# theislab/dca

Hardware: AMD Instinct MI355X
Metric: cells/sec training (ZINB AE, 68k x 20k) (higher is better)
Workload: dtype f32

## Files before the change

dca_amd/build.py:

```python
import os
import shutil
import subprocess
import sys

HERE = os.path.dirname(os.path.abspath(__file__))
ROOT = os.path.dirname(HERE)
CSRC = os.path.join(HERE, 'csrc')
LIB = os.path.join(CSRC, 'libdcahip.so')
SOURCES = ['dcahip_zinb.hip', 'dcahip_gemm.hip', 'dcahip_layers.hip', 'dcahip_heads.hip', 'dcahip_prep.hip', 'dcahip_opt.hip',
           'dcahip_dropout.hip', 'dcahip_sparse.hip', 'dcahip_peer.hip', 'dcahip_knn.hip', 'dcahip_kmeans.hip', 'dcahip_gram.hip',
           'dcahip_silhouette.hip', 'dcahip_ranksum.hip', 'dcahip_louvain.hip']
HEADERS = ['zinb_math.hpp', 'h2_math.hpp', 'philox.hpp', 'knn_dist.hpp']
ARCH = 'gfx950'
HOST_LIB = os.path.join(CSRC, 'libdcahost.so')
HOST_SOURCES = ['dcahost_tsv.cpp', 'dcahost_read.cpp']


def _hipcc():
    for c in (shutil.which('hipcc'), '/opt/rocm/bin/hipcc'):
        if c and os.path.exists(c):
            return c
    raise RuntimeError('hipcc not found: cannot build libdcahip.so')


def _deps():
    return [os.path.join(CSRC, s) for s in SOURCES + HEADERS] + [os.path.join(ROOT, 'include', 'dcahip.h')]


def source_fingerprint():
    import hashlib
    h = hashlib.sha256()
    for d in _deps():
        h.update(os.path.basename(d).encode())
        if os.path.exists(d):
            with open(d, 'rb') as f:
                h.update(f.read())
    return h.hexdigest()


def needs_build():
    if not os.path.exists(LIB):
        return True
    t = os.path.getmtime(LIB)
    if any(os.path.exists(d) and os.path.getmtime(d) > t for d in _deps()):
        return True
    try:
        with open(LIB + '.src') as f:
            return f.read().strip() != source_fingerprint()
    except OSError:
        return True


def _obj_path(src, tag):
    return os.path.join(CSRC, '_obj', os.path.basename(src) + ('.' + tag if tag else '') + '.o')


def _obj_fingerprint(src, hdrs, defines):
    import hashlib
    h = hashlib.sha256()
    for d in [src] + list(hdrs):
        h.update(os.path.basename(d).encode())
        with open(d, 'rb') as f:
            h.update(f.read())
    h.update('\0'.join(defines).encode())
    return h.hexdigest()


def _obj_is_fresh(obj, fp):
    try:
        with open(obj + '.src') as f:
            return os.path.exists(obj) and f.read().strip() == fp
    except OSError:
        return False


def build_hip(force=False, verbose=True, defines=(), out=None):
    out = out or LIB
    if not force and not defines and out == LIB and not needs_build():
        return LIB
    from concurrent.futures import ThreadPoolExecutor
    os.makedirs(os.path.join(CSRC, '_obj'), exist_ok=True)
    tag = '_'.join(d.replace('=', '-') for d in defines)
    hdrs = [os.path.join(CSRC, h) for h in HEADERS] + [os.path.join(ROOT, 'include', 'dcahip.h')]
    hdrs = [h for h in hdrs if os.path.exists(h)]
    srcs = [os.path.join(CSRC, s) for s in SOURCES if os.path.exists(os.path.join(CSRC, s))]
    jobs, stamps = [], []
    for src in srcs:
        obj = _obj_path(src, tag)
        fp = _obj_fingerprint(src, hdrs, defines)
        if force or not _obj_is_fresh(obj, fp):
            if os.path.exists(obj + '.src'):
                os.remove(obj + '.src')
            jobs.append([_hipcc(), '--offload-arch=' + ARCH, '-O3', '-std=c++17', '-fPIC', '-c',
                         '-I' + os.path.join(ROOT, 'include')] + ['-D' + d for d in defines] + ['-o', obj, src])
            stamps.append((obj, fp))
# ... 44 lines not shown
```

dca_amd/config.py:

```python
import os
from dataclasses import dataclass, fields


def _flag(name, default):
    v = os.environ.get(name)
    return default if v is None else v not in ('0', '', 'off', 'false', 'False')


@dataclass
class EngineConfig:
    stack: str = 'steps'
    bwd_chain: bool = True
    wide_planes: bool = True
    wide_h2: bool = True
    dp_sharded_opt: bool = False
    dp_graph: bool = True
    dp_peer_exchange: bool = False
    device_prep: bool = True
    fused_write: bool = True
    resident: str = 'auto'
    counts_compact: bool = False
    graph_steps: int = 8
    sparse_dw_min: int = 512
    lut_fwd_min: int = 1024
    enc0_nt_min: int = 256
    predict_chunk: int = 1024

    _ENV = {'stack': 'DCA_AMD_STACK', 'bwd_chain': 'DCA_AMD_BWD_CHAIN', 'wide_planes': 'DCA_AMD_WIDE_PLANES', 'wide_h2': 'DCA_AMD_WIDE_H2',
            'dp_sharded_opt': 'DCA_AMD_DP_SHARDED_OPT', 'dp_graph': 'DCA_AMD_DP_GRAPH', 'device_prep': 'DCA_AMD_DEVICE_PREP',
            'fused_write': 'DCA_AMD_FUSED_WRITE', 'dp_peer_exchange': 'DCA_AMD_DP_PEER', 'resident': 'DCA_AMD_RESIDENT',
            'counts_compact': 'DCA_AMD_COUNTS_COMPACT'}

    @classmethod
    def from_env(cls):
        c = cls()
        for f in fields(cls):
            env = cls._ENV.get(f.name)
            if env is None:
                continue
            if f.type is bool or isinstance(getattr(c, f.name), bool):
                setattr(c, f.name, _flag(env, getattr(c, f.name)))
            elif os.environ.get(env) is not None:
                setattr(c, f.name, type(getattr(c, f.name))(os.environ[env]))
        if c.stack not in ('steps', 'coop', 'off'):
            raise ValueError('DCA_AMD_STACK must be steps, coop or off (got %r)' % c.stack)
        if c.resident not in ('auto', 'counts', 'dense'):
            raise ValueError('DCA_AMD_RESIDENT must be auto, counts or dense (got %r)' % c.resident)
        return c


def current():
    return EngineConfig.from_env()
```

dca_amd/csrc/dcahip_heads.hip:

```cpp
#include <hip/hip_runtime.h>
#include <stdint.h>
#include <type_traits>
#include "dcahip.h"
#include "zinb_math.hpp"

namespace {

using f32x16 = __attribute__((ext_vector_type(16))) float;

constexpr int kTG = 32;
constexpr int kTR = 32;
constexpr int kLdS = 33;
constexpr int kWG = 2;
constexpr int kMaxGrid = 2048;
constexpr int kMaxSmallGrid = 8192;
constexpr int kCUs = 256;
constexpr int kZU = 4;
constexpr int kQCap = 320;

__device__ __forceinline__ int rowmap(int e, int hi) { return (e & 3) + 8 * (e >> 2) + 4 * hi; }

__device__ __forceinline__ void wave_sync() {
    __builtin_amdgcn_fence(__ATOMIC_RELEASE, "wavefront");
    __builtin_amdgcn_wave_barrier();
    __builtin_amdgcn_fence(__ATOMIC_ACQUIRE, "wavefront");
}

using f16x8 = __attribute__((ext_vector_type(8))) _Float16;
using f16x2v = __attribute__((ext_vector_type(2))) _Float16;
using f32x2v = __attribute__((ext_vector_type(2))) float;
using u32x4 = __attribute__((ext_vector_type(4))) unsigned;
using u32x2 = __attribute__((ext_vector_type(2))) unsigned;
using s16x4 = __attribute__((ext_vector_type(4))) short;

constexpr int kWR2 = 8;
constexpr int kWr8MinNT = 5;
constexpr int kHTile = 2 * 32 * 64;
constexpr int kTop = 13;
constexpr int kDExp0 = 8;
constexpr float kDLim = 30000.f;
constexpr int kDSlack = 2;
constexpr int kEHZero = 64;

#define MFMAH(a, b, c) __builtin_amdgcn_mfma_f32_32x32x16_f16(__builtin_bit_cast(f16x8, a), __builtin_bit_cast(f16x8, b), c, 0, 0, 0)

__device__ __forceinline__ unsigned pk_f16(float a, float b) {
    return __builtin_bit_cast(unsigned, __builtin_convertvector(f32x2v{a, b}, f16x2v));
}
__device__ __forceinline__ float resid_lo(unsigned p, float x) {
    float r;
    asm("v_fma_mix_f32 %0, %1, -1.0, %2 op_sel:[0,0,0] op_sel_hi:[1,0,0]" : "=v"(r) : "v"(p), "v"(x));
    return r;
}
__device__ __forceinline__ float resid_hi(unsigned p, float x) {
    float r;
    asm("v_fma_mix_f32 %0, %1, -1.0, %2 op_sel:[1,0,0] op_sel_hi:[1,0,0]" : "=v"(r) : "v"(p), "v"(x));
    return r;
}
__device__ __forceinline__ void split_pair(float x0, float x1, unsigned& p0, unsigned& p1) {
    p0 = pk_f16(x0, x1);
    p1 = pk_f16(resid_lo(p0, x0), resid_hi(p0, x1));
}
__device__ __forceinline__ void split8(const float (&x)[8], u32x4 (&f)[2]) {
#pragma unroll
    for (int j = 0; j < 4; ++j) {
        unsigned a, b;
        split_pair(x[2 * j], x[2 * j + 1], a, b);
        f[0][j] = a; f[1][j] = b;
    }
}
#ifdef DCA_EXP_H2_TWO
#define MFMA_H3(A, Bf, ACC) { ACC = MFMAH(A[0], Bf[1], ACC); ACC = MFMAH(A[0], Bf[0], ACC); }
#else
#define MFMA_H3(A, Bf, ACC) { ACC = MFMAH(A[1], Bf[0], ACC); ACC = MFMAH(A[0], Bf[1], ACC); ACC = MFMAH(A[0], Bf[0], ACC); }
#endif

__device__ __forceinline__ float pow2i(int e) { return __uint_as_float((unsigned)(127 + e) << 23); }
__device__ __forceinline__ int block_exp(float m) {
    if (!(m > 0.f) || !(m < INFINITY)) return 0;
    const int e = kTop + 1 - __builtin_amdgcn_frexp_expf(m);
    return e < -60 ? -60 : (e > 60 ? 60 : e);
}
__device__ __forceinline__ float wave_max(float v) {
    int l = (int)__builtin_amdgcn_mbcnt_hi(~0u, __builtin_amdgcn_mbcnt_lo(~0u, 0u));
    asm volatile("" : "+v"(l));
#pragma unroll
    for (int off = 32; off > 0; off >>= 1)
// ... 651 lines not shown

    __syncthreads();

    {
        float* red = lds;
#pragma unroll
        for (int step = 1; step < WR; step *= 2) {
            const int slot = r / (2 * step);
            float* rs = red + (long)slot * NRED * 64 + lane;
            if (r % (2 * step) == step) {
                int n = 0;
#pragma unroll
                for (int h = 0; h < NH; ++h)
#pragma unroll
                    for (int ib = 0; ib < 2; ++ib)
#pragma unroll
                        for (int e = 0; e < 16; ++e) rs[(n++) * 64] = dW[h][ib][e];
#pragma unroll
                for (int h = 0; h < NH; ++h) rs[(n++) * 64] = bsum[h];
                rs[(n++) * 64] = thsum;
            }
            __syncthreads();
            if (r % (2 * step) == 0 && r + step < WR) {
                int n = 0;
#pragma unroll
                for (int h = 0; h < NH; ++h)
#pragma unroll
                    for (int ib = 0; ib < 2; ++ib)
#pragma unroll
                        for (int e = 0; e < 16; ++e) dW[h][ib][e] += rs[(n++) * 64];
#pragma unroll
                for (int h = 0; h < NH; ++h) bsum[h] += rs[(n++) * 64];
                thsum += rs[(n++) * 64];
            }
            __syncthreads();
        }
    }
    if (r == 0 && tile_ok) {
        const bool direct = p.S == 1;
        float* out = direct ? p.gW : p.ws_dw + (long)s * p.dw_stride;
        const long ldo = direct ? p.ldg : p.ldws;
        const float fin = direct ? p.inv_n : 1.f;
        const bool cw = gene < p.plane;
#pragma unroll
        for (int h = 0; h < NH; ++h) {
#pragma unroll
            for (int ib = 0; ib < 2; ++ib)
#pragma unroll
                for (int e = 0; e < 16; ++e) {
                    const int i = ib * 32 + rowmap(e, hi);
                    if (cw && i < p.hL) out[(long)i * ldo + (long)h * p.plane + gene] = dW[h][ib][e] * fin;
                }
            const float bv = bsum[h] + __shfl_xor(bsum[h], 32, 64);
            if (cw && hi == 0) out[(long)p.hL * ldo + (long)h * p.plane + gene] = bv * fin;
        }
        if (CONST_DISP) {
            const float tv = thsum + __shfl_xor(thsum, 32, 64);
            if (direct) {
                if (gvalid && hi == 0) {
                    const float e = expf(p.theta_w[gene]);
                    p.g_theta[gene] = (e >= 1e-3f && e <= 1e4f) ? tv * p.inv_n * e : 0.f;
                }
            } else if (cw && hi == 0) {
                out[(long)(p.hL + 1) * ldo + gene] = tv;
            }
        }
    }
    __syncthreads();
    first_item = false;
    }

#pragma unroll
    for (int off = 32; off > 0; off >>= 1) dacc += __shfl_down(dacc, off, 64);
    if (lane == 0) lred[wave] = dacc;
    __syncthreads();
    if (tid == 0) {
        double v = 0.0;
        for (int w = 0; w < WR; ++w) v += lred[w];
        p.partials[blockIdx.x] = v;
    }
}


struct ReduceDwArgs {
    const float* ws; int S; long stride; int hL; long ldws, ncols; float* gW; long ldg;
    const float* theta_w; float* g_theta; int G;
    float scale;
    const float* ws2; int S2; const int* tail_tiles; int ntail; long plane;
    int tail_first;
};

__device__ __forceinline__ void reduce_dw_body(const ReduceDwArgs& q, int bid, int nblk) {
    const int hL = q.hL;
    const long ldws = q.ldws, ncols = q.ncols; float* gW = q.gW; const long ldg = q.ldg;
    const float* theta_w = q.theta_w; float* g_theta = q.g_theta; const int G = q.G;
    const float sc = q.scale;
    __shared__ unsigned tailbm[kMaxGrid / 32];
    if (q.ntail > 0) {
        for (int i = threadIdx.x; i < kMaxGrid / 32; i += 256) tailbm[i] = 0u;
        __syncthreads();
        for (int i = threadIdx.x; i < q.ntail; i += 256) {
            const int tl = q.tail_tiles ? q.tail_tiles[i] : q.tail_first + i;
            if (tl >= 0 && tl < kMaxGrid) atomicOr(&tailbm[tl >> 5], 1u << (tl & 31));
        }
        __syncthreads();
    }
    auto is_tail = [&](long col_in_plane) { const int tl = (int)(col_in_plane / kTG); return q.ntail > 0 && ((tailbm[tl >> 5] >> (tl & 31)) & 1u); };
    if ((ncols & 3) == 0 && (ldws & 3) == 0 && (ldg & 3) == 0 && (q.stride & 3) == 0 && (q.plane & 3) == 0 &&
        ((reinterpret_cast<uintptr_t>(q.ws) | reinterpret_cast<uintptr_t>(gW) | reinterpret_cast<uintptr_t>(q.ws2)) & 15) == 0) {
        const long nq = ncols >> 2, totalq = (long)(hL + 1) * nq;
        for (long idx = (long)bid * 256 + threadIdx.x; idx < totalq; idx += (long)nblk * 256) {
            const long i = idx / nq, c = (idx - i * nq) << 2;
            const bool tl = is_tail(c % q.plane);
            const float* ws = tl ? q.ws2 : q.ws; const int S = tl ? q.S2 : q.S; const long stride = q.stride;
            float4 v = *reinterpret_cast<const float4*>(ws + i * ldws + c);
            for (int s = 1; s < S; ++s) {
                const float4 x = *reinterpret_cast<const float4*>(ws + (long)s * stride + i * ldws + c);
                v.x += x.x; v.y += x.y; v.z += x.z; v.w += x.w;
            }
            v.x *= sc; v.y *= sc; v.z *= sc; v.w *= sc;
            *reinterpret_cast<float4*>(gW + i * ldg + c) = v;
        }
    } else {
        const long total = (long)(hL + 1) * ncols;
        for (long idx = (long)bid * 256 + threadIdx.x; idx < total; idx += (long)nblk * 256) {
            const long i = idx / ncols, c = idx - i * ncols;
            const bool tl = is_tail(c % q.plane);
            const float* ws = tl ? q.ws2 : q.ws; const int S = tl ? q.S2 : q.S;
            float v = 0.f;
            for (int s = 0; s < S; ++s) v += ws[(long)s * q.stride + i * ldws + c];
            gW[i * ldg + c] = v * sc;
        }
    }
    if (g_theta) {
        for (long c = (long)bid * 256 + threadIdx.x; c < G; c += (long)nblk * 256) {
            const bool tl = is_tail(c);
            const float* ws = tl ? q.ws2 : q.ws; const int S = tl ? q.S2 : q.S; const long stride = q.stride;
            float v = 0.f;
            for (int s = 0; s < S; ++s) v += ws[(long)s * stride + (long)(hL + 1) * ldws + c];
            const float e = expf(theta_w[c]);
            g_theta[c] = (e >= 1e-3f && e <= 1e4f) ? v * sc * e : 0.f;
        }
    }
}

__global__ __launch_bounds__(256) void heads_reduce_dw_kernel(ReduceDwArgs q) { reduce_dw_body(q, blockIdx.x, gridDim.x); }

struct ReduceDhArgs {
    const float* ws; int ntg, B, Bpad, KT, hL; float* dH; long lddh; float scale;
    const double* loss_partials; int n_partials; double loss_scale; float* loss_out;
    const float* ws2; int ntg2;
};

template <int GL>
__device__ __forceinline__ void reduce_dh_body(const ReduceDhArgs& q, int bid) {
    const float* ws = q.ws; const int ntg = q.ntg, B = q.B, KT = q.KT, hL = q.hL; float* dH = q.dH; const long lddh = q.lddh;
    const double* loss_partials = q.loss_partials; const int n_partials = q.n_partials; const double loss_scale = q.loss_scale;
    float* loss_out = q.loss_out;
    constexpr int OUT = 256 / GL;
    __shared__ float4 red[256];
    const int o = threadIdx.x % OUT, gl = threadIdx.x / OUT;
    const int q4 = KT / 4;
    const long nq = (long)B * q4;
    const long quad = (long)bid * OUT + o;
    float4 v = make_float4(0.f, 0.f, 0.f, 0.f);
    if (quad < nq) {
        const long tq = (long)kTR * q4;
        const long t = quad / tq, within = quad - t * tq;
        const float4* src = reinterpret_cast<const float4*>(ws) + t * ntg * tq + within;
        for (int gt0 = gl; gt0 < ntg; gt0 += 8 * GL) {
            float4 x[8];
#pragma unroll
            for (int u = 0; u < 8; ++u) {
                const int gt = gt0 + u * GL;
                x[u] = src[(long)(gt < ntg ? gt : gl) * tq];
            }
#pragma unroll
            for (int u = 0; u < 8; ++u)
                if (gt0 + u * GL < ntg) { v.x += x[u].x; v.y += x[u].y; v.z += x[u].z; v.w += x[u].w; }
        }
        if (q.ntg2 > 0) {
            const float4* src2 = reinterpret_cast<const float4*>(q.ws2) + t * q.ntg2 * tq + within;
            for (int gt = gl; gt < q.ntg2; gt += GL) { const float4 x = src2[(long)gt * tq]; v.x += x.x; v.y += x.y; v.z += x.z; v.w += x.w; }
        }
    }
    red[threadIdx.x] = v;
    __syncthreads();
    if (gl == 0 && quad < nq) {
#pragma unroll
        for (int k = 1; k < GL; ++k) {
            const float4 x = red[k * OUT + o];
            v.x += x.x; v.y += x.y; v.z += x.z; v.w += x.w;
        }
        const long row = quad / q4;
        const int i = (int)(quad - row * q4) * 4;
        float* d = dH + row * lddh + i;
        if (i + 0 < hL) d[0] = v.x * q.scale;
        if (i + 1 < hL) d[1] = v.y * q.scale;
        if (i + 2 < hL) d[2] = v.z * q.scale;
        if (i + 3 < hL) d[3] = v.w * q.scale;
    }
    if (loss_out && bid == 0) {
        __shared__ double lsum[256];
        double a = 0.0;
        for (int i = threadIdx.x; i < n_partials; i += 256) a += loss_partials[i];
        lsum[threadIdx.x] = a;
        __syncthreads();
        for (int st = 128; st > 0; st >>= 1) {
            if ((int)threadIdx.x < st) lsum[threadIdx.x] += lsum[threadIdx.x + st];
            __syncthreads();
        }
        if (threadIdx.x == 0) {
            float lf = (float)(lsum[0] * loss_scale);
            if (isnan(lf)) lf = INFINITY;
            *loss_out = lf;
        }
    }
}

template <int GL>
__global__ __launch_bounds__(256) void heads_reduce_dh_kernel(ReduceDhArgs q) { reduce_dh_body<GL>(q, blockIdx.x); }

template <int GL>
__global__ __launch_bounds__(256) void heads_reduce_both_kernel(ReduceDhArgs qh, ReduceDwArgs qw, int n_dh) {
    if ((int)blockIdx.x < n_dh) reduce_dh_body<GL>(qh, blockIdx.x);
    else reduce_dw_body(qw, blockIdx.x - n_dh, gridDim.x - n_dh);
}
// ... 463 lines not shown
        const long ldo = p.NT == 1 ? p.ldg : p.ldws;
        const float fin = p.NT == 1 ? p.inv_n : 1.f;
        const float wun = pow2i(-(eHt + kD0 - shift)) * 1.f;
#pragma unroll
        for (int ib = 0; ib < 2; ++ib)
#pragma unroll
            for (int e = 0; e < 16; ++e) {
                const int i = ib * 32 + rowmap(e, hi);
                const float v = dW[ib][e] * wun * fin;
                if (cw && i < p.hL) out[(long)i * ldo + (long)h * p.plane + gene] = v;
            }
        const float bv = (bsum + __shfl_xor(bsum, 32, 64)) * pow2i(-kD0) * fin;
        if (cw && hi == 0) out[(long)p.hL * ldo + (long)h * p.plane + gene] = bv;
    }

#pragma unroll
    for (int off = 32; off > 0; off >>= 1) dacc += __shfl_down(dacc, off, 64);
    if (lane == 0) lred[wave] = dacc;
    __syncthreads();
    if (tid == 0) p.partials[blockIdx.x] = ((lred[0] + lred[1]) + lred[2]) + lred[3];
}

__global__ __launch_bounds__(64) void x3_product_kernel(const float* A, const float* B, float* C, int K) {
    const int lane = threadIdx.x, l31 = lane & 31, hi = lane >> 5;
    float ma = 0.f, mb = 0.f;
    for (int k0 = 0; k0 < K; k0 += 16)
#pragma unroll
        for (int j = 0; j < 8; ++j) {
            ma = fmaxf(ma, fabsf(A[(long)l31 * K + k0 + 8 * hi + j]));
            mb = fmaxf(mb, fabsf(B[(long)(k0 + 8 * hi + j) * 32 + l31]));
        }
    const int ea = block_exp(wave_max(ma)), eb = block_exp(wave_max(mb));
    const float sa = pow2i(ea), sb = pow2i(eb);
    f32x16 acc;
#pragma unroll
    for (int e = 0; e < 16; ++e) acc[e] = 0.f;
    for (int k0 = 0; k0 < K; k0 += 16) {
        float av[8], bv[8];
#pragma unroll
        for (int j = 0; j < 8; ++j) {
            av[j] = A[(long)l31 * K + k0 + 8 * hi + j] * sa;
            bv[j] = B[(long)(k0 + 8 * hi + j) * 32 + l31] * sb;
        }
        u32x4 af[2], bf[2];
        split8(av, af);
        split8(bv, bf);
        MFMA_H3(af, bf, acc)
    }
    const float un = pow2i(-(ea + eb));
#pragma unroll
    for (int e = 0; e < 16; ++e) C[rowmap(e, hi) * 32 + l31] = acc[e] * un;
}

template <bool P, bool C, bool YC>
void launch_fused(const HeadsPlan& pl, const HeadsArgs2& a, hipStream_t s) {
    if (pl.small) hipLaunchKernelGGL((heads_fused_small_kernel<P, C, YC>), dim3(pl.grid), dim3(256), 0, s, a);
    else hipLaunchKernelGGL((heads_fused_h2_kernel<P, C, YC>), dim3(pl.grid), dim3(64 * kWR2), 0, s, a);
}

}

extern "C" long dcahip_heads_fused_workspace_bytes(int B, int hL, int G, long plane, int flags) {
    HeadsPlan p;
    if (!make_heads_plan(B, hL, G, plane, flags, &p)) return 0;
    long need = 0;
    for (int nt = 1; nt <= p.NT; ++nt) {
        const int b = nt * kTR < B ? nt * kTR : B;
        HeadsPlan q;
        if (!make_heads_plan(b, hL, G, plane, flags, &q)) continue;
        const long n = q.dw_bytes + q.dh_bytes + q.hs_bytes + q.dw2_bytes + q.dh2_bytes;
        if (n > need) need = n;
    }
    return need;
}

extern "C" int dcahip_x3_product_32x32(const float* A, const float* B, float* C, int K, void* stream) {
    if (!A || !B || !C || K <= 0 || (K & 15)) return DCAHIP_EINVAL;
    hipLaunchKernelGGL(x3_product_kernel, dim3(1), dim3(64), 0, static_cast<hipStream_t>(stream), A, B, C, K);
    return (int)hipGetLastError();
}

extern "C" int dcahip_heads_tile_order_len(int G) { return G > 0 ? (((G + kTG - 1) / kTG + kWG - 1) / kWG) * kWG : 0; }

extern "C" int dcahip_heads_fused(const float* H, long ldh, const float* Wh, long ldw,
                                  const float* bh, long plane, const float* theta_w,
                                  const float* y, long ldy,
                                  const unsigned char* yc, long ldc, const int* ovf_ptr, const int* ovf_col,
                                  const float* ovf_val, const float* sf, const int* perm,
                                  const long long* cursor, int B, int hL, int G, float ridge,
                                  float inv_n, int flags, float* gW, long ldg, float* g_theta,
                                  float* dH, long lddh, double* loss_partials, int* n_partials_out,
                                  void* workspace, long workspace_bytes, const int* tile_order,
                                  float* loss_out, int d_exp, void* stream) {
    const bool has_pi = flags & DCAHIP_NLL_HAS_PI, cdisp = flags & DCAHIP_NLL_CONST_DISP;
    HeadsPlan pl;
    if (!make_heads_plan(B, hL, G, plane, flags, &pl)) return DCAHIP_EINVAL;
    if (!H || !Wh || !bh || (!y && !yc) || !sf || !gW || !dH || !loss_partials || !workspace) return DCAHIP_EINVAL;
    if (cdisp && (!theta_w || !g_theta)) return DCAHIP_EINVAL;
    if (workspace_bytes < pl.dw_bytes + pl.dh_bytes + pl.hs_bytes + pl.dw2_bytes + pl.dh2_bytes) return DCAHIP_EINVAL;
    if (!al16(H) || !al16(Wh) || !al16(workspace) || (ldh & 3) || (ldw & 3) || ldh < ((hL + 3) & ~3))
        return DCAHIP_EINVAL;
    if (d_exp > 0 || d_exp < -24 || !(ridge >= 0.f) || ridge > 1e3f) return DCAHIP_EINVAL;
    const int NH = 1 + (cdisp ? 0 : 1) + (has_pi ? 1 : 0);
    if (ldw < (long)NH * plane || ldg < (long)NH * plane) return DCAHIP_EINVAL;
    if (yc ? (ldc < G || ldc > 0xffffffffL) : (ldy < G || ldy > 0xffffffffL)) return DCAHIP_EINVAL;
    float* ws_dh = static_cast<float*>(workspace);
    float* ws_dw = ws_dh + pl.dh_bytes / sizeof(float);
    float* ws_dh2 = ws_dw + pl.dw_bytes / sizeof(float);
    float* ws_dw2 = ws_dh2 + pl.dh2_bytes / sizeof(float);
    hipStream_t s = static_cast<hipStream_t>(stream);
    bool direct_dw = false;
    {
        unsigned short* HA = reinterpret_cast<unsigned short*>(reinterpret_cast<char*>(workspace) + pl.dh_bytes + pl.dw_bytes +
                                                               pl.dh2_bytes + pl.dw2_bytes);
        unsigned short* HT = HA + (long)pl.NT * kHTile;
        int* eH = reinterpret_cast<int*>(HT + (long)pl.NT * kHTile);
        if (!pl.small) {
            hipLaunchKernelGGL(heads_split_h_kernel, dim3(pl.NT), dim3(256), 0, s, H, ldh, B, hL, HA, HT, eH);
            int rc0 = (int)hipGetLastError();
            if (rc0 != 0) return rc0;
        }
        direct_dw = pl.S == 1;
        HeadsArgs2 a{HA, HT, eH, H, ldh, gW, ldg, g_theta, Wh, ldw, bh, theta_w, y, ldy, yc, ldc, ovf_ptr, ovf_col, ovf_val,
                     sf, perm, cursor, ws_dw, pl.dw_stride, ws_dh,
                     pl.npart, pl.nitems, tile_order, loss_partials, plane, pl.ldws, B, hL, G, pl.S, pl.NT, ridge, inv_n, d_exp, 0};
        auto launch = [&](const HeadsPlan& q, const HeadsArgs2& b) {
            if (yc) {
                if (has_pi && cdisp) launch_fused<true, true, true>(q, b, s);
                else if (has_pi) launch_fused<true, false, true>(q, b, s);
                else if (cdisp) launch_fused<false, true, true>(q, b, s);
                else launch_fused<false, false, true>(q, b, s);
            } else {
                if (has_pi && cdisp) launch_fused<true, true, false>(q, b, s);
                else if (has_pi) launch_fused<true, false, false>(q, b, s);
                else if (cdisp) launch_fused<false, true, false>(q, b, s);
                else launch_fused<false, false, false>(q, b, s);
            }
        };
        launch(pl, a);
        if (pl.ntail > 0) {
            HeadsPlan q2 = pl;
            q2.grid = pl.grid2; q2.S = pl.S2;
            HeadsArgs2 b = a;
            b.ws_dw = ws_dw2; b.ws_dh = ws_dh2; b.npart = pl.npart2; b.nitems = pl.nitems2; b.S = pl.S2;
            b.partials = loss_partials + pl.grid; b.tile_base = pl.nmain;
            launch(q2, b);
        }
    }
    int rc = (int)hipGetLastError();
    if (rc != 0) return rc;
    const int n_part = pl.grid + pl.grid2;
    if (n_partials_out) *n_partials_out = n_part;
    {
        const int KT = pl.HLB * 32;
        const long nq = (long)B * (KT / 4);
        const ReduceDhArgs qh{ws_dh, pl.npart, B, pl.NT * kTR, KT, hL, dH, lddh, inv_n, loss_partials, n_part, (double)inv_n, loss_out,
                              ws_dh2, pl.npart2};
        const long total = (long)(hL + 1) * pl.ldws;
        long gr = (total / 4 + 255) / 256;
        if (gr > 2048) gr = 2048;
        if (gr < 1) gr = 1;
        const ReduceDwArgs qw{ws_dw, pl.S, pl.dw_stride, hL, pl.ldws, pl.ldws, gW, ldg, cdisp ? theta_w : nullptr,
                              cdisp ? g_theta : nullptr, G, inv_n,
                              ws_dw2, pl.S2, (pl.ntail > 0 && tile_order) ? tile_order + pl.nmain : nullptr, pl.ntail, plane, pl.nmain};
        const int gl = (nq <= 1024 && pl.npart >= 256) ? 64 : (nq >= 64L * 512 ? 4 : 16);
        const int n_dh = (int)((nq + 256 / gl - 1) / (256 / gl));
        if (!direct_dw) {
            const dim3 grid(n_dh + (int)gr);
            if (gl == 64) hipLaunchKernelGGL(heads_reduce_both_kernel<64>, grid, dim3(256), 0, s, qh, qw, n_dh);
            else if (gl == 4) hipLaunchKernelGGL(heads_reduce_both_kernel<4>, grid, dim3(256), 0, s, qh, qw, n_dh);
            else hipLaunchKernelGGL(heads_reduce_both_kernel<16>, grid, dim3(256), 0, s, qh, qw, n_dh);
        } else {
            if (gl == 64) hipLaunchKernelGGL(heads_reduce_dh_kernel<64>, dim3(n_dh), dim3(256), 0, s, qh);
            else if (gl == 4) hipLaunchKernelGGL(heads_reduce_dh_kernel<4>, dim3(n_dh), dim3(256), 0, s, qh);
            else hipLaunchKernelGGL(heads_reduce_dh_kernel<16>, dim3(n_dh), dim3(256), 0, s, qh);
        }
        rc = (int)hipGetLastError();
    }
    return rc;
}
```

dca_amd/csrc/dcahip_layers.hip:

```cpp
#include <hip/hip_runtime.h>
#include <stdint.h>
#include "dcahip.h"

namespace {

constexpr int kMaxChunks = 256;
constexpr int kApplyRows = 16;

constexpr float kSeluScale = 1.0507009873554805f, kSeluAlpha = 1.6732632423543772f;
constexpr int kActPre = 12;

__device__ __attribute__((noinline)) float act_fwd_other(int a, float x) {
    switch (a) {
        case 2: return tanhf(x);
        case 3: { const float e = expf(-fabsf(x)); const float s = 1.f / (1.f + e); return x >= 0.f ? s : e * s; }
        case 4: return x > 0.f ? x : expm1f(x);
        case 5: return kSeluScale * (x > 0.f ? x : kSeluAlpha * expm1f(x));
        case 6: return fmaxf(x, 0.f) + log1pf(expf(-fabsf(x)));
        case 7: return x / (1.f + fabsf(x));
        case 10: return fminf(fmaxf(0.2f * x + 0.5f, 0.f), 1.f);
        case 11: return expf(x);
        case 12: { const float e = expf(-fabsf(x)); const float s = 1.f / (1.f + e); return x * (x >= 0.f ? s : e * s); }
        case 13: return 0.5f * x * (1.f + erff(x * 0.70710678118654752f));
        default: return x > 0.f ? x : 0.3f * x;
    }
}
__device__ __forceinline__ float act_fwd(int a, float x) {
    if (a == 1) return fmaxf(x, 0.f);
    if (a == 0) return x;
    return act_fwd_other(a, x);
}

__device__ __attribute__((noinline)) float act_grad_other(int a, float v) {
    switch (a) {
        case 2: return 1.f - v * v;
        case 3: return v * (1.f - v);
        case 4: return v > 0.f ? 1.f : v + 1.f;
        case 5: return v > 0.f ? kSeluScale : v + kSeluScale * kSeluAlpha;
        case 6: return -expm1f(-v);
        case 7: { const float t = 1.f - fabsf(v); return t * t; }
        case 10: return v > 0.f && v < 1.f ? 0.2f : 0.f;
        case 11: return v;
        case 12: {
            const float e = expf(-fabsf(v)); const float s0 = 1.f / (1.f + e); const float s = v >= 0.f ? s0 : e * s0;
            return s * (1.f + v * (1.f - s));
        }
        case 13:
            return 0.5f * (1.f + erff(v * 0.70710678118654752f)) + v * 0.39894228040143268f * expf(-0.5f * v * v);
        default: return v > 0.f ? 1.f : 0.3f;
    }
}
__device__ __forceinline__ float act_grad(int a, float h) {
    if (a == 1) return h > 0.f ? 1.f : 0.f;
    if (a == 0) return 1.f;
    return act_grad_other(a, h);
}
__device__ __forceinline__ float act_slope(int a, float h, float xh, float bc) {
    if (a == 1) return h > 0.f ? 1.f : 0.f;
    if (a == 0) return 1.f;
    return act_grad_other(a, a >= kActPre ? xh + bc : h);
}
__device__ __forceinline__ float pre_beta(int a, const float* beta, int c) {
    return a >= kActPre ? beta[c] : 0.f;
}

__host__ __device__ inline int n_chunks(int B) {
    int r = (B + 63) / 64;
    return r < 1 ? 1 : (r > kMaxChunks ? kMaxChunks : r);
}
__host__ __device__ inline int chunk_rows(int B, int R) { return (B + R - 1) / R; }
inline int strip_blocks(int H, int row_blocks) {
    const int strips = (H + 63) / 64;
    int y = row_blocks > 0 ? 512 / row_blocks : strips;
    if (y < 1) y = 1;
    return y < strips ? y : strips;
}

__device__ __forceinline__ float wg_rowlane_sum(float v, float* sm ) {
    const int tx = threadIdx.x & 63, ty = threadIdx.x >> 6;
    __syncthreads();
    sm[ty * 64 + tx] = v;
    __syncthreads();
    return (sm[tx] + sm[64 + tx]) + (sm[128 + tx] + sm[192 + tx]);
}

// ... 737 lines not shown
            for (int r = 0; r < a.B; ++r) {
                const float d = dZs[r][c];
                cs += d;
#pragma unroll
                for (int j = 0; j < NK; ++j) {
                    const int k = wg + kBwdWGs * (ty + 4 * j);
                    acc[j] = fmaf(k < a.K ? Hs[r][k] : 0.f, d, acc[j]);
                }
            }
#pragma unroll
            for (int j = 0; j < NK; ++j) {
                const int k = wg + kBwdWGs * (ty + 4 * j);
                if (k < a.K) a.gW[(long)k * a.ldg + c] = acc[j];
            }
            if (wg == 0 && ty == 0) a.gW[(long)a.K * a.ldg + c] = cs;
        }
    }
    if (a.dHp) {
        const int k = tx;
        if (k < a.K) {
            constexpr int NR = RPT / kBwdWGs;
            float acc[NR];
#pragma unroll
            for (int j = 0; j < NR; ++j) acc[j] = 0.f;
            for (int c = 0; c < a.H; ++c) {
                const float w = Ws[k][c];
#pragma unroll
                for (int j = 0; j < NR; ++j) {
                    const int r = wg + kBwdWGs * (ty + 4 * j);
                    acc[j] = fmaf(r < a.B ? dZs[r][c] : 0.f, w, acc[j]);
                }
            }
#pragma unroll
            for (int j = 0; j < NR; ++j) {
                const int r = wg + kBwdWGs * (ty + 4 * j);
                if (r < a.B) a.dHp[(long)r * a.lddp + k] = acc[j];
            }
        }
    }
}

__global__ __launch_bounds__(256) void relu_bwd_kernel(const float* dH, long ldd, const float* Hact,
                                                       long ldh, int B, int H, float* dZ, long ldz, int act) {
    const long total = (long)B * H;
    for (long i = (long)blockIdx.x * 256 + threadIdx.x; i < total; i += (long)gridDim.x * 256) {
        const int r = (int)(i / H), c = (int)(i - (long)r * H);
        dZ[(long)r * ldz + c] = dH[(long)r * ldd + c] * act_grad(act, Hact[(long)r * ldh + c]);
    }
}

__global__ __launch_bounds__(256) void relu_fwd_kernel(const float* Z, long ldz, int B, int H,
                                                       float* Hout, long ldh, int act) {
    const long total = (long)B * H;
    for (long i = (long)blockIdx.x * 256 + threadIdx.x; i < total; i += (long)gridDim.x * 256) {
        const int r = (int)(i / H), c = (int)(i - (long)r * H);
        Hout[(long)r * ldh + c] = act_fwd(act, Z[(long)r * ldz + c]);
    }
}

__global__ __launch_bounds__(256) void colsum_chain_kernel(const float* x, long ldx, int B, int N,
                                                           const float* theta_w, float* out) {
    __shared__ float sm[256];
    const int tx = threadIdx.x & 63, ty = threadIdx.x >> 6;
    const int c = blockIdx.x * 64 + tx;
    float s = 0.f;
    if (c < N) for (int i = ty; i < B; i += 4) s += x[(long)i * ldx + c];
    const float tot = wg_rowlane_sum(s, sm);
    if (c < N && ty == 0) {
        float chain = 1.f;
        if (theta_w) {
            const float e = expf(theta_w[c]);
            chain = (e >= 1e-3f && e <= 1e4f) ? e : 0.f;
        }
        out[c] = tot * chain;
    }
}

struct StepEnd {
    const float* loss; double weight; float* hist; int rows_per_slot; double* acc; long long* cursor; int advance; int on;
};

__global__ __launch_bounds__(256) void rmsprop_clip_kernel(float* w, const float* g, float* ms,
                                                           long n, const float* lrp, float rho,
                                                           float eps, float clip, StepEnd se) {
    if (se.on && blockIdx.x == 0 && threadIdx.x == 0) {
        const long long c = se.cursor ? *se.cursor : 0;
        if (se.loss) {
            const float l = *se.loss;
            if (se.hist) se.hist[se.rows_per_slot > 0 ? c / se.rows_per_slot : 0] = l;
            if (se.acc) *se.acc += (double)l * se.weight;
        }
        if (se.cursor) *se.cursor = c + se.advance;
    }
    const float lr = *lrp;
    const long nv = n >> 2;
    const long stride = (long)gridDim.x * 256;
    for (long i = (long)blockIdx.x * 256 + threadIdx.x; i < nv; i += stride) {
        float4 gv = reinterpret_cast<const float4*>(g)[i];
        float4 mv = reinterpret_cast<const float4*>(ms)[i];
        float4 wv = reinterpret_cast<const float4*>(w)[i];
        float* gp = &gv.x; float* mp = &mv.x; float* wp = &wv.x;
#pragma unroll
        for (int j = 0; j < 4; ++j) {
            float gj = gp[j];
            if (clip > 0.f) gj = fminf(fmaxf(gj, -clip), clip);
            mp[j] = rho * mp[j] + (1.f - rho) * gj * gj;
            wp[j] = wp[j] - lr * gj / (sqrtf(mp[j]) + eps);
        }
        reinterpret_cast<float4*>(ms)[i] = mv;
        reinterpret_cast<float4*>(w)[i] = wv;
    }
    for (long i = (nv << 2) + (long)blockIdx.x * 256 + threadIdx.x; i < n; i += stride) {
        float gj = g[i];
        if (clip > 0.f) gj = fminf(fmaxf(gj, -clip), clip);
        const float m = rho * ms[i] + (1.f - rho) * gj * gj;
        ms[i] = m;
        w[i] = w[i] - lr * gj / (sqrtf(m) + eps);
    }
}

__global__ __launch_bounds__(256) void transpose_kernel(const float* __restrict__ src, long lds_, int R, int C,
                                                        float* __restrict__ dst, long ldd,
                                                        const int* __restrict__ perm, const long long* __restrict__ cursor) {
    __shared__ float tile[32][33];
    const int tx = threadIdx.x & 31, ty = threadIdx.x >> 5;
    const int r0 = blockIdx.y * 32, c0 = blockIdx.x * 32;
    const long long cur = (perm && cursor) ? *cursor : 0;
#pragma unroll
    for (int k = 0; k < 4; ++k) {
        const int r = r0 + ty + 8 * k, c = c0 + tx;
        float v = 0.f;
        if (r < R && c < C) {
            const long sr = perm ? (long)perm[cur + r] : (long)r;
            v = src[sr * lds_ + c];
        }
        tile[ty + 8 * k][tx] = v;
    }
    __syncthreads();
#pragma unroll
    for (int k = 0; k < 4; ++k) {
        const int c = c0 + ty + 8 * k, r = r0 + tx;
        if (c < C && r < R) dst[(long)c * ldd + r] = tile[tx][ty + 8 * k];
    }
}

__global__ __launch_bounds__(256) void transpose64_kernel(const float* __restrict__ src, long lds_, int R, int C,
                                                          float* __restrict__ dst, long ldd,
                                                          const int* __restrict__ perm, const long long* __restrict__ cursor) {
    __shared__ float tile[64][65];
    const int tq = threadIdx.x & 15, tr = threadIdx.x >> 4;
    const int r0 = blockIdx.y * 64, c0 = blockIdx.x * 64;
    const long long cur = (perm && cursor) ? *cursor : 0;
    float4 v[4];
#pragma unroll
    for (int k = 0; k < 4; ++k) {
        const int r = r0 + tr + 16 * k, c = c0 + 4 * tq;
        const int rc = r < R ? r : R - 1;
        const long sr = perm ? (long)perm[cur + rc] : (long)rc;
        v[k] = *reinterpret_cast<const float4*>(src + sr * lds_ + (c < C ? c : 0));
    }
#pragma unroll
    for (int k = 0; k < 4; ++k) {
        const int r = tr + 16 * k, c = 4 * tq;
        tile[r][c] = v[k].x; tile[r][c + 1] = v[k].y; tile[r][c + 2] = v[k].z; tile[r][c + 3] = v[k].w;
    }
    __syncthreads();
#pragma unroll
    for (int k = 0; k < 4; ++k) {
        const int c = tr + 16 * k, r = 4 * tq;
        if (c0 + c < C) {
            const float4 o = make_float4(tile[r][c], tile[r + 1][c], tile[r + 2][c], tile[r + 3][c]);
            float* d = dst + (long)(c0 + c) * ldd + r0 + r;
            if (r0 + r + 4 <= R) *reinterpret_cast<float4*>(d) = o;
            else {
                if (r0 + r < R) d[0] = o.x;
                if (r0 + r + 1 < R) d[1] = o.y;
                if (r0 + r + 2 < R) d[2] = o.z;
            }
        }
    }
}

constexpr int kStackMaxLayers = 8;
constexpr int kStackRows = 64;
constexpr int kStackMaxWG = 256;
constexpr int kStackLd = 68;

struct StackBwdLayer {
    const float* W; long ldw; int K, H;
    const float* Hact; long ldh; const float* xhat; long ldx; const float* inv_std;
    const float* Hprev; long ldp;
    float* gW; long ldg; float* dbeta;
    float* dHin; long lddh;
    const float* beta;
};

struct StackFwdArgs {
    SmallLayer l[kStackMaxLayers];
    int n, B, act, nwg, first, last;
    float momentum, eps;
// ... 331 lines not shown
            }
        }
        __syncthreads();
        prep(i - 1, false, true);
        fresh = true;
    }
    if (a.last > a.n) {
        if (fresh) grid_barrier(a.sync, (unsigned)nwg * (++nbar));
        for (int i = 1; i < a.n; ++i) {
            const StackBwdLayer& L = a.l[i];
            const int total = (L.K + 1) * L.H;
            const float* gw = a.gwp + (long)i * nwg * 65 * 64;
            const int el = tid & 31, sl = tid >> 5;
            const int per = (nwg + 7) / 8;
            for (int e0 = wg * 32; e0 < total; e0 += nwg * 32) {
                const int e = e0 + el;
                const int ec = e < total ? e : total - 1;
                const int k = ec / L.H, cc = ec - k * L.H;
                const float* src = gw + (long)k * 64 + cc;
                float v = 0.f;
                for (int b0 = sl * per; b0 < min(nwg, (sl + 1) * per); b0 += 16) {
                    float pv[16];
#pragma unroll
                    for (int u = 0; u < 16; ++u) pv[u] = src[(long)min(b0 + u, nwg - 1) * 65 * 64];
#pragma unroll
                    for (int u = 0; u < 16; ++u) if (b0 + u < min(nwg, (sl + 1) * per)) v += pv[u];
                }
                __syncthreads();
                smf[tid] = v;
                __syncthreads();
                if (tid < 32 && e < total) {
                    float t = 0.f;
#pragma unroll
                    for (int q8 = 0; q8 < 8; ++q8) t += smf[q8 * 32 + tid];
                    L.gW[(long)k * L.ldg + cc] = t;
                }
            }
        }
    }
    if (nbar) grid_exit(a.sync, (unsigned)nwg);
}

__device__ __forceinline__ bool w_tile_vec(const float* W, long ldw, int H) {
    return (H & 3) == 0 && (ldw & 3) == 0 && (reinterpret_cast<uintptr_t>(W) & 15) == 0;
}
template <int VEC = 0>
__device__ __forceinline__ void w_tile_request(const float* W, long ldw, int K, int H, int tid, float4 (&wv)[4]) {
    if (VEC == 0 && (!W || K <= 0)) {
#pragma unroll
        for (int q = 0; q < 4; ++q) wv[q] = make_float4(0.f, 0.f, 0.f, 0.f);
        return;
    }
    const bool vec = VEC == 1 || (VEC == 0 && w_tile_vec(W, ldw, H));
    if (vec) {
#pragma unroll
        for (int q = 0; q < 4; ++q) {
            const int idx = tid + 256 * q, k = min(idx >> 4, K - 1), c4 = min((idx & 15) * 4, H - 4);
            wv[q] = *reinterpret_cast<const float4*>(W + (long)k * ldw + c4);
        }
    } else {
#pragma unroll
        for (int q = 0; q < 4; ++q) {
            const int idx = tid + 256 * q, k = min(idx >> 4, K - 1), c4 = (idx & 15) * 4;
            const float* src = W + (long)k * ldw;
            wv[q].x = src[min(c4 + 0, H - 1)]; wv[q].y = src[min(c4 + 1, H - 1)];
            wv[q].z = src[min(c4 + 2, H - 1)]; wv[q].w = src[min(c4 + 3, H - 1)];
        }
    }
}
__device__ __forceinline__ void w_tile_store(float* wl, int K, int H, int tid, const float4 (&wv)[4]) {
#pragma unroll
    for (int q = 0; q < 4; ++q) {
        const int idx = tid + 256 * q, k = idx >> 4, c4 = (idx & 15) * 4;
        float4 v = wv[q];
        if (k >= K || c4 + 0 >= H) v.x = 0.f;
        if (k >= K || c4 + 1 >= H) v.y = 0.f;
        if (k >= K || c4 + 2 >= H) v.z = 0.f;
        if (k >= K || c4 + 3 >= H) v.w = 0.f;
        *reinterpret_cast<float4*>(wl + k * kStackLd + c4) = v;
    }
}

constexpr int kStepRows = 32;

struct StepFwdArgs {
    SmallLayer cur, nxt;
    int B, act, nwg, stats_only;
    float momentum, eps;
    const float* part_in;
    float* part_out;
    const float* ext_in; const float* ext_counts; int ext_E;
};

__global__ __launch_bounds__(256) void stack_fwd_step_kernel(StepFwdArgs a) {
    __shared__ __attribute__((aligned(16))) float ht[kStepRows * kStackLd];
    __shared__ __attribute__((aligned(16))) float wl[64 * kStackLd];
    __shared__ float smf[256];
    __shared__ double smd[1024];
    const int tid = threadIdx.x, tx = tid & 63, ty = tid >> 6;
    const int wg = blockIdx.x, E = a.nwg;
    const int cr = chunk_rows(a.B, E);
    const int r0 = wg * cr;
    const int nrows = max(0, min(a.B, r0 + cr) - r0);
    const int c = tx;
    const SmallLayer& L = a.cur;
    const int H = L.H, cc = c < H ? c : H - 1;
    float z[kStepRows / 4];
#pragma unroll
    for (int j = 0; j < kStepRows / 4; ++j) {
        const int r = ty + 4 * j;
        z[j] = L.Z[(long)(r0 + (r < nrows ? r : (nrows > 0 ? nrows - 1 : 0))) * L.ldz + cc];
    }
    float out_z[kStepRows / 4];
    int Hs = H;
    if (!a.stats_only) {
        const bool ext = a.ext_in && !(a.ext_E == 1 && a.ext_counts[0] == (float)a.B);
        const float* const ein = ext ? a.ext_in : a.part_in;
        const float* const cnt = ext ? a.ext_counts : nullptr;
        const int Em = ext ? a.ext_E : E;
        float pm[32], pq[32];
#pragma unroll
        for (int u = 0; u < 32; ++u) {
            const long eo = (long)(ty + 4 * u < Em ? ty + 4 * u : Em - 1) * 2;
            pm[u] = ein[(eo + 0) * H + cc]; pq[u] = ein[(eo + 1) * H + cc];
        }
        const SmallLayer& N = a.nxt;
        const int K = H, HN = N.W ? N.H : 0;
        float4 wv[4];
        w_tile_request(N.W, N.ldw, N.W ? K : 0, HN, tid, wv);
        const float beta = L.beta ? L.beta[cc] : 0.f;
        const float nbias = (N.W && N.bias && c < HN) ? N.bias[c] : 0.f;
        double n = 0.0, sw = 0.0, sq = 0.0;
#pragma unroll
        for (int u = 0; u < 32; ++u) {
            const int e = ty + 4 * u;
            const double ne = (e < Em && c < H) ? entry_count(cnt, e, Em, a.B) : 0.0;
            n += ne; sw += ne * (double)pm[u]; sq += ne > 0.0 ? (double)pq[u] + ne * (double)pm[u] * (double)pm[u] : 0.0;
        }
        for (int e0 = ty + 128; e0 < Em; e0 += 128) {
#pragma unroll 4
            for (int u = 0; u < 32; ++u) {
                const int e = e0 + 4 * u;
                if (e < Em && c < H) {
                    const double ne = entry_count(cnt, e, Em, a.B);
                    const double me = (double)ein[((long)e * 2 + 0) * H + cc], qe = (double)ein[((long)e * 2 + 1) * H + cc];
                    n += ne; sw += ne * me; sq += ne > 0.0 ? qe + ne * me * me : 0.0;
                }
            }
        }
        smd[ty * 64 + tx] = n; smd[256 + ty * 64 + tx] = sw; smd[512 + ty * 64 + tx] = sq;
        __syncthreads();
        n = (smd[tx] + smd[64 + tx]) + (smd[128 + tx] + smd[192 + tx]);
        sw = (smd[256 + tx] + smd[320 + tx]) + (smd[384 + tx] + smd[448 + tx]);
        sq = (smd[512 + tx] + smd[576 + tx]) + (smd[640 + tx] + smd[704 + tx]);
        const double meand = n > 0.0 ? sw / n : 0.0;
        const float mean = (float)meand;
        double m2 = sq - n * meand * meand;
        if (m2 < 0.0) m2 = 0.0;
        const float var = n > 0.0 ? bn_var(m2, n) : 0.f;
        const float inv = bn_inv_std(var, a.eps);
        if (wg == 0 && ty == 0 && c < H) {
            L.mm[c] = bn_moving(L.mm[c], mean, a.momentum);
            L.mv[c] = bn_moving(L.mv[c], var, a.momentum);
            if (L.inv_std) L.inv_std[c] = inv;
        }
#pragma unroll
        for (int j = 0; j < kStepRows / 4; ++j) {
            const int r = ty + 4 * j;
            float h = 0.f;
            if (r < nrows && c < H) {
                const float xh = bn_xhat(z[j], mean, inv);
                h = act_fwd(a.act, xh + beta);
                if (L.xhat) L.xhat[(long)(r0 + r) * L.ldx + c] = xh;
                L.Hout[(long)(r0 + r) * L.ldh + c] = h;
            }
            ht[r * kStackLd + c] = h;
        }
        if (!N.W) return;
        w_tile_store(wl, K, HN, tid, wv);
        __syncthreads();
        float acc[kStepRows / 4];
#pragma unroll
        for (int j = 0; j < kStepRows / 4; ++j) acc[j] = 0.f;
        tile_fwd<kStepRows / 4, kStackLd, kStackLd, 0>(acc, wl, ht, (K + 3) & ~3, tx, ty);
        Hs = HN;
#pragma unroll
        for (int j = 0; j < kStepRows / 4; ++j) {
            const int r = ty + 4 * j;
            out_z[j] = acc[j] + nbias;
            if (r < nrows && c < HN && N.Z) N.Z[(long)(r0 + r) * N.ldz + c] = out_z[j];
        }
    } else {
#pragma unroll
        for (int j = 0; j < kStepRows / 4; ++j) out_z[j] = z[j];
    }
    float sv = 0.f;
#pragma unroll
    for (int j = 0; j < kStepRows / 4; ++j) if (ty + 4 * j < nrows && c < Hs) sv += out_z[j];
    const float tot = wg_rowlane_sum(sv, smf);
    const float bmean = nrows > 0 ? tot / (float)nrows : 0.f;
    float q = 0.f;
#pragma unroll
    for (int j = 0; j < kStepRows / 4; ++j) if (ty + 4 * j < nrows && c < Hs) { const float d = out_z[j] - bmean; q += d * d; }
    const float bm2 = wg_rowlane_sum(q, smf);
    if (c < Hs && ty == 0) {
        a.part_out[((long)wg * 2 + 0) * Hs + c] = bmean;
        a.part_out[((long)wg * 2 + 1) * Hs + c] = bm2;
    }
}

struct StepBwdArgs {
    StackBwdLayer cur, low;
    int B, act, nwg, sums_only;
    float n_total;
    float* dZ0; long ldz0;
    const float* part_in;
    float* part_out;
    float* gwp;
    const float* ext_in;
};

__global__ __launch_bounds__(256) void stack_bwd_step_kernel(StepBwdArgs a) {
    __shared__ __attribute__((aligned(16))) float dyt[kStepRows * kStackLd];
    __shared__ __attribute__((aligned(16))) float ht[kStepRows * kStackLd];
    __shared__ __attribute__((aligned(16))) float wl[64 * kStackLd];
    __shared__ float smf[256];
    const int tid = threadIdx.x, tx = tid & 63, ty = tid >> 6;
    const int wg = blockIdx.x, E = a.nwg;
    const int cr = chunk_rows(a.B, E);
    const int r0 = wg * cr;
    const int nrows = max(0, min(a.B, r0 + cr) - r0);
    const int c = tx;
    const StackBwdLayer& L = a.cur;
    const int H = L.H, cc = c < H ? c : H - 1;
    float dh[kStepRows / 4], hv[kStepRows / 4], xv[kStepRows / 4];
#pragma unroll
    for (int j = 0; j < kStepRows / 4; ++j) {
        const int r = ty + 4 * j;
        const long row = r0 + (r < nrows ? r : (nrows > 0 ? nrows - 1 : 0));
        dh[j] = L.dHin[row * L.lddh + cc]; hv[j] = L.Hact[row * L.ldh + cc]; xv[j] = L.xhat[row * L.ldx + cc];
    }
    float dy[kStepRows / 4];
    const float bc = pre_beta(a.act, L.beta, cc);
    if (a.sums_only) {
        float s1 = 0.f, s2 = 0.f;
        tile_dy_sums(dy, xv, c < H, nrows, ty, [&](int j) { return dh[j] * act_slope(a.act, hv[j], xv[j], bc); }, s1, s2);
        const float t1 = wg_rowlane_sum(s1, smf), t2 = wg_rowlane_sum(s2, smf);
        if (c < H && ty == 0) { a.part_out[((long)wg * 2 + 0) * H + c] = t1; a.part_out[((long)wg * 2 + 1) * H + c] = t2; }
        return;
    }
    const float* const ein = a.ext_in ? a.ext_in : a.part_in;
    const int Em = a.ext_in ? 1 : E;
    float p1[16], p2[16];
#pragma unroll
    for (int u = 0; u < 16; ++u) {
        const long eo = (long)(ty + 4 * u < Em ? ty + 4 * u : Em - 1) * 2;
        p1[u] = ein[(eo + 0) * H + cc]; p2[u] = ein[(eo + 1) * H + cc];
    }
    const bool has_low = a.low.Hact != nullptr;
    const int K = has_low ? L.K : 0;
    float4 wv[4];
    float hp[kStepRows / 4];
    w_tile_request(has_low ? L.W : nullptr, L.ldw, K, H, tid, wv);
#pragma unroll
    for (int j = 0; j < kStepRows / 4; ++j) {
        const int r = ty + 4 * j;
        const long row = r0 + (r < nrows ? r : (nrows > 0 ? nrows - 1 : 0));
        const int kc = tx < K ? tx : (K > 0 ? K - 1 : 0);
        hp[j] = has_low ? L.Hprev[row * L.ldp + kc] : 0.f;
    }
    const float inv = L.inv_std[cc];
    float v1 = 0.f, v2 = 0.f;
#pragma unroll
    for (int u = 0; u < 16; ++u) if (ty + 4 * u < Em && c < H) { v1 += p1[u]; v2 += p2[u]; }
#pragma unroll 1
    for (int e0 = ty + 64; e0 < Em; e0 += 64) {
        float q1[16], q2[16];
#pragma unroll
        for (int u = 0; u < 16; ++u) {
            const long eo = (long)(e0 + 4 * u < Em ? e0 + 4 * u : Em - 1) * 2;
            q1[u] = ein[(eo + 0) * H + cc]; q2[u] = ein[(eo + 1) * H + cc];
        }
#pragma unroll
        for (int u = 0; u < 16; ++u) if (e0 + 4 * u < Em && c < H) { v1 += q1[u]; v2 += q2[u]; }
    }
    v1 = wg_rowlane_sum(v1, smf);
    v2 = wg_rowlane_sum(v2, smf);
    if (wg == 0 && ty == 0 && c < H && L.dbeta && !a.ext_in) L.dbeta[c] = v1;
    const float m1 = v1 / a.n_total, m2 = v2 / a.n_total;
#pragma unroll
    for (int j = 0; j < kStepRows / 4; ++j) {
        const int r = ty + 4 * j;
        float dz = 0.f;
        if (r < nrows && c < H) {
            dz = bn_dz(inv, dh[j] * act_slope(a.act, hv[j], xv[j], bc), xv[j], m1, m2);
            if (!has_low) a.dZ0[(long)(r0 + r) * a.ldz0 + c] = dz;
        }
        dyt[r * kStackLd + c] = dz;
        ht[r * kStackLd + tx] = (r < nrows && tx < K) ? hp[j] : 0.f;
    }
    if (!has_low) return;
    w_tile_store(wl, K, H, tid, wv);
    __syncthreads();
    float lh[kStepRows / 4], lx[kStepRows / 4];
#pragma unroll
// ... 437 lines not shown
    double sk = 0.0, sc = 0.0;
    for (int r = blockIdx.y; r < B; r += gridDim.y) {
        const float dp = d_pi[(long)r * ldd + g];
        sk += (double)(dp * m[(long)r * lda + g]);
        sc += (double)dp;
        d_mean[(long)r * ldd + g] = -(d_mean[(long)r * ldd + g] + kg * dp);
    }
    partial[((long)blockIdx.y * 2 + 0) * G + g] = sk;
    partial[((long)blockIdx.y * 2 + 1) * G + g] = sc;
}

__global__ __launch_bounds__(256) void elempi_finish_kernel(const double* __restrict__ partial, int R, int G,
                                                            float* __restrict__ gk, float* __restrict__ gc) {
    const int g = blockIdx.x * 256 + threadIdx.x;
    if (g >= G) return;
    double sk = 0.0, sc = 0.0;
    for (int y = 0; y < R; ++y) {
        sk += partial[((long)y * 2 + 0) * G + g];
        sc += partial[((long)y * 2 + 1) * G + g];
    }
    gk[g] = (float)sk;
    gc[g] = (float)sc;
}

constexpr int kElemPiSlices = 32;

extern "C" int dcahip_elempi_workspace_doubles(int G) { return G > 0 ? kElemPiSlices * 2 * G : 0; }

extern "C" int dcahip_elempi_fwd(float* a_mean, long lda, const float* k, const float* c, int B, int G,
                                 float* a_pi, long ldp, void* stream) {
    if (!a_mean || !k || !c || !a_pi || B <= 0 || G <= 0 || lda < G || ldp < G) return DCAHIP_EINVAL;
    const int gy = B < 64 ? B : 64;
    hipLaunchKernelGGL(elempi_fwd_kernel, dim3((G + 255) / 256, gy), dim3(256), 0, static_cast<hipStream_t>(stream),
                       a_mean, lda, k, c, B, G, a_pi, ldp);
    return (int)hipGetLastError();
}

extern "C" int dcahip_elempi_bwd(const float* m, long lda, float* d_mean, const float* d_pi, long ldd, const float* k,
                                 int B, int G, float* gk, float* gc, double* workspace, void* stream) {
    if (!m || !d_mean || !d_pi || !k || !gk || !gc || !workspace || B <= 0 || G <= 0 || lda < G || ldd < G)
        return DCAHIP_EINVAL;
    const int R = B < kElemPiSlices ? B : kElemPiSlices;
    hipStream_t s = static_cast<hipStream_t>(stream);
    hipLaunchKernelGGL(elempi_bwd_kernel, dim3((G + 255) / 256, R), dim3(256), 0, s, m, lda, d_mean, d_pi, ldd, k, B, G,
                       workspace);
    hipLaunchKernelGGL(elempi_finish_kernel, dim3((G + 255) / 256), dim3(256), 0, s, workspace, R, G, gk, gc);
    return (int)hipGetLastError();
}

extern "C" int dcahip_bcast_cols(const float* s, long lds, int B, int G, float* out, long ldo, void* stream) {
    if (!s || !out || B <= 0 || G <= 0 || ldo < G || lds < 1) return DCAHIP_EINVAL;
    int gx = (G + 255) / 256;
    if (gx > 64) gx = 64;
    hipLaunchKernelGGL(bcast_cols_kernel, dim3(gx, B), dim3(256), 0, static_cast<hipStream_t>(stream), s, lds, B, G, out, ldo);
    return (int)hipGetLastError();
}

extern "C" int dcahip_row_sums_strided(const float* x, long ldx, int B, int G, float* out, long ldo, void* stream) {
    if (!x || !out || B <= 0 || G <= 0 || ldx < G || ldo < 1) return DCAHIP_EINVAL;
    hipLaunchKernelGGL(row_sums_strided_kernel, dim3((B + 3) / 4), dim3(256), 0, static_cast<hipStream_t>(stream),
                       x, ldx, B, G, out, ldo);
    return (int)hipGetLastError();
}

extern "C" int dcahip_colsum_chain(const float* x, long ldx, int B, int N, const float* theta_w,
                                   float* out, void* stream) {
    if (!x || !out || B <= 0 || N <= 0) return DCAHIP_EINVAL;
    hipLaunchKernelGGL(colsum_chain_kernel, dim3((N + 63) / 64), dim3(256), 0,
                       static_cast<hipStream_t>(stream), x, ldx, B, N, theta_w, out);
    return (int)hipGetLastError();
}

extern "C" int dcahip_rmsprop_clip(float* w, const float* g, float* ms, long n, const float* lr,
                                   float rho, float eps, float clip, const float* loss, double weight,
                                   float* hist, int rows_per_slot, double* acc, long long* cursor, int advance,
                                   void* stream) {
    if (!w || !g || !ms || !lr || n <= 0) return DCAHIP_EINVAL;
    if (!al16(w) || !al16(g) || !al16(ms)) return DCAHIP_EINVAL;
    long grid = ((n >> 2) + 255) / 256;
    if (grid > 2048) grid = 2048;
    if (grid < 1) grid = 1;
    hipLaunchKernelGGL(rmsprop_clip_kernel, dim3((int)grid), dim3(256), 0,
                       static_cast<hipStream_t>(stream), w, g, ms, n, lr, rho, eps, clip,
                       StepEnd{loss, weight, hist, rows_per_slot, acc, cursor, advance, (loss || hist || acc || cursor) ? 1 : 0});
    return (int)hipGetLastError();
}

extern "C" int dcahip_hidden_stack_max_rows(void) { return kStackMaxWG * kStackRows; }

extern "C" long dcahip_hidden_stack_workspace_bytes(int n_layers, int B) {
    if (n_layers < 1 || n_layers > kStackMaxLayers || B <= 0 || B > kStackMaxWG * kStackRows) return 0;
    const long nwg = stack_workgroups(B, 16);
    return 256 + ((long)n_layers * nwg * 2 * 64 + (long)n_layers * nwg * 65 * 64) * (long)sizeof(float);
}

static int stack_plan(int n, int B, int rows_per_wg, int first, int last, int nsteps, int* nwg_out) {
    if (rows_per_wg < 16 || rows_per_wg > kStackRows || first < 0 || last < first || last >= nsteps) return DCAHIP_EINVAL;
    const int nwg = stack_workgroups(B, rows_per_wg);
    if (nwg > kStackMaxPhaseWG) return DCAHIP_EINVAL;
    if (last > first && nwg > kStackMaxWG) return DCAHIP_EINVAL;
    *nwg_out = nwg;
    return 0;
}

static bool stack_shape_ok(const void* layers, int n, int B) {
    return layers && n >= 1 && n <= kStackMaxLayers && B > 0 && B <= kStackMaxWG * kStackRows;
}

static bool stack_workspace_ok(const void* workspace, long workspace_bytes, int n, int B) {
    return workspace && workspace_bytes >= dcahip_hidden_stack_workspace_bytes(n, B) && al16(workspace);
}

static bool stack_fwd_layers(const dcahip_small_layer* layers, int n, bool need_z, SmallLayer* l) {
    for (int i = 0; i < n; ++i) {
        const dcahip_small_layer& q = layers[i];
        if (q.H <= 0 || q.H > 64 || !q.Hout || !q.moving_mean || !q.moving_var) return false;
        if (i == 0 ? !q.Z : (!q.W || q.K != layers[i - 1].H || (need_z && !q.Z))) return false;
        l[i] = small_layer(q);
    }
    return true;
}

static bool stack_bwd_layers(const dcahip_stack_bwd_layer* layers, int n, int act, bool need_dh, StackBwdLayer* l) {
    for (int i = 0; i < n; ++i) {
        const dcahip_stack_bwd_layer& q = layers[i];
        if (q.H <= 0 || q.H > 64 || !q.Hact || !q.xhat || !q.inv_std || (act >= kActPre && !q.beta)) return false;
        if (i > 0 && (!q.W || !q.Hprev || !q.gW || q.K != layers[i - 1].H || q.K > 64)) return false;
        if (!q.dH && (i == n - 1 || need_dh)) return false;
        l[i] = StackBwdLayer{q.W, q.ldw, q.K, q.H, q.Hact, q.ldh, q.xhat, q.ldx, q.inv_std, q.Hprev, q.ldp, q.gW, q.ldg,
                             q.dbeta, q.dH, q.lddh, q.beta};
    }
    return true;
}

static StepFwdArgs stack_fwd_step(const SmallLayer* l, int n, int B, float momentum, float eps, int act, int step, int nwg,
                                  float* part) {
    StepFwdArgs q{};
    const int i = step == 0 ? 0 : step - 1;
    q.cur = l[i];
    if (step > 0 && i + 1 < n) q.nxt = l[i + 1];
    q.B = B; q.act = act; q.nwg = nwg; q.stats_only = step == 0; q.momentum = momentum; q.eps = eps;
    q.part_in = part + (long)i * nwg * 2 * 64;
    q.part_out = part + (long)step * nwg * 2 * 64;
    return q;
}

static int stack_bwd_made(int n, int step) { return step == 0 ? n - 1 : n - step - 1; }

static StepBwdArgs stack_bwd_step(const StackBwdLayer* l, int n, int B, float n_total, int act, float* dZ0, long ldz0, int step,
                                  int nwg, float* part) {
    StepBwdArgs q{};
    const int i = step == 0 ? n - 1 : n - step;
    const int made = stack_bwd_made(n, step);
    q.cur = l[i];
    if (step > 0 && i > 0) q.low = l[i - 1];
    q.B = B; q.act = act; q.nwg = nwg; q.sums_only = step == 0; q.n_total = n_total;
    q.dZ0 = dZ0; q.ldz0 = ldz0;
    q.part_in = part + (long)i * nwg * 2 * 64;
    q.part_out = part + (long)(made >= 0 ? made : 0) * nwg * 2 * 64;
    q.gwp = part + (long)n * nwg * 2 * 64 + (long)i * nwg * 65 * 64;
    return q;
}

extern "C" int dcahip_hidden_stack_fwd(const dcahip_small_layer* layers, int n, int B, float momentum, float eps, int act,
                                       int rows_per_wg, int first_step, int last_step,
                                       void* workspace, long workspace_bytes, void* stream) {
    if (!stack_shape_ok(layers, n, B) || !stack_workspace_ok(workspace, workspace_bytes, n, B)) return DCAHIP_EINVAL;
    StackFwdArgs a{};
    if (stack_plan(n, B, rows_per_wg, first_step, last_step, n + 1, &a.nwg)) return DCAHIP_EINVAL;
    if (!stack_fwd_layers(layers, n, !(first_step == 0 && last_step == n), a.l)) return DCAHIP_EINVAL;
    a.n = n; a.B = B; a.act = act; a.first = first_step; a.last = last_step; a.momentum = momentum; a.eps = eps;
    a.sync = static_cast<unsigned*>(workspace);
    a.part = reinterpret_cast<float*>(static_cast<char*>(workspace) + 256);
    if (first_step == last_step && rows_per_wg == kStepRows) {
        const StepFwdArgs q = stack_fwd_step(a.l, n, B, momentum, eps, act, first_step, a.nwg, a.part);
        hipLaunchKernelGGL(stack_fwd_step_kernel, dim3(a.nwg), dim3(256), 0, static_cast<hipStream_t>(stream), q);
        return (int)hipGetLastError();
    }
    hipLaunchKernelGGL(hidden_stack_fwd_kernel, dim3(a.nwg), dim3(256), 0, static_cast<hipStream_t>(stream), a);
    return (int)hipGetLastError();
}

extern "C" int dcahip_hidden_stack_step_blocks(int B) { return B > 0 ? stack_workgroups(B, kStepRows) : 0; }

extern "C" int dcahip_hidden_stack_fwd_sync(const dcahip_small_layer* layers, int n, int B, float momentum, float eps, int act,
                                            int step, const float* ext_entries, const float* ext_counts, int ext_E,
                                            float* stat_out, void* workspace, long workspace_bytes, void* stream) {
    if (!stack_shape_ok(layers, n, B) || !stack_workspace_ok(workspace, workspace_bytes, n, B)) return DCAHIP_EINVAL;
    if (step < 0 || step > n || (step > 0 && (!ext_entries || !ext_counts || ext_E <= 0))) return DCAHIP_EINVAL;
    const int nwg = stack_workgroups(B, kStepRows);
    if (nwg > kStackMaxPhaseWG) return DCAHIP_EINVAL;
    SmallLayer l[kStackMaxLayers];
    if (!stack_fwd_layers(layers, n, true, l)) return DCAHIP_EINVAL;
    float* part = reinterpret_cast<float*>(static_cast<char*>(workspace) + 256);
    StepFwdArgs q = stack_fwd_step(l, n, B, momentum, eps, act, step, nwg, part);
    if (step > 0) { q.ext_in = ext_entries; q.ext_counts = ext_counts; q.ext_E = ext_E; }
    hipStream_t st = static_cast<hipStream_t>(stream);
    hipLaunchKernelGGL(stack_fwd_step_kernel, dim3(nwg), dim3(256), 0, st, q);
    if (step < n && stat_out) {
        const int Hm = l[step].H;
        hipLaunchKernelGGL(moments_combine_kernel, dim3((Hm + 63) / 64), dim3(256), 0, st,
                           (const float*)q.part_out, (const float*)nullptr, nwg, Hm, stat_out, B);
    }
    return (int)hipGetLastError();
}

extern "C" int dcahip_hidden_stack_bwd_sync(const dcahip_stack_bwd_layer* layers, int n, int B, float n_total, int act,
                                            float* dZ0, long ldz0, int step, const float* ext_sums, float* sums_out,
                                            void* workspace, long workspace_bytes, void* stream) {
    if (!stack_shape_ok(layers, n, B) || !dZ0 || !stack_workspace_ok(workspace, workspace_bytes, n, B)) return DCAHIP_EINVAL;
    if (step < 0 || step > n || (step > 0 && !ext_sums)) return DCAHIP_EINVAL;
    const int nwg = stack_workgroups(B, kStepRows);
    if (nwg > kStackMaxPhaseWG) return DCAHIP_EINVAL;
    StackBwdLayer l[kStackMaxLayers];
    if (!stack_bwd_layers(layers, n, act, true, l)) return DCAHIP_EINVAL;
    float* part = reinterpret_cast<float*>(static_cast<char*>(workspace) + 256);
    StepBwdArgs q = stack_bwd_step(l, n, B, n_total, act, dZ0, ldz0, step, nwg, part);
    if (step > 0) q.ext_in = ext_sums;
    hipStream_t st = static_cast<hipStream_t>(stream);
    hipLaunchKernelGGL(stack_bwd_step_kernel, dim3(nwg), dim3(256), 0, st, q);
    const int made = stack_bwd_made(n, step);
    if (made >= 0 && sums_out)
        hipLaunchKernelGGL(stack_sums_combine_kernel, dim3(1), dim3(64), 0, st, (const float*)q.part_out, nwg, l[made].H, sums_out,
                           l[made].dbeta);
    return (int)hipGetLastError();
}

extern "C" int dcahip_hidden_stack_bwd(const dcahip_stack_bwd_layer* layers, int n, int B, float n_total, int act,
                                       float* dZ0, long ldz0, int rows_per_wg, int first_step, int last_step,
                                       void* workspace, long workspace_bytes, void* stream) {
    if (!stack_shape_ok(layers, n, B) || !dZ0) return DCAHIP_EINVAL;
    const bool one_launch = first_step == 0 && last_step == n + 1;
    const bool chain = one_launch && B <= kStackRows && n <= 4;
    if (!chain && !stack_workspace_ok(workspace, workspace_bytes, n, B)) return DCAHIP_EINVAL;
    StackBwdArgs a{};
    if (stack_plan(n, B, rows_per_wg, first_step, last_step, n + 2, &a.nwg)) return DCAHIP_EINVAL;
    if (!stack_bwd_layers(layers, n, act, !one_launch, a.l)) return DCAHIP_EINVAL;
    a.n = n; a.B = B; a.act = act; a.first = first_step; a.last = last_step; a.n_total = n_total;
    a.dZ0 = dZ0; a.ldz0 = ldz0;
    if (chain) {
        ChainBwdArgs q{};
        for (int i = 0; i < n; ++i) q.l[i] = a.l[i];
        q.B = B; q.act = act; q.n_total = n_total; q.dZ0 = dZ0; q.ldz0 = ldz0;
        bool vec = true;
        for (int i = 1; i < n; ++i) vec = vec && (q.l[i].H & 3) == 0 && (q.l[i].ldw & 3) == 0 && al16(q.l[i].W);
        hipStream_t st = static_cast<hipStream_t>(stream);
        if (B <= 32) { if (vec) launch_bwd_chain<8, true>(n, q, st); else launch_bwd_chain<8, false>(n, q, st); }
        else { if (vec) launch_bwd_chain<16, true>(n, q, st); else launch_bwd_chain<16, false>(n, q, st); }
        return (int)hipGetLastError();
    }
    a.sync = static_cast<unsigned*>(workspace);
    a.part = reinterpret_cast<float*>(static_cast<char*>(workspace) + 256);
    a.gwp = a.part + (long)n * a.nwg * 2 * 64;
    if (first_step == last_step && first_step <= n && rows_per_wg == kStepRows) {
        const StepBwdArgs q = stack_bwd_step(a.l, n, B, n_total, act, dZ0, ldz0, first_step, a.nwg, a.part);
        hipLaunchKernelGGL(stack_bwd_step_kernel, dim3(a.nwg), dim3(256), 0, static_cast<hipStream_t>(stream), q);
        return (int)hipGetLastError();
    }
    hipLaunchKernelGGL(hidden_stack_bwd_kernel, dim3(a.nwg), dim3(256), 0, static_cast<hipStream_t>(stream), a);
    return (int)hipGetLastError();
}
```

dca_amd/engine.py:

```python
import math

import numpy as np
import torch

from . import prep as _prep

BN_MOMENTUM = 0.99
BN_EPS = 1e-3
RMS_RHO = 0.9
RMS_EPS = 1e-7

AE_HEADS = {
    'zinb-conddisp': (('mean', 'disp', 'pi'), False),
    'zinb': (('mean', 'pi'), True),
    'nb-conddisp': (('mean', 'disp'), False),
    'nb': (('mean',), True),
    'poisson': (('mean',), False),
    'normal': (('mean',), False),
    'nb-shared': (('mean', 'disp'), False, ('disp',)),
    'zinb-shared': (('mean', 'disp', 'pi'), False, ('disp', 'pi')),
    'nb-fork': (('mean', 'disp'), False, ()),
    'zinb-fork': (('mean', 'disp', 'pi'), False, ()),
}
AE_FORK = ('nb-fork', 'zinb-fork')
AE_HEADS['zinb-elempi'] = (('mean', 'disp', 'pi'), False, ())
AE_ELEMPI = ('zinb-elempi',)
ACT_CODES = {'linear': 0, 'relu': 1, 'tanh': 2, 'sigmoid': 3, 'elu': 4, 'selu': 5, 'softplus': 6,
             'softsign': 7, 'LeakyReLU': 8, 'PReLU': 9,
             'hard_sigmoid': 10, 'exponential': 11, 'swish': 12, 'gelu': 13}
ACT_PRE = 12


def unsupported_activation(activation):
    if activation == 'softmax':
        return NotImplementedError("activation 'softmax' is not available on the MI355X path: it normalises over a layer's "
                                   "units (a row reduction), not element by element like the other Activation names")
    return NotImplementedError('activation %r is not available on the MI355X path (supported: %s)'
                               % (activation, ', '.join(ACT_CODES)))
INPUT_DROPOUT_LAYER = 255
AE_LOSS_FLAG = {'poisson': 4, 'normal': 8}


def _r4(x):
    return (x + 3) // 4 * 4


def _r16(x):
    return (x + 15) // 16 * 16


def _d_exp_of_histogram(cnt, numel):
    tail = torch.flip(torch.cumsum(torch.flip(cnt, [0]), 0), [0]).to(torch.float64) / float(numel)
    over = torch.nonzero(tail > 5e-5)
    c = float(over.max().item()) if over.numel() else 0.0
    need = 2.0 * c / 117.0
    return 0 if need <= 1.0 else -min(24, int(np.ceil(np.log2(need))))


class _NullSection:
    def __enter__(self):
        return self

    def __exit__(self, *a):
        return False


_NULL = _NullSection()


class EventProfiler:

    class _Sec:
        def __init__(self, prof, name):
            self.prof, self.name = prof, name

        def __enter__(self):
            self.s = torch.cuda.Event(enable_timing=True)
            self.e = torch.cuda.Event(enable_timing=True)
            self.s.record()
            return self

        def __exit__(self, *a):
            self.e.record()
            self.prof.ev.setdefault(self.name, []).append((self.s, self.e))
            return False

    def __init__(self):
# ... 139 lines not shown
        return flat[off:off + int(np.prod(shape))].view(*shape)

    def head_cols(self, head):
        if head in self.shared:
            c = len(self.planes) * self.Gp + self.shared.index(head)
            return c, c + 1
        k = self.planes.index(head)
        return k * self.Gp, k * self.Gp + self.G_out

    def plane_offset(self, head):
        if head in self.shared:
            return self.NH + self.shared.index(head) * self.Gp
        if head not in self.planes:
            return self.NH
        return self.planes.index(head) * self.Gp


class Engine:
    def __init__(self, ae_type, input_size, output_size=None, hidden_size=(64, 32, 64),
                 batchnorm=True, ridge=0.0, ops=None, comm=None, device=None, activation='relu',
                 hidden_dropout=0., input_dropout=0., dropout_seed=0, sharedpi=False, config=None):
        if ae_type not in AE_HEADS:
            raise NotImplementedError('ae_type %r is not available on the MI355X path yet '
                                      '(supported: %s)' % (ae_type, ', '.join(AE_HEADS)))
        if ops is None:
            from .ops import HipOps
            ops = HipOps()
        self.ops = ops
        self.comm = comm or SingleProcess()
        from . import config as _config
        self.cfg = config if config is not None else _config.current()
        self.dev = torch.device(device) if device is not None else (
            torch.device('cuda', torch.cuda.current_device()) if ops.device_type == 'cuda'
            else torch.device('cpu'))
        output_size = input_size if output_size is None else output_size
        self.lay = ParamLayout(ae_type, input_size, output_size, hidden_size, batchnorm, prelu=(activation == 'PReLU'))
        self.ridge = float(ridge)
        if activation not in ACT_CODES:
            raise unsupported_activation(activation)
        self.act = ACT_CODES[activation]
        self.act_pre = self.act >= ACT_PRE
        self.prelu = activation == 'PReLU'
        if self.prelu:
            self.act = 0
        lay = self.lay
        self.has_pi = 'pi' in lay.heads
        self.flags = (1 if self.has_pi else 0) | (2 if lay.const_disp else 0) | AE_LOSS_FLAG.get(ae_type, 0)
        self.center = lay.center
        f32 = dict(dtype=torch.float32, device=self.dev)
        pad = 4 * self.comm.world
        self.flat_len = (lay.total + pad - 1) // pad * pad
        self.w = torch.zeros(self.flat_len, **f32)
        self.g = torch.zeros(self.flat_len, **f32)
        self.ms = torch.zeros(self.flat_len, **f32)
        self.sharded_opt = self.comm.dp and self.cfg.dp_sharded_opt
        if self.comm.dp and self.cfg.dp_peer_exchange and batchnorm and hasattr(self.comm, 'enable_peer_exchange') \
                and self.dev.type == 'cuda' and self.lay.hidden:
            self.comm.enable_peer_exchange(2 * max(self.lay.hidden))
        self.mm = [torch.zeros(h, **f32) for h in lay.hidden] if batchnorm else []
        self.mv = [torch.ones(h, **f32) for h in lay.hidden] if batchnorm else []
        self.lr = torch.full((1,), 1e-3, **f32)
        self.cursor = torch.zeros(1, dtype=torch.int64, device=self.dev)
        self.acc = torch.zeros(2, dtype=torch.float64, device=self.dev)
        self.partials = torch.zeros(ops.max_partials, dtype=torch.float64, device=self.dev)
        self.val_loss_tmp = torch.zeros(1, **f32)
        self.clip = 5.0
        self.ldD = lay.ldA + (lay.Gp if lay.const_disp else 0)
        self.Bmax = 0
        self._hl = None
        self.X = self.Y = self.sf = self.perm = None
        self.has_targets = False
        self.csr = None
        self.out_cols = self.col_out = None
        self.perm_id = self.cursor0 = None
        self.tile_order = None
        self.hist = None
        self.prof = None
        self.use_fused = not (lay.shared or lay.fork or lay.elempi)
        self.sharedpi = bool(sharedpi) and lay.elempi
        self.ws_elempi = torch.zeros(ops.elempi_workspace_doubles(lay.G_out), dtype=torch.float64, device=self.dev) \
            if lay.elempi else None
        self.ws_heads = None
        self._pending = None
        self.W0T = None
        self.WhT = self.HT = self.XT = self.dZT = None
        self.pl = None
        self.opt_kind = 'rmsprop'
        self.slot2 = None
        self.m_sched = None
        self.opt_iter = torch.zeros(1, dtype=torch.int64, device=self.dev)
        self.reg = None
        self.reg_ws = None
        self._counts_world_key = None
        self._counts_local, self._counts_world = {}, {}
        n_conf = len(tuple(hidden_size))
        hd = list(hidden_dropout) if isinstance(hidden_dropout, (list, tuple)) else [hidden_dropout] * n_conf
        assert len(hd) == n_conf
        if lay.fork:
            hd = hd[:lay.center + 1] + [hd[-1]]
        self.drop = [float(r) for r in hd]
        self.in_drop = float(input_dropout)
        assert all(0.0 <= r < 1.0 for r in self.drop + [self.in_drop]), 'dropout rates must be in [0, 1)'
        self.has_dropout = any(r > 0.0 for r in self.drop) or self.in_drop > 0.0
        self.drop_seed = int(dropout_seed) & (2 ** 64 - 1)
        self.drop_iter = torch.zeros(1, dtype=torch.int64, device=self.dev)
        self.row0 = 0
        self.Xb = None
        self.cc = self.cc_in = None
        self.cc_csr = None
        self._tile_lut = False
        self.ws_enc0 = self.ws_enc0l = None
        self.ws_stack = None
        self.stack_mode = self.cfg.stack
        self.sparse_dw_min = self.cfg.sparse_dw_min

    def _t(self, name):
        return self.prof.section(name) if self.prof is not None else _NULL

    @property
    def _kperm(self):
        return self.perm_id if self.csr is not None else self.perm

    @property
    def _kcur(self):
        return self.cursor0 if self.csr is not None else self.cursor

    @property
    def _dhl(self):
        return self.dH[-1] if self.lay.hidden else self.dHin0

    def init_params(self, seed=0, init='glorot_uniform'):
        rng = np.random.RandomState(seed)
        lay = self.lay
        p = {}
        fan_in = lay.G_in
        for i, h in enumerate(lay.hidden):
            if lay.fork and i == len(lay.hidden) - 1:
                p['W%d' % i] = np.concatenate([keras_initializer(init, rng, fan_in, lay.hfork)
                                               for _ in range(lay.fork)], axis=1)
            else:
                p['W%d' % i] = keras_initializer(init, rng, fan_in, h)
            fan_in = h
        for hd in lay.dense_heads:
            p['W_' + hd] = keras_initializer(init, rng, lay.hL, 1 if hd in lay.shared else lay.G_out)
        if lay.elempi:
            units = 1 if self.sharedpi else lay.G_out
            k = keras_initializer(init, rng, units, units, shape=(units,))
            p['pi_k'] = np.full(lay.G_out, k[0], np.float32) if self.sharedpi else k
        self.set_params(p)

    def set_params(self, p):
        lay = self.lay
        w = self.w.cpu()
        for name, (off, shape) in lay.seg.items():
            if name in ('Wh', 'bh', 'theta_w', 'pi_k', 'pi_c'):
                continue
            if name in p:
                w[off:off + int(np.prod(shape))] = torch.as_tensor(
                    np.asarray(p[name], dtype=np.float32).reshape(-1))
        Wh = lay.view(w, 'Wh'); bh = lay.view(w, 'bh')
        for hd in lay.dense_heads:
            c0, c1 = lay.head_cols(hd)
            if 'W_' + hd in p:
                Wh[:, c0:c1] = torch.as_tensor(np.asarray(p['W_' + hd], dtype=np.float32))
            if 'b_' + hd in p:
                bh[c0:c1] = torch.as_tensor(np.asarray(p['b_' + hd], dtype=np.float32))
# ... 827 lines not shown
        if not lay.fork:
            return [(0, lay.NH, 0)]
        return [(j * lay.Gp, lay.Gp, j * lay.hfork) for j in range(lay.fork)]

    def _plane(self, buf, head):
        lay = self.lay
        if head not in lay.heads:
            return None
        return buf[:, lay.plane_offset(head):]

    def _nll(self, B, perm, cursor, Y, sf, inv_n, grad):
        lay, ops = self.lay, self.ops
        A, D = self.A, self.D
        tw = lay.view(self.w, 'theta_w') if lay.const_disp else None
        if grad and self._h2(B):
            return ops.zinb_nll_planes_h2(self._plane(A, 'mean'), self._plane(A, 'disp'), self._plane(A, 'pi'), lay.ldA, tw,
                                          Y, self.ldy, sf, perm, cursor, B, lay.G_out, self.ridge, inv_n, self.flags, self.d_exp,
                                          self.pl['D'], lay.plane_offset('mean'),
                                          0 if lay.const_disp else lay.plane_offset('disp'),
                                          lay.plane_offset('pi') if 'pi' in lay.heads else 0,
                                          self.Dth, self.ldD, self.partials)
        if grad and self._planes_nll(B):
            return ops.zinb_nll_planes(self._plane(A, 'mean'), self._plane(A, 'disp'), self._plane(A, 'pi'), lay.ldA, tw,
                                       Y, self.ldy, sf, perm, cursor, B, lay.G_out, self.ridge, inv_n, self.flags,
                                       self.pl['D'], lay.plane_offset('mean'),
                                       0 if lay.const_disp else lay.plane_offset('disp'),
                                       lay.plane_offset('pi') if 'pi' in lay.heads else 0,
                                       self.Dth, self.ldD, self.partials)
        d_disp = (self.Dth if lay.const_disp else self._plane(D, 'disp')) if grad else None
        n = ops.zinb_nll(self._plane(A, 'mean'), self._plane(A, 'disp'), self._plane(A, 'pi'),
                         lay.ldA, tw, Y, self.ldy, sf, perm, cursor, B, lay.G_out, self.ridge,
                         inv_n, self.flags, self._plane(D, 'mean') if grad else None, d_disp,
                         self._plane(D, 'pi') if grad else None, self.ldD if grad else 0,
                         self.partials)
        if grad and lay.elempi:
            gk, gc = lay.view(self.g, 'pi_k'), lay.view(self.g, 'pi_c')
            ops.elempi_bwd(self._plane(A, 'mean'), lay.ldA, self._plane(D, 'mean'), self._plane(D, 'pi'), self.ldD,
                           lay.view(self.w, 'pi_k'), B, lay.G_out, gk, gc, self.ws_elempi)
            if self.sharedpi:
                gk[:lay.G_out] = gk[:lay.G_out].sum()
                gc[:lay.G_out] = gc[:lay.G_out].sum()
        if grad:
            for hd in lay.shared:
                c0, _ = lay.head_cols(hd)
                ops.row_sums_strided(self._plane(D, hd), self.ldD, B, lay.G_out, D[:, c0:], self.ldD)
        return n

    def _not_capturing(self, what):
        if self.dev.type == 'cuda' and torch.cuda.is_current_stream_capturing():
            raise RuntimeError('host -> device copy inside a graph capture (%s): run one eager step of this shape first' % what)

    def set_world_counts(self, world_counts):
        key = tuple(world_counts)
        if self._counts_world_key != key:
            cw = self._counts_world.get(key)
            if cw is None:
                self._not_capturing('per-rank row counts not seen before')
                cw = torch.as_tensor(world_counts, dtype=torch.float32).to(self.dev)
                self._counts_world[key] = cw
            self.counts_world = cw
            self._counts_world_key = key
        self.row0 = int(sum(world_counts[:self.comm.rank]))

    def assert_finite(self, where=''):
        lay = self.lay
        bad = []
        if not bool(torch.isfinite(self.g[lay.P]).item()):
            bad.append('loss')
        if not bool(torch.isfinite(self.g[:lay.P]).all().item()) or not bool(torch.isfinite(self.w[:lay.P]).all().item()):
            for name in lay.seg:
                for flat, kind in ((self.g, 'gradient of '), (self.w, '')):
                    if not bool(torch.isfinite(lay.view(flat, name)).all().item()):
                        bad.append(kind + name)
        if bad:
            raise FloatingPointError('dca: %s has inf/nans%s' % (', '.join(bad), (' (' + where + ')') if where else ''))

    def train_step(self, B, B_global=None, world_counts=None, rows_per_slot=None):
        lay, ops, comm = self.lay, self.ops, self.comm
        Bg = B if B_global is None else B_global
        inv_n = 1.0 / (float(Bg) * lay.G_out)
        w, g = self.w, self.g
        if comm.dp:
            self.set_world_counts(world_counts)
        if B > 0:
            if self.csr is not None:
                with self._t('csr_gather'):
                    self._gather_step(B)
            self._forward_backward(B, Bg, inv_n)
        else:
            self._empty_step()
        if comm.dp and self._use_sharded_opt():
            sh = self.flat_len // comm.world
            lo = comm.rank * sh
            comm.all_reduce_sum(g[lay.P:lay.P + 1])
            gs = comm.reduce_scatter_sum(g, self._g_shard(sh))
            n_upd = max(0, min(sh, lay.P - lo))
            if n_upd > 0:
                with self._t('rmsprop_clip'):
                    ops.rmsprop_clip(w[lo:lo + sh], gs, self.ms[lo:lo + sh], n_upd, self.lr, RMS_RHO, RMS_EPS, self.clip)
            comm.all_gather_into(w, w[lo:lo + sh])
            if self.has_dropout:
                ops.counter_add(self.drop_iter, 1)
            ops.step_end(g[lay.P:], float(Bg), self.hist, rows_per_slot or max(self.Bmax, 1), self.acc, self.cursor, B)
            return
        if comm.dp:
            comm.all_reduce_sum(g[:lay.seg['Wh'][0]])
            if self._pending is not None:
                comm.wait(self._pending)
                self._pending = None
        if self.reg is not None:
            ops.l1l2_apply(self.reg, w, g, g[lay.P:], self.reg_ws)
        fused_end = self.opt_kind == 'rmsprop' and not self.has_dropout and hasattr(ops, 'rmsprop_clip_end')
        if fused_end:
            with self._t('rmsprop_clip'):
                ops.rmsprop_clip_end(w, g, self.ms, lay.P, self.lr, RMS_RHO, RMS_EPS, self.clip, g[lay.P:], float(Bg),
                                     self.hist, rows_per_slot or max(self.Bmax, 1), self.acc, self.cursor, B)
            return
        if self.opt_kind == 'rmsprop':
            with self._t('rmsprop_clip'):
                ops.rmsprop_clip(w, g, self.ms, lay.P, self.lr, RMS_RHO, RMS_EPS, self.clip)
        elif self.opt_kind == 'nadam':
            ops.nadam_step(w, g, self.ms, self.slot2, lay.P, self.lr, self.opt_iter, self.m_sched, self.clip)
            ops.counter_add(self.opt_iter, 1)
        else:
            ops.optimizer_step(self.opt_kind, w, g, None if self.opt_kind == 'sgd' else self.ms,
                               self.slot2, lay.P, self.lr, self.opt_iter, self.clip)
            ops.counter_add(self.opt_iter, 1)
        if self.has_dropout:
            ops.counter_add(self.drop_iter, 1)
        ops.step_end(g[lay.P:], float(Bg), self.hist, rows_per_slot or max(self.Bmax, 1), self.acc,
                     self.cursor, B)

    def _heads_compact(self):
        kw = {'compact': self.cc} if self.cc is not None else {}
        if getattr(self, 'heads_d_exp', 0):
            kw['d_exp'] = self.heads_d_exp
        return kw

    def _use_sharded_opt(self):
        return self.sharded_opt and self.opt_kind == 'rmsprop' and self.reg is None

    def _g_shard(self, sh):
        if getattr(self, '_gshard', None) is None or self._gshard.numel() != sh:
            self._gshard = torch.zeros(sh, dtype=torch.float32, device=self.dev)
        return self._gshard

    def _launch_heads_bucket(self):
        if self.comm.dp and not self._use_sharded_opt():
            lay = self.lay
            self._pending = self.comm.all_reduce_sum_async(self.g[lay.seg['Wh'][0]:lay.P + 1])

    def _empty_step(self):
        lay = self.lay
        self.g.zero_()
        for i, h in enumerate(lay.hidden):
            if lay.batchnorm:
                entries, cnts, E = self._batch_moments(i, 0, h, self.counts_world)
                self.ops.bn_relu_apply(self.Z[i], self.ldh[i], 0, h, entries, cnts, E,
                                       lay.view(self.w, 'beta%d' % i), self.mm[i], self.mv[i],
                                       BN_MOMENTUM, BN_EPS, self.act, self.H[i], self.ldh[i], None, 0, None)
        self._launch_heads_bucket()
        for i in reversed(range(len(lay.hidden))):
            if lay.batchnorm:
                s = torch.zeros(2 * lay.hidden[i], dtype=torch.float32, device=self.dev)
                self.comm.all_reduce_sum(s)

    def heads_fused_launch(self, B, KL, inv_n):
        lay, w, g = self.lay, self.w, self.g
        self.ops.heads_fused(self._hl[0], self._hl[1], lay.view(w, 'Wh'), lay.NH,
                             lay.view(w, 'bh'), lay.Gp,
                             lay.view(w, 'theta_w') if lay.const_disp else None, self.Y,
                             self.ldy, self.sf, self._kperm, self._kcur, B, KL, lay.G_out,
                             self.ridge, inv_n, self.flags, lay.view(g, 'Wh'), lay.NH,
                             lay.view(g, 'theta_w') if lay.const_disp else None,
                             self._dhl, self._hl[1], self.partials, self.ws_heads,
                             tile_order=self.tile_order, loss_out=g[lay.P:], **self._heads_compact())

    def _forward_backward(self, B, Bg, inv_n):
        lay, ops, comm = self.lay, self.ops, self.comm
        w, g = self.w, self.g
        KL = self._hidden_forward(B, ('perm',), True, self.counts_world)
        self._last_heads_args = (B, KL, inv_n)
        if self.ws_heads is not None:
            with self._t('heads_fused'):
                self.heads_fused_launch(B, KL, inv_n)
        else:
            self._heads_backward_unfused(B, KL, inv_n)
        self._launch_heads_bucket()
        L = len(lay.hidden)
        chain = self._stack_chain(B)
        sync = self._stack_sync(B)
        coop = chain or sync or self._stack_coop(B)
        if coop:
            layers = []
            for i, h in enumerate(lay.hidden):
                d = dict(H=h, Hact=self.H[i], ldh=self.ldh[i], xhat=self.XH[i], ldx=self.ldh[i], inv_std=self.inv_std[i],
                         dbeta=lay.view(g, 'beta%d' % i), dH=self.dH[i], lddh=self.ldh[i], **self._pre_kw(i))
                if i > 0:
                    d.update(W=lay.view(w, 'W%d' % i), ldw=h, K=lay.hidden[i - 1], Hprev=self.H[i - 1], ldp=self.ldh[i - 1],
                             gW=lay.view(g, 'W%d' % i), ldg=h)
                layers.append(d)
            if sync:
                ops.hidden_stack_bwd_sync(layers, B, float(Bg), self.act, self.dZ[0], self.ldh[0], 0, None, self.bsum[L - 1],
                                          self.ws_stack)
                comm.all_reduce_sum(self.bsum[L - 1])
                for st in range(1, L + 1):
                    i = L - st
                    ops.hidden_stack_bwd_sync(layers, B, float(Bg), self.act, self.dZ[0], self.ldh[0], st, self.bsum[i],
                                              self.bsum[i - 1] if i > 0 else None, self.ws_stack)
                    if i > 0:
                        comm.all_reduce_sum(self.bsum[i - 1])
                ops.hidden_stack_bwd(layers, B, float(Bg), self.act, self.dZ[0], self.ldh[0], self.ws_stack,
                                     rows_per_wg=32, steps=(L + 1, L + 1))
            elif chain:
                ops.hidden_stack_bwd(layers, B, float(Bg), self.act, self.dZ[0], self.ldh[0], None, rows_per_wg=64)
            elif self.stack_mode == 'coop' and B <= 256 * 64:
                ops.hidden_stack_bwd(layers, B, float(Bg), self.act, self.dZ[0], self.ldh[0], self.ws_stack, rows_per_wg=64)
            else:
                for st in range(L + 2):
                    ops.hidden_stack_bwd(layers, B, float(Bg), self.act, self.dZ[0], self.ldh[0], self.ws_stack,
                                         rows_per_wg=self._stack_rows(B), steps=(st, st))
        for i in reversed(range(L)):
            if coop and i > 0:
                continue
            h = lay.hidden[i]
            if not coop:
                if self.drop[i] > 0.0:
                    ops.dropout_apply(self.dH[i], self.ldh[i], None, None, B, h, self.drop[i], self.drop_seed,
                                      self.drop_iter, i, self.row0, self.dH[i], self.ldh[i])
                if self.prelu:
                    ops.prelu_bwd(self.dH[i], self.ldh[i], self.H[i], self.ldh[i], lay.view(w, 'alpha%d' % i), B, h,
                                  lay.view(g, 'alpha%d' % i), self.ws_prelu)
                if self._layer_small(B, i):
                    Kp = lay.hidden[i - 1]
                    ops.dense_bn_bwd_small(self.dH[i], self.ldh[i], self._slope_in(i), self.ldh[i],
                                           self.XH[i] if lay.batchnorm else None, self.ldh[i], self.inv_std[i],
                                           self.Hcur[i - 1], self.ldh[i - 1], lay.view(w, 'W%d' % i), h, B, Kp, h,
                                           lay.batchnorm, float(Bg), self.act, lay.view(g, 'W%d' % i), h,
                                           lay.view(g, 'beta%d' % i) if lay.batchnorm else None,
                                           self.dH[i - 1], self.ldh[i - 1], **self._pre_kw(i))
                    continue
                if lay.batchnorm and self._bn_small(B):
                    ops.bn_bwd_small(self.dH[i], self.ldh[i], self.H[i], self.ldh[i], self.XH[i], self.ldh[i],
                                     self.inv_std[i], float(Bg), B, h, self.dZ[i], self.ldh[i],
                                     lay.view(g, 'beta%d' % i), self.act, **self._pre_kw(i))
                elif lay.batchnorm:
                    ops.bn_bwd_sums(self.dH[i], self.ldh[i], self.H[i], self.ldh[i], self.XH[i],
                                    self.ldh[i], B, h, self.bpart[i], self.act, **self._pre_kw(i))
                    E = ops.col_moments_chunks(B)
                    sums, dbeta = self.bpart[i], lay.view(g, 'beta%d' % i)
                    if comm.dp:
                        sums, E = self._reduce_bwd_sums(i, E, h, dbeta), 1
                        dbeta = None
                    ops.bn_bwd_apply(self.dH[i], self.ldh[i], self.H[i], self.ldh[i], self.XH[i],
                                     self.ldh[i], self.inv_std[i], sums, E, float(Bg), B, h,
                                     self.dZ[i], self.ldh[i], dbeta, self.act, **self._pre_kw(i))
                else:
                    ops.relu_bwd(self.dH[i], self.ldh[i], self._slope_in(i), self.ldh[i], B, h, self.dZ[i],
                                 self.ldh[i], self.act)
            Kp = lay.G_in if i == 0 else lay.hidden[i - 1]
            gW = lay.view(g, 'W%d' % i)
            if i == 0:
                with self._t('gemm_enc0_dW'):
                    if self._sparse_dw(B):
                        if self.cc_in.lutp is None:
                            self._not_capturing('first use of the byte-store weight gradient')
                            self.cc_in.ensure_lut(ops)
                        ops.enc0_dw_sparse(self.cc_in, self._kperm, self._kcur, 0, B, Kp, h, self.dZ[0], self.ldh[0], gW, h,
                                           self.ws_enc0)
                    elif self._h2_enc0(B, True):
                        ops.absmax_exp(self.dZ[0], self.ldh[0], B, h, self.pl_exp['dZ0'])
                        ops.split_planes_h2(self.dZ[0], self.ldh[0], B, h, self.pl['dZ0'], self.pl_exp['dZ0'])
                        ops.gemm_h2(1, 0, Kp, h, B, self.pl['X'], self.pl['dZ0'], gW, h, exp_a=self.x_exp,
                                    exp_b=self.pl_exp['dZ0'], colsum_row=True, ws=self.ws)
                    elif self._planes_enc0(B, True):
                        ops.split_planes(self.dZ[0], self.ldh[0], B, h, self.pl['dZ0'])
                        ops.gemm_p3(1, 0, Kp, h, B, self.pl['X'], self.pl['dZ0'], gW, h, colsum_row=True, ws=self.ws)
                    elif self.in_drop > 0.0:
                        ops.sgemm(1, 0, Kp, h, B, self.Xb, self.ldx, self.dZ[0], self.ldh[0], gW, h,
                                  colsum_row=True, ws=self.ws)
                    elif self.XT is not None and B >= 256:
                        ops.transpose(self.X, self.ldx, B, Kp, self.XT, self.ldb_t, perm=self._kperm, cursor=self._kcur)
                        ops.transpose(self.dZ[0], self.ldh[0], B, h, self.dZT, self.ldb_t)
                        ops.sgemm(0, 1, Kp, h, B, self.XT, self.ldb_t, self.dZT, self.ldb_t, gW, h, ws=self.ws)
                        ops.row_sums_strided(self.dZT, self.ldb_t, h, B, lay.view(g, 'b0'), 1)
                    else:
                        ops.sgemm(1, 0, Kp, h, B, self.X, self.ldx, self.dZ[0], self.ldh[0], gW, h,
                                  perm=self._kperm, cursor=self._kcur, colsum_row=True, ws=self.ws)
            else:
                ops.sgemm(1, 0, Kp, h, B, self.Hcur[i - 1], self.ldh[i - 1], self.dZ[i], self.ldh[i], gW,
                          h, colsum_row=True, ws=self.ws)
                ops.sgemm(0, 1, B, Kp, h, self.dZ[i], self.ldh[i], lay.view(w, 'W%d' % i), h,
                          self.dH[i - 1], self.ldh[i - 1], ws=self.ws)

    def _heads_backward_unfused(self, B, KL, inv_n):
        lay, ops = self.lay, self.ops
        w, g = self.w, self.g
        self._heads_forward(B, KL)
        with self._t('zinb_nll'):
            n = self._nll(B, self._kperm, self._kcur, self.Y, self.sf, inv_n, True)
        ops.loss_finalize(self.partials, n, inv_n, g[lay.P:])
        gWh, Wh = lay.view(g, 'Wh'), lay.view(w, 'Wh')
# ... 422 lines not shown
```

dca_amd/hip.py:

```python
import ctypes
import os
import re

import torch

from . import build as _build

_c = ctypes

NLL_HAS_PI = 1
NLL_CONST_DISP = 2
NLL_POISSON = 4
NLL_MSE = 8

REG_MAX_SEGS = 16


class SmallLayer(_c.Structure):
    _fields_ = [('W', _c.c_void_p), ('ldw', _c.c_long), ('bias', _c.c_void_p), ('K', _c.c_int), ('H', _c.c_int),
                ('beta', _c.c_void_p), ('moving_mean', _c.c_void_p), ('moving_var', _c.c_void_p),
                ('Z', _c.c_void_p), ('ldz', _c.c_long), ('xhat', _c.c_void_p), ('ldx', _c.c_long),
                ('Hout', _c.c_void_p), ('ldh', _c.c_long), ('inv_std', _c.c_void_p)]


class StackBwdLayer(_c.Structure):
    _fields_ = [('W', _c.c_void_p), ('ldw', _c.c_long), ('K', _c.c_int), ('H', _c.c_int),
                ('Hact', _c.c_void_p), ('ldh', _c.c_long), ('xhat', _c.c_void_p), ('ldx', _c.c_long),
                ('inv_std', _c.c_void_p), ('Hprev', _c.c_void_p), ('ldp', _c.c_long),
                ('gW', _c.c_void_p), ('ldg', _c.c_long), ('dbeta', _c.c_void_p), ('dH', _c.c_void_p), ('lddh', _c.c_long),
                ('beta', _c.c_void_p)]


class RegDesc(_c.Structure):
    _fields_ = [('nseg', _c.c_int), ('start', _c.c_long * REG_MAX_SEGS), ('end', _c.c_long * REG_MAX_SEGS),
                ('l1', _c.c_float * REG_MAX_SEGS), ('l2', _c.c_float * REG_MAX_SEGS)]


ACT_CODES = {'linear': 0, 'relu': 1, 'tanh': 2, 'sigmoid': 3, 'elu': 4, 'selu': 5, 'softplus': 6,
             'softsign': 7, 'LeakyReLU': 8, 'hard_sigmoid': 10, 'exponential': 11, 'swish': 12, 'gelu': 13}
ACT_PRE = 12

OPT_KINDS = {'sgd': 0, 'rmsprop': 1, 'adagrad': 2, 'adadelta': 3, 'adam': 4, 'adamax': 5}

_SCALARS = {'int': _c.c_int, 'long': _c.c_long, 'long long': _c.c_long, 'unsigned long long': _c.c_ulonglong,
            'float': _c.c_float, 'double': _c.c_double}
_STRUCTS = {'dcahip_small_layer': SmallLayer, 'dcahip_stack_bwd_layer': StackBwdLayer, 'dcahip_reg_desc': RegDesc}
_POINTEES = set(_SCALARS) | {'void', 'unsigned', 'unsigned char'}


def _ctype(param):
    param = re.sub(r'^(.*\S)\s+(\w+)\s*\[\s*\d*\s*\]$', r'\1* \2', param)
    words = param.replace('*', ' * ').split()
    if '*' in words:
        base = ' '.join(w for w in words[:words.index('*')] if w != 'const')
        if base in _STRUCTS:
            return _c.POINTER(_STRUCTS[base])
        if base in _POINTEES:
            return _c.c_void_p
    elif ' '.join(words[:-1]) in _SCALARS:
        return _SCALARS[' '.join(words[:-1])]
    raise ValueError('dca_amd.hip: include/dcahip.h: cannot bind the parameter %r' % param)


def _parse_header(text):
    text = re.sub(r'/\*.*?\*/', ' ', text, flags=re.S)
    sigs = {}
    for res, name, params in re.findall(r'\b(int|long)\s+(dcahip_\w+)\s*\(([^()]*)\)\s*;', text):
        params = [q.strip() for q in params.split(',')]
        sigs[name] = (_SCALARS[res], [] if params in ([''], ['void']) else [_ctype(q) for q in params])
    missed = set(re.findall(r'\b(dcahip_\w+)\s*\(', text)) - set(sigs)
    if missed:
        raise ValueError('dca_amd.hip: include/dcahip.h: cannot split the declaration of %s' % ', '.join(sorted(missed)))
    return sigs


with open(os.path.join(_build.ROOT, 'include', 'dcahip.h')) as _f:
    _SIGNATURES = _parse_header(_f.read())

_lib = None


class HipExtensionMissing(RuntimeError):
    pass


def lib():
    global _lib
    if _lib is not None:
        return _lib
    path = _build.LIB
    if _build.needs_build():
        try:
            _build.build_hip(verbose=False)
        except Exception as e:
            if not os.path.exists(path):
                raise HipExtensionMissing(
                    'dca_amd: libdcahip.so is missing and could not be built (%s). The HIP '
                    'extension is mandatory; there is no CPU fallback.' % e) from e
    try:
        L = ctypes.CDLL(path)
    except OSError as e:
        raise HipExtensionMissing('dca_amd: cannot load %s: %s' % (path, e)) from e
    for name, (res, args) in _SIGNATURES.items():
        fn = getattr(L, name)
        fn.restype, fn.argtypes = res, args
    assert L.dcahip_version() == 2
    _lib = L
    return L


def exported_symbols():
    return sorted(_SIGNATURES)


def require_gpu():
    if not torch.cuda.is_available():
        raise RuntimeError('dca_amd: no AMD GPU visible (torch.cuda.is_available() is False); the '
                           'training path runs on MI355X only -- there is no CPU fallback.')


def ptr(t):
    if t is None:
        return None
    if not t.is_cuda:
        raise RuntimeError('dca_amd.hip: host tensor passed to a HIP kernel')
    return t.data_ptr()


_raw_stream = getattr(torch._C, '_cuda_getCurrentRawStream', None)
# ... 12 lines not shown
```

dca_amd/ops.py:

```python
import ctypes

import torch

from . import hip


class HipOps:
    name = 'hip'
    device_type = 'cuda'

    def __init__(self):
        hip.require_gpu()
        self.L = hip.lib()
        self.max_partials = self.L.dcahip_zinb_max_partials()

    def zinb_nll(self, a_mean, a_disp, a_pi, lda, theta_w, Y, ldy, sf, perm, cursor, B, G, ridge,
                 inv_n, flags, d_mean, d_disp, d_pi, ldd, partials):
        n = ctypes.c_int(0)
        p = hip.ptr
        hip.check(self.L.dcahip_zinb_nll(p(a_mean), p(a_disp), p(a_pi), lda, p(theta_w), p(Y), ldy,
                                         p(sf), p(perm), p(cursor), B, G, ridge, inv_n, flags,
                                         p(d_mean), p(d_disp), p(d_pi), ldd, p(partials),
                                         ctypes.byref(n), hip.stream()), 'zinb_nll')
        return n.value
# ... 37 lines not shown
        p = hip.ptr
        hip.check(self.L.dcahip_group_moments(p(a_mean), lda, p(sf), p(codes), B, G, K, flags, p(sum_acc), p(sumsq_acc),
                                              ldg, p(ws), hip.stream()), 'group_moments')

    def gram_workspace_doubles(self, B, G):
        n = int(self.L.dcahip_gram_workspace_doubles(B, G))
        hip.check(min(n, 0), 'gram_workspace_doubles')
        return n

    def gram(self, x, ldx, cols, keep, shift, B, G, cross, ldc, dsum, ws):
        p = hip.ptr
        hip.check(self.L.dcahip_gram(p(x), ldx, p(cols), p(keep), p(shift), B, G, p(cross), ldc, p(dsum), p(ws),
                                     hip.stream()), 'gram')

    def ranksum_workspace_bytes(self, g, n):
        from .groups import check_ranksum_args
        check_ranksum_args(int(g), int(n))
        nbytes = int(self.L.dcahip_ranksum_workspace_bytes(g, n))
        hip.check(min(nbytes, 0), 'ranksum_workspace_bytes')
        return nbytes

    def ranksum(self, x, ldx, g, n, order, m, gstart, K, ref, rank2, tie, ldr, ws):
        from .groups import check_ranksum_args
        g, n, m, K, ref = int(g), int(n), int(m), int(K), int(ref)
        check_ranksum_args(g, n, m, K, ref)
        if ldx < n or ldr < g:
            raise ValueError('dca_amd: ranksum: ldx = %d for %d cells, ldr = %d for %d genes' % (ldx, n, ldr, g))
        if x.dtype != torch.float32 or rank2.dtype != torch.int64 or tie.dtype != torch.int64:
            raise ValueError('dca_amd: ranksum: x is float32, rank2 and tie are int64')
        if gstart.dtype != torch.int32 or gstart.numel() < K + 1 or (m and (order.dtype != torch.int32 or order.numel() < m)):
            raise ValueError('dca_amd: ranksum: order is int32 [%d], gstart int32 [%d]' % (m, K + 1))
        need = self.ranksum_workspace_bytes(g, n)
        if ws.numel() * ws.element_size() < need:
            raise ValueError('dca_amd: ranksum: the workspace holds %d bytes, %d are needed'
                             % (ws.numel() * ws.element_size(), need))
        p = hip.ptr
        hip.check(self.L.dcahip_ranksum(p(x), ldx, g, n, p(order) if m else None, m, p(gstart), K, ref, p(rank2), p(tie), ldr,
                                        p(ws), hip.stream()), 'ranksum')

    def loss_finalize(self, partials, n, scale, loss_out):
        hip.check(self.L.dcahip_loss_finalize(hip.ptr(partials), n, scale, hip.ptr(loss_out),
                                              hip.stream()), 'loss_finalize')

    def step_end(self, loss, weight, hist, rows_per_slot, acc, cursor, advance):
        p = hip.ptr
        hip.check(self.L.dcahip_step_end(p(loss), weight, p(hist), rows_per_slot, p(acc), p(cursor),
                                         advance, hip.stream()), 'step_end')

    def heads_infer(self, a_mean, a_disp, a_pi, lda, sf, B, G, mean_sf, theta, pi, ldo, flags=0):
        p = hip.ptr
        hip.check(self.L.dcahip_zinb_heads_infer(p(a_mean), p(a_disp), p(a_pi), lda, p(sf), B, G,
                                                 p(mean_sf), p(theta), p(pi), ldo, flags, hip.stream()),
                  'heads_infer')

    def heads_fused_workspace_bytes(self, B, hL, G, plane, flags):
        return self.L.dcahip_heads_fused_workspace_bytes(B, hL, G, plane, flags)

    def x3_product_32x32(self, A, B, C, K):
        hip.check(self.L.dcahip_x3_product_32x32(hip.ptr(A), hip.ptr(B), hip.ptr(C), K, hip.stream()), "x3_product_32x32")

    def has(self, entry):
        return hasattr(self.L, entry)

    def heads_tile_order_len(self, G):
        return int(self.L.dcahip_heads_tile_order_len(G))

    def heads_fused(self, H, ldh, Wh, ldw, bh, plane, theta_w, Y, ldy, sf, perm, cursor, B, hL, G,
                    ridge, inv_n, flags, gW, ldg, g_theta, dH, lddh, partials, ws, tile_order=None, loss_out=None,
                    compact=None, d_exp=0):
        n = ctypes.c_int(0)
        p = hip.ptr
        c = compact
        hip.check(self.L.dcahip_heads_fused(p(H), ldh, p(Wh), ldw, p(bh), plane, p(theta_w), p(Y), ldy,
                                            p(c.Yc) if c is not None else None, c.ldc if c is not None else 0,
                                            p(c.ovf_ptr) if c is not None else None,
                                            p(c.ovf_col) if c is not None else None,
                                            p(c.ovf_val) if c is not None else None,
                                            p(sf), p(perm), p(cursor), B, hL, G, ridge, inv_n, flags,
                                            p(gW), ldg, p(g_theta), p(dH), lddh, p(partials),
                                            ctypes.byref(n), p(ws), ws.numel() * ws.element_size(),
                                            p(tile_order), p(loss_out), int(d_exp), hip.stream()), 'heads_fused')
        return n.value

    def counts_compact_ld(self, G):
        return int(self.L.dcahip_counts_compact_ld(G))

    def counts_compact(self, Y, ldy, n, G, Yc, ldc, status):
        hip.check(self.L.dcahip_counts_compact(hip.ptr(Y), ldy, n, G, hip.ptr(Yc), ldc, hip.ptr(status), hip.stream()),
                  'counts_compact')

    def enc0_lut_entries(self):
        return int(self.L.dcahip_enc0_lut_entries())

    def enc0_lut(self, fac, do_log, n, lutp):
        hip.check(self.L.dcahip_enc0_lut(hip.ptr(fac), int(do_log), n, hip.ptr(lutp), hip.stream()), 'enc0_lut')

    def enc0_sparse_supported(self, H1):
        return bool(self.L.dcahip_enc0_sparse_supported(int(H1)))

    def enc0_dw_sparse_workspace_bytes(self, B, G, H1):
        return int(self.L.dcahip_enc0_dw_sparse_workspace_bytes(B, G, H1))

    def enc0_dw_sparse(self, c, perm, cursor, row_base, B, G, H1, dZ, ldz, gW, ldg, ws, form=0):
        p = hip.ptr
        c.ensure_lut(self)
        hip.check(self.L.dcahip_enc0_dw_sparse(p(c.Yc), c.ldc, p(c.ovf_ptr), p(c.ovf_col), p(c.ovf_val), p(c.fac),
                                               int(c.do_log), p(c.lutp), p(c.mean), p(c.std), p(perm), p(cursor), int(row_base),
                                               B, G, H1, p(dZ), ldz, p(gW), ldg, p(ws), ws.numel() * ws.element_size(),
                                               int(form), hip.stream()), 'enc0_dw_sparse')

    def enc0_fwd_lut_workspace_bytes(self, B, G, H1):
        return int(self.L.dcahip_enc0_fwd_lut_workspace_bytes(B, G, H1))

    def enc0_fwd_lut(self, c, perm, cursor, row_base, B, G, H1, W, ldw, bias, Z, ldz, ws):
        p = hip.ptr
        c.ensure_lut(self)
        hip.check(self.L.dcahip_enc0_fwd_lut(p(c.Yc), c.ldc, p(c.ovf_ptr), p(c.ovf_col), p(c.ovf_val), p(c.fac),
                                             int(c.do_log), p(c.lutp), p(c.mean), p(c.std), p(perm), p(cursor), int(row_base),
                                             B, G, H1, p(W), ldw, p(bias), p(Z), ldz, p(ws),
                                             ws.numel() * ws.element_size(), hip.stream()), 'enc0_fwd_lut')

    def sgemm_workspace_bytes(self, ta, tb, M, N, K, colsum_row=False, split_k=0):
        return self.L.dcahip_sgemm_workspace_bytes(int(ta), int(tb), M, N, K, int(colsum_row), split_k)

    def sgemm(self, ta, tb, M, N, K, A, lda, B, ldb, C, ldc, bias=None, perm=None, cursor=None,
              colsum_row=False, split_k=0, ws=None):
        p = hip.ptr
        wsb = ws.numel() * ws.element_size() if ws is not None else 0
        hip.check(self.L.dcahip_sgemm(int(ta), int(tb), M, N, K, p(A), lda, p(B), ldb, p(C), ldc,
                                      p(bias), p(perm), p(cursor), int(colsum_row), split_k, p(ws),
                                      wsb, hip.stream()), 'sgemm')

    def sgemm_plan(self, ta, tb, M, N, K, A, lda, B, ldb, colsum_row=False, split_k=0):
        out = (ctypes.c_int * 8)()
        hip.check(self.L.dcahip_sgemm_plan(int(ta), int(tb), M, N, K, int(colsum_row), split_k, hip.ptr(A), lda,
                                           hip.ptr(B), ldb, ctypes.addressof(out)), 'sgemm_plan')
        return tuple(out)

    @staticmethod
    def sgemm_reduce_lanes(split, outputs):
        if split <= 1:
            return 0
        return 16 if split >= 16 and outputs <= 65536 else 1

    def planes_alloc(self, rows, cols, device):
        return torch.zeros(3, rows, (cols + 7) // 8 * 8, dtype=torch.bfloat16, device=device)

    def split_planes(self, src, ld, R, C, planes, perm=None, cursor=None):
        hip.check(self.L.dcahip_split_planes(hip.ptr(src), ld, hip.ptr(perm), hip.ptr(cursor), R, C, hip.ptr(planes),
                                             planes.shape[2], planes.stride(0), hip.stream()), 'split_planes')

    def gemm_p3_workspace_bytes(self, M, N, K, colsum_row=False, split_k=0):
        return self.L.dcahip_gemm_p3_workspace_bytes(M, N, K, int(colsum_row), split_k)

    def gemm_p3(self, ta, tb, M, N, K, A, B, C, ldc, bias=None, perm=None, cursor=None, colsum_row=False, split_k=0,
                ws=None):
        p = hip.ptr
        wsb = ws.numel() * ws.element_size() if ws is not None else 0
        hip.check(self.L.dcahip_gemm_p3(int(ta), int(tb), M, N, K, p(A), A.stride(1), A.stride(0), p(B), B.stride(1),
                                        B.stride(0), p(C), ldc, p(bias), p(perm), p(cursor), int(colsum_row), split_k,
                                        p(ws), wsb, hip.stream()), 'gemm_p3')

    def absmax_exp(self, src, ld, R, C, exp):
        hip.check(self.L.dcahip_absmax_exp(hip.ptr(src), ld, R, C, hip.ptr(exp), hip.ptr(exp[1:]), hip.stream()), 'absmax_exp')

    def split_planes_h2(self, src, ld, R, C, planes, exp=None, perm=None, cursor=None):
# ... 19 lines not shown
                                               hip.ptr(dst), ld_dst, hip.stream()), 'transpose')

    def col_moments_chunks(self, B):
        return self.L.dcahip_col_moments_chunks(B)

    def col_moments(self, Z, ldz, B, H, part):
        hip.check(self.L.dcahip_col_moments(hip.ptr(Z), ldz, B, H, hip.ptr(part), hip.stream()),
                  'col_moments')

    def moments_combine(self, entries, counts, E, H, out):
        hip.check(self.L.dcahip_moments_combine(hip.ptr(entries), hip.ptr(counts), E, H, hip.ptr(out),
                                                hip.stream()), 'moments_combine')

    def bn_relu_apply(self, Z, ldz, B, H, entries, counts, E, beta, mm, mv, momentum, eps, relu,
                      Hout, ldh, xhat, ldx, inv_std):
        p = hip.ptr
        hip.check(self.L.dcahip_bn_relu_apply(p(Z), ldz, B, H, p(entries), p(counts), E, p(beta),
                                              p(mm), p(mv), momentum, eps, int(relu), p(Hout), ldh,
                                              p(xhat), ldx, p(inv_std), hip.stream()), 'bn_relu_apply')

    def bn_bwd_sums(self, dH, ldd, Hact, ldh, xhat, ldx, B, H, part, act=1, beta=None):
        p = hip.ptr
        hip.check(self.L.dcahip_bn_bwd_sums(p(dH), ldd, p(Hact), ldh, p(xhat), ldx, B, H, p(part),
                                            act, p(beta), hip.stream()), 'bn_bwd_sums')

    def bn_bwd_apply(self, dH, ldd, Hact, ldh, xhat, ldx, inv_std, sums, E, n_total, B, H, dZ, ldz,
                     dbeta, act=1, beta=None):
        p = hip.ptr
        hip.check(self.L.dcahip_bn_bwd_apply(p(dH), ldd, p(Hact), ldh, p(xhat), ldx, p(inv_std),
                                             p(sums), E, float(n_total), B, H, p(dZ), ldz, p(dbeta),
                                             act, p(beta), hip.stream()), 'bn_bwd_apply')

    @property
    def bn_fused_max_rows(self):
        return int(self.L.dcahip_bn_fused_max_rows())

    def bn_relu_train_small(self, Z, ldz, B, H, beta, mm, mv, momentum, eps, act, Hout, ldh, xhat, ldx, inv_std):
        p = hip.ptr
        hip.check(self.L.dcahip_bn_relu_train_small(p(Z), ldz, B, H, p(beta), p(mm), p(mv), momentum, eps, int(act),
                                                    p(Hout), ldh, p(xhat), ldx, p(inv_std), hip.stream()),
                  'bn_relu_train_small')

    def bn_bwd_small(self, dH, ldd, Hact, ldh, xhat, ldx, inv_std, n_total, B, H, dZ, ldz, dbeta, act=1, beta=None):
        p = hip.ptr
        hip.check(self.L.dcahip_bn_bwd_small(p(dH), ldd, p(Hact), ldh, p(xhat), ldx, p(inv_std), float(n_total), B, H,
                                             p(dZ), ldz, p(dbeta), act, p(beta), hip.stream()), 'bn_bwd_small')

    @property
    def dense_small_max_k(self):
        return int(self.L.dcahip_dense_small_max_k())

    def dense_bn_small(self, Hp, ldp, W, ldw, bias, B, K, H, batchnorm, beta, mm, mv, momentum, eps, act, Z, ldz,
                       xhat, ldx, Hout, ldh, inv_std):
        p = hip.ptr
        hip.check(self.L.dcahip_dense_bn_small(p(Hp), ldp, p(W), ldw, p(bias), B, K, H, int(batchnorm), p(beta), p(mm), p(mv),
                                               momentum, eps, int(act), p(Z), ldz, p(xhat), ldx, p(Hout), ldh, p(inv_std),
                                               hip.stream()), 'dense_bn_small')

    def hidden_small_chain(self, layers, Hin, ldin, B, batchnorm, momentum, eps, act):
        arr = self._small_layers(layers)
        hip.check(self.L.dcahip_hidden_small_chain(arr, len(layers), hip.ptr(Hin), ldin, B, int(batchnorm), momentum, eps,
                                                   int(act), hip.stream()), 'hidden_small_chain')

    @property
    def hidden_stack_max_rows(self):
        return int(self.L.dcahip_hidden_stack_max_rows())

    def hidden_stack_workspace_bytes(self, n_layers, B):
        return int(self.L.dcahip_hidden_stack_workspace_bytes(n_layers, B))

    def hidden_stack_fwd(self, layers, B, momentum, eps, act, ws, rows_per_wg=64, steps=None):
        arr = self._small_layers(layers)
        first, last = steps if steps is not None else (0, len(layers))
        hip.check(self.L.dcahip_hidden_stack_fwd(arr, len(layers), B, momentum, eps, int(act), int(rows_per_wg), first, last,
                                                 hip.ptr(ws), ws.numel() * ws.element_size(), hip.stream()), 'hidden_stack_fwd')

    def hidden_stack_bwd(self, layers, B, n_total, act, dZ0, ldz0, ws, rows_per_wg=64, steps=None):
        arr = self._bwd_layers(layers)
        first, last = steps if steps is not None else (0, len(layers) + 1)
        hip.check(self.L.dcahip_hidden_stack_bwd(arr, len(layers), B, float(n_total), int(act), hip.ptr(dZ0), ldz0,
                                                 int(rows_per_wg), first, last, hip.ptr(ws),
                                                 0 if ws is None else ws.numel() * ws.element_size(),
                                                 hip.stream()), 'hidden_stack_bwd')

    def _small_layers(self, layers):
        arr = (hip.SmallLayer * len(layers))()
        for q, d in zip(arr, layers):
            for k in ('W', 'bias', 'beta', 'moving_mean', 'moving_var', 'Z', 'xhat', 'Hout', 'inv_std'):
                setattr(q, k, hip.ptr(d.get(k)))
            for k in ('ldw', 'K', 'H', 'ldz', 'ldx', 'ldh'):
                setattr(q, k, int(d.get(k, 0)))
        return arr

    def _bwd_layers(self, layers):
        arr = (hip.StackBwdLayer * len(layers))()
        for q, d in zip(arr, layers):
            for k in ('W', 'Hact', 'xhat', 'inv_std', 'Hprev', 'gW', 'dbeta', 'dH', 'beta'):
                setattr(q, k, hip.ptr(d.get(k)))
            for k in ('ldw', 'K', 'H', 'ldh', 'ldx', 'ldp', 'ldg', 'lddh'):
                setattr(q, k, int(d.get(k, 0)))
        return arr

    def hidden_stack_fwd_sync(self, layers, B, momentum, eps, act, step, ext_entries, ext_counts, ext_E, stat_out, ws):
        arr = self._small_layers(layers)
        hip.check(self.L.dcahip_hidden_stack_fwd_sync(arr, len(layers), B, momentum, eps, int(act), int(step),
                                                      hip.ptr(ext_entries), hip.ptr(ext_counts), int(ext_E), hip.ptr(stat_out),
                                                      hip.ptr(ws), ws.numel() * ws.element_size(), hip.stream()),
                  'hidden_stack_fwd_sync')

    def hidden_stack_bwd_sync(self, layers, B, n_total, act, dZ0, ldz0, step, ext_sums, sums_out, ws):
        arr = self._bwd_layers(layers)
        hip.check(self.L.dcahip_hidden_stack_bwd_sync(arr, len(layers), B, float(n_total), int(act), hip.ptr(dZ0), ldz0,
                                                      int(step), hip.ptr(ext_sums), hip.ptr(sums_out), hip.ptr(ws),
                                                      ws.numel() * ws.element_size(), hip.stream()), 'hidden_stack_bwd_sync')

    def dense_bn_bwd_small(self, dH, ldd, Hact, ldh, xhat, ldx, inv_std, Hp, ldp, W, ldw, B, K, H, batchnorm, n_total, act,
                           gW, ldg, dbeta, dHp, lddp, beta=None):
        p = hip.ptr
        hip.check(self.L.dcahip_dense_bn_bwd_small(p(dH), ldd, p(Hact), ldh, p(xhat), ldx, p(inv_std), p(Hp), ldp, p(W), ldw,
                                                   B, K, H, int(batchnorm), float(n_total), int(act), p(gW), ldg, p(dbeta),
                                                   p(dHp), lddp, p(beta), hip.stream()), 'dense_bn_bwd_small')

    def relu_bwd(self, dH, ldd, Hact, ldh, B, H, dZ, ldz, act=1):
        p = hip.ptr
        hip.check(self.L.dcahip_relu_bwd(p(dH), ldd, p(Hact), ldh, B, H, p(dZ), ldz, act, hip.stream()),
                  'relu_bwd')

    def relu_fwd(self, Z, ldz, B, H, Hout, ldh, act=1):
        hip.check(self.L.dcahip_relu_fwd(hip.ptr(Z), ldz, B, H, hip.ptr(Hout), ldh, act, hip.stream()),
                  'relu_fwd')

    def colsum_chain(self, x, ldx, B, N, theta_w, out):
        p = hip.ptr
        hip.check(self.L.dcahip_colsum_chain(p(x), ldx, B, N, p(theta_w), p(out), hip.stream()),
                  'colsum_chain')

    def optimizer_step(self, kind, w, g, slot1, slot2, n, lr, it, clip):
        p = hip.ptr
        hip.check(self.L.dcahip_optimizer_step(hip.OPT_KINDS[kind], p(w), p(g), p(slot1), p(slot2), n, p(lr),
                                               p(it), clip, hip.stream()), 'optimizer_step')

    def prelu_workspace_doubles(self, h):
        return int(self.L.dcahip_prelu_workspace_doubles(h))

    def prelu_fwd(self, x, ldx, alpha, B, h, out, ldo):
        p = hip.ptr
        hip.check(self.L.dcahip_prelu_fwd(p(x), ldx, p(alpha), B, h, p(out), ldo, hip.stream()), 'prelu_fwd')

    def prelu_bwd(self, d, ldd, x, ldx, alpha, B, h, galpha, ws):
        p = hip.ptr
        hip.check(self.L.dcahip_prelu_bwd(p(d), ldd, p(x), ldx, p(alpha), B, h, p(galpha), p(ws), hip.stream()),
                  'prelu_bwd')

    def elempi_workspace_doubles(self, G):
        return int(self.L.dcahip_elempi_workspace_doubles(G))

    def elempi_fwd(self, a_mean, lda, k, c, B, G, a_pi, ldp):
        p = hip.ptr
        hip.check(self.L.dcahip_elempi_fwd(p(a_mean), lda, p(k), p(c), B, G, p(a_pi), ldp, hip.stream()), 'elempi_fwd')

    def elempi_bwd(self, m, lda, d_mean, d_pi, ldd, k, B, G, gk, gc, ws):
        p = hip.ptr
        hip.check(self.L.dcahip_elempi_bwd(p(m), lda, p(d_mean), p(d_pi), ldd, p(k), B, G, p(gk), p(gc), p(ws),
                                           hip.stream()), 'elempi_bwd')

    def bcast_cols(self, s, lds, B, G, out, ldo):
# ... 272 lines not shown
                 cluster_mean=torch.full((k,), nan, dtype=torch.float64, device=dev),
                 mean=torch.full((1,), nan, dtype=torch.float64, device=dev))
        status = torch.zeros(1, dtype=torch.int32, device=dev)
        hip.check(self.L.dcahip_silhouette(p(X) if n else None, ldx, n, d, p(labels) if n else None, k, splits, p(r['s']), p(r['a']),
                                           p(r['b']), p(r['nearest']), p(r['counts']), p(r['cluster_mean']), p(r['mean']),
                                           p(ws), p(status), hip.stream()), 'silhouette')
        self.silhouette_raise(status, r['counts'])
        return r

    def graph_symmetrize_workspace_bytes(self, n, k):
        from .community import check_graph_args
        check_graph_args(int(n), int(k))
        nbytes = int(self.L.dcahip_graph_symmetrize_workspace_bytes(n, k))
        hip.check(min(nbytes, 0), 'graph_symmetrize_workspace_bytes')
        return nbytes

    def graph_symmetrize(self, idx):
        from .community import check_graph_args
        p = hip.ptr
        if idx.dtype != torch.int32 or idx.dim() != 2 or (idx.shape[1] > 1 and idx.stride(1) != 1):
            raise ValueError('dca_amd: louvain: the neighbour indices are a 2-d int32 tensor with unit column stride')
        n, k = idx.shape
        check_graph_args(n, k)
        dev = idx.device
        rowptr = torch.zeros(n + 1, dtype=torch.int64, device=dev)
        deg = torch.zeros(n, dtype=torch.int32, device=dev)
        cap = 2 * n * k
        col = torch.empty(max(cap, 1), dtype=torch.int32, device=dev)
        if n == 0:
            return rowptr, col[:0], deg
        ws = torch.empty(max(self.graph_symmetrize_workspace_bytes(n, k), 16), dtype=torch.uint8, device=dev)
        status = torch.zeros(1, dtype=torch.int32, device=dev)
        hip.check(self.L.dcahip_graph_symmetrize(p(idx), idx.stride(0) if n > 1 else k, n, k, p(rowptr), p(col), cap, p(deg),
                                                 p(ws), p(status), hip.stream()), 'graph_symmetrize')
        bad = int(status.item())
        if bad:
            raise ValueError('dca_amd: louvain: %d neighbour indices lie outside 0 .. %d (and are not the padding -1)' % (bad, n - 1))
        return rowptr, col[:int(rowptr[n].item())], deg

    def louvain_level(self, rowptr, col, wt, twom, g, max_sweeps, labels=None, best_q=None):
        return LouvainLevel(self, rowptr, col, wt, twom, g, max_sweeps, labels, best_q)

    def csr_gather(self, csr, perm, cursor, row0, B, sf, fac, do_log, mean, std, Y, ldy, X, ldx, sf_out, status):
        p = hip.ptr
        hip.check(self.L.dcahip_csr_gather(p(csr.indptr), p(csr.indices), p(csr.values), csr.nnz, csr.n, csr.G, p(perm),
                                           p(cursor), int(row0), B, p(sf), p(fac), int(bool(do_log)), p(mean), p(std),
                                           p(Y), ldy, p(X), ldx if X is not None else 0, p(sf_out), p(status),
                                           hip.stream()), 'csr_gather')

    def csr_gather_cols(self, csr, col_out, G_out, perm, cursor, row0, B, sf, fac, do_log, mean, std, Y, ldy, X, ldx, sf_out,
                        status):
        p = hip.ptr
        assert col_out.dtype == torch.int32 and col_out.numel() >= csr.G
        hip.check(self.L.dcahip_csr_gather_cols(p(csr.indptr), p(csr.indices), p(csr.values), csr.nnz, csr.n, csr.G, p(perm),
                                                p(cursor), int(row0), B, p(sf), p(fac), int(bool(do_log)), p(mean), p(std),
                                                p(Y), ldy, p(X), ldx if X is not None else 0, p(sf_out), p(status),
                                                p(col_out), int(G_out), hip.stream()), 'csr_gather_cols')

    def csr_gather_compact(self, csr, perm, cursor, row0, B, sf, fac, do_log, mean, std, Yc, ldc, ovf_ptr, ovf_col, ovf_val,
                           X, ldx, sf_out, fac_out, status):
        p = hip.ptr
        cap = int(ovf_col.numel()) if ovf_col is not None else 0
        hip.check(self.L.dcahip_csr_gather_compact(p(csr.indptr), p(csr.indices), p(csr.values), csr.nnz, csr.n, csr.G,
                                                   p(perm), p(cursor), int(row0), B, p(sf), p(fac), int(bool(do_log)), p(mean),
                                                   p(std), p(Yc), ldc, p(ovf_ptr), p(ovf_col), p(ovf_val), cap, p(X),
                                                   ldx if X is not None else 0, p(sf_out), p(fac_out), p(status),
                                                   hip.stream()), 'csr_gather_compact')

    def csr_col_pass(self, csr, fac, do_log, col_part, status):
        p = hip.ptr
        hip.check(self.L.dcahip_csr_col_pass(p(csr.indptr), p(csr.indices), p(csr.values), csr.nnz, csr.n, csr.G, p(fac),
                                             int(bool(do_log)), p(col_part), p(status), hip.stream()), 'csr_col_pass')

    def csr_row_sums(self, csr, out, status):
        p = hip.ptr
        hip.check(self.L.dcahip_csr_row_sums(p(csr.indptr), p(csr.indices), p(csr.values), csr.nnz, csr.n, csr.G, p(out),
                                             p(status), hip.stream()), 'csr_row_sums')

    def rmsprop_clip_end(self, w, g, ms, n, lr, rho, eps, clip, loss, weight, hist, rows_per_slot, acc, cursor, advance):
        p = hip.ptr
        hip.check(self.L.dcahip_rmsprop_clip(p(w), p(g), p(ms), n, p(lr), rho, eps, clip, p(loss), weight, p(hist),
                                             rows_per_slot, p(acc), p(cursor), advance, hip.stream()), 'rmsprop_clip')

    def rmsprop_clip(self, w, g, ms, n, lr, rho, eps, clip):
        self.rmsprop_clip_end(w, g, ms, n, lr, rho, eps, clip, None, 0.0, None, 0, None, None, 0)


class LouvainLevel:

    def __init__(self, ops, rowptr, col, wt, twom, g, max_sweeps, labels=None, best_q=None):
        from .community import check_level_args
        n = rowptr.numel() - 1
        nnz = col.numel()
        twom, g, max_sweeps = int(twom), int(g), int(max_sweeps)
        check_level_args(n, nnz, twom, g, max_sweeps)
        if rowptr.dtype != torch.int64 or col.dtype != torch.int32 or not rowptr.is_contiguous() or not col.is_contiguous() or \
                (wt is not None and (wt.dtype != torch.int32 or wt.numel() != nnz or not wt.is_contiguous())):
            raise ValueError('dca_amd: louvain: the graph is rowptr int64 [n + 1], col int32 [nnz], wt int32 [nnz] or None')
        dev = rowptr.device
        p = hip.ptr
        self.n, self.g, self.twom = n, g, twom
        self.ki = torch.zeros(n, dtype=torch.int32, device=dev)
        self.labels = torch.zeros(n, dtype=torch.int32, device=dev)
        self.tot = torch.zeros(n, dtype=torch.int32, device=dev)
        self.labels_new = torch.zeros(n, dtype=torch.int32, device=dev)
        self.tot_new = torch.zeros(n, dtype=torch.int32, device=dev)
        self.state = torch.zeros(24, dtype=torch.int64, device=dev)
        self._keep = (rowptr, col, wt)
        graph = (n, nnz, p(rowptr), p(col) if nnz else None, p(wt) if wt is not None and nnz else None)
        L = ops.L
        hip.check(L.dcahip_louvain_begin(*graph, p(self.ki) if n else None, p(self.labels) if n else None,
                                         p(self.tot) if n else None, twom, g, p(self.state), hip.stream()), 'louvain_begin')
        if labels is not None:
            if labels.dtype != torch.int32 or tuple(labels.shape) != (n,):
                raise ValueError('dca_amd: louvain: labels is an int32 tensor of shape (%d,)' % n)
            if n and (int(labels.min()) < 0 or int(labels.max()) >= n):
                raise ValueError('dca_amd: louvain: labels lie in 0 .. %d' % (n - 1))
            self.labels.copy_(labels)
            self.tot.zero_().index_add_(0, labels.long(), self.ki)
            q = int(best_q)
            if not -(1 << 127) <= q < 1 << 127:
                raise ValueError('dca_amd: louvain: best_q is a 128-bit integer')
            self.state[2] = self.state[10] = (q & ((1 << 64) - 1)) - ((1 << 64) if q & (1 << 63) else 0)
            self.state[3] = self.state[11] = q >> 64
        tail = (p(self.ki), p(self.labels), p(self.tot), p(self.labels_new), p(self.tot_new)) if n else (None,) * 5
        fn, st = L.dcahip_louvain_sweep, p(self.state)

        def sweep(s):
            hip.check(fn(*graph, *tail, twom, g, int(s), max_sweeps, st, hip.stream()), 'louvain_sweep')
        self.sweep = sweep

    def read(self, s):
        w = [int(v) for v in self.state.cpu().tolist()]
        st = w[8 * ((s + 1) & 1):][:8]
        sm = w[16 + 4 * (s & 1):][:4]
        u = lambda v: v & ((1 << 64) - 1)
        return dict(done=st[0], sweeps=st[1], q=(st[3] << 64) | u(st[2]), idle=st[4], kept=bool(st[5]), moved=u(sm[0]),
                    inside=u(sm[1]), tot2=u(sm[2]))
```

include/dcahip.h:

```cpp
#ifndef DCAHIP_H
#define DCAHIP_H

#ifdef __cplusplus
extern "C" {
#endif

#define DCAHIP_VERSION 2
#define DCAHIP_EINVAL (-22)

#define DCAHIP_NLL_HAS_PI      1
#define DCAHIP_NLL_CONST_DISP  2
#define DCAHIP_NLL_POISSON     4
#define DCAHIP_NLL_MSE         8

int dcahip_version(void);

int dcahip_zinb_max_partials(void);

int dcahip_zinb_nll(const float* a_mean, const float* a_disp, const float* a_pi, long lda,
                    const float* theta_w,
                    const float* y, long ldy, const float* sf,
                    const int* perm, const long long* cursor,
                    int B, int G, float ridge, float inv_n, int flags,
                    float* d_mean, float* d_disp, float* d_pi, long ldd,
                    double* loss_partials, int* n_partials_out, void* stream);

int dcahip_zinb_nll_planes(const float* a_mean, const float* a_disp, const float* a_pi, long lda,
                           const float* theta_w, const float* y, long ldy, const float* sf,
                           const int* perm, const long long* cursor, int B, int G, float ridge,
                           float inv_n, int flags, void* d_planes, long ldp, long plane_stride,
                           long col_mean, long col_disp, long col_pi, float* d_theta, long ldd_theta,
                           double* loss_partials, int* n_partials_out, void* stream);

int dcahip_zinb_nll_planes_h2(const float* a_mean, const float* a_disp, const float* a_pi, long lda,
                              const float* theta_w, const float* y, long ldy, const float* sf,
                              const int* perm, const long long* cursor, int B, int G, float ridge,
                              float inv_n, int flags, int d_exp, void* d_planes, long ldp, long plane_stride,
                              long col_mean, long col_disp, long col_pi, float* d_theta, long ldd_theta,
                              double* loss_partials, int* n_partials_out, void* stream);

int dcahip_nll_marginals_workspace_doubles(int B, int G);
int dcahip_nll_marginals(const float* a_mean, const float* a_disp, const float* a_pi, long lda,
                         const float* theta_w, const float* y, long ldy, const float* sf,
                         int B, int G, float ridge, int flags,
                         double* cell_out, double* gene_acc, double* workspace, void* stream);

#define DCAHIP_GROUP_NO_SF   16
#define DCAHIP_GROUP_LOG1P   32
int dcahip_group_moments_workspace_doubles(int B, int G, int K);
int dcahip_group_moments(const float* a_mean, long lda, const float* sf, const int* codes,
                         int B, int G, int K, int flags,
                         double* sum_acc, double* sumsq_acc, long ldg,
                         double* workspace, void* stream);

long dcahip_ranksum_workspace_bytes(int g, int n);
int dcahip_ranksum(const float* x, long ldx, int g, int n,
                   const int* order, int m, const int* gstart, int K, int ref,
                   long long* rank2, long long* tie, long ldr,
                   void* workspace, void* stream);

long dcahip_gram_workspace_doubles(int B, int G);
int dcahip_gram(const float* x, long ldx, const int* cols, const int* keep, const double* shift,
                int B, int G, double* cross, long ldc, double* dsum, double* ws, void* stream);

int dcahip_loss_finalize(const double* partials, int n_partials, double scale,
                         float* loss_out, void* stream);

int dcahip_step_end(const float* loss, double weight, float* hist, int rows_per_slot,
                    double* acc, long long* cursor, int advance, void* stream);

int dcahip_zinb_heads_infer(const float* a_mean, const float* a_disp, const float* a_pi,
                            long lda, const float* sf, int B, int G,
                            float* mean_sf, float* theta, float* pi, long ldo, int flags,
                            void* stream);

long dcahip_heads_fused_workspace_bytes(int B, int hL, int G, long plane, int flags);
int dcahip_heads_tile_order_len(int G);
int dcahip_heads_fused(const float* H, long ldh, const float* Wh, long ldw, const float* bh,
                       long plane, const float* theta_w,
                       const float* y, long ldy,
                       const unsigned char* yc, long ldc, const int* ovf_ptr, const int* ovf_col,
                       const float* ovf_val, const float* sf,
                       const int* perm, const long long* cursor,
                       int B, int hL, int G, float ridge, float inv_n, int flags,
                       float* gW, long ldg, float* g_theta, float* dH, long lddh,
                       double* loss_partials, int* n_partials_out,
                       void* workspace, long workspace_bytes, const int* tile_order,
                       float* loss_out, int d_exp, void* stream);
int dcahip_x3_product_32x32(const float* A, const float* B, float* C, int K, void* stream);

int dcahip_sgemm(int ta, int tb, int M, int N, int K,
                 const float* A, long lda, const float* B, long ldb, float* C, long ldc,
                 const float* bias, const int* perm, const long long* cursor,
                 int colsum_row, int split_k, void* workspace, long workspace_bytes,
                 void* stream);
long dcahip_sgemm_workspace_bytes(int ta, int tb, int M, int N, int K, int colsum_row, int split_k);
int dcahip_sgemm_plan(int ta, int tb, int M, int N, int K, int colsum_row, int split_k,
                      const float* A, long lda, const float* B, long ldb, int out[8]);
int dcahip_split_planes(const float* src, long ld, const int* perm, const long long* cursor, long R, int C,
                        void* planes, long ldp, long plane_stride, void* stream);
int dcahip_gemm_p3(int ta, int tb, int M, int N, int K, const void* A, long lda, long plane_a,
                   const void* B, long ldb, long plane_b, float* C, long ldc, const float* bias,
                   const int* perm, const long long* cursor, int colsum_row, int split_k,
                   void* workspace, long workspace_bytes, void* stream);
long dcahip_gemm_p3_workspace_bytes(int M, int N, int K, int colsum_row, int split_k);
int dcahip_absmax_exp(const float* src, long ld, long R, int C, int* exp_out, void* scratch_word, void* stream);
int dcahip_split_planes_h2(const float* src, long ld, const int* perm, const long long* cursor, long R, int C,
                           void* planes, long ldp, long plane_stride, const int* exp, void* stream);
int dcahip_gemm_h2_supported(int M, int N, int K);
long dcahip_gemm_h2_workspace_bytes(int M, int N, int K, int colsum_row, int split_k);
int dcahip_gemm_h2(int ta, int tb, int M, int N, int K, const void* A, long lda, long plane_a, const int* exp_a, int exp_a_add,
                   const void* B, long ldb, long plane_b, const int* exp_b, int exp_b_add, float alpha,
                   float* C, long ldc, const float* bias, int colsum_row, int split_k,
                   void* workspace, long workspace_bytes, void* stream);
int dcahip_transpose(const float* src, long ld_src, int R, int C, float* dst, long ld_dst, void* stream);
int dcahip_transpose_rows(const float* src, long ld_src, const int* perm, const long long* cursor, int R, int C,
                          float* dst, long ld_dst, void* stream);

int dcahip_col_moments_chunks(int B);
int dcahip_col_moments(const float* Z, long ldz, int B, int H, float* part, void* stream);
int dcahip_moments_combine(const float* entries, const float* counts, int E, int H,
                           float* out , void* stream);
int dcahip_bn_relu_apply(const float* Z, long ldz, int B, int H,
                         const float* entries, const float* counts, int E,
                         const float* beta, float* moving_mean, float* moving_var,
                         float momentum, float eps, int relu,
                         float* Hout, long ldh, float* xhat, long ldx, float* inv_std,
                         void* stream);

int dcahip_bn_fused_max_rows(void);
int dcahip_dense_small_max_k(void);
int dcahip_dense_bn_small(const float* Hp, long ldp, const float* W, long ldw, const float* bias,
                          int B, int K, int H, int batchnorm, const float* beta,
                          float* moving_mean, float* moving_var, float momentum, float eps, int act,
                          float* Z, long ldz, float* xhat, long ldx, float* Hout, long ldh,
                          float* inv_std, void* stream);
int dcahip_dense_bn_bwd_small(const float* dH, long ldd, const float* Hact, long ldh,
                              const float* xhat, long ldx, const float* inv_std,
                              const float* Hp, long ldp, const float* W, long ldw,
                              int B, int K, int H, int batchnorm, float n_total, int act,
                              float* gW, long ldg, float* dbeta, float* dHp, long lddp, const float* beta,
                              void* stream);
typedef struct dcahip_small_layer {
    const float* W; long ldw;
    const float* bias;
    int K, H;
    const float* beta; float* moving_mean; float* moving_var;
    float* Z; long ldz;
    float* xhat; long ldx; float* Hout; long ldh; float* inv_std;
} dcahip_small_layer;
int dcahip_hidden_small_chain(const dcahip_small_layer* layers, int n, const float* Hin, long ldin, int B,
                              int batchnorm, float momentum, float eps, int act, void* stream);
typedef struct dcahip_stack_bwd_layer {
    const float* W; long ldw; int K, H;
    const float* Hact; long ldh;
    const float* xhat; long ldx; const float* inv_std;
    const float* Hprev; long ldp;
    float* gW; long ldg; float* dbeta;
    float* dH; long lddh;
    const float* beta;
} dcahip_stack_bwd_layer;
int dcahip_hidden_stack_max_rows(void);
long dcahip_hidden_stack_workspace_bytes(int n_layers, int B);
int dcahip_hidden_stack_fwd(const dcahip_small_layer* layers, int n, int B, float momentum, float eps, int act,
                            int rows_per_wg, int first_step, int last_step,
                            void* workspace, long workspace_bytes, void* stream);
int dcahip_hidden_stack_bwd(const dcahip_stack_bwd_layer* layers, int n, int B, float n_total, int act,
                            float* dZ0, long ldz0, int rows_per_wg, int first_step, int last_step,
                            void* workspace, long workspace_bytes, void* stream);

int dcahip_hidden_stack_step_blocks(int B);
int dcahip_hidden_stack_fwd_sync(const dcahip_small_layer* layers, int n, int B, float momentum, float eps, int act,
                                 int step, const float* ext_entries, const float* ext_counts, int ext_E,
                                 float* stat_out, void* workspace, long workspace_bytes, void* stream);
int dcahip_hidden_stack_bwd_sync(const dcahip_stack_bwd_layer* layers, int n, int B, float n_total, int act,
                                 float* dZ0, long ldz0, int step, const float* ext_sums, float* sums_out,
                                 void* workspace, long workspace_bytes, void* stream);
int dcahip_bn_relu_train_small(const float* Z, long ldz, int B, int H, const float* beta,
                               float* moving_mean, float* moving_var, float momentum, float eps,
                               int act, float* Hout, long ldh, float* xhat, long ldx,
                               float* inv_std, void* stream);
int dcahip_bn_bwd_small(const float* dH, long ldd, const float* Hact, long ldh,
                        const float* xhat, long ldx, const float* inv_std, float n_total,
                        int B, int H, float* dZ, long ldz, float* dbeta, int act, const float* beta, void* stream);

int dcahip_bn_bwd_sums(const float* dH, long ldd, const float* Hact, long ldh,
                       const float* xhat, long ldx, int B, int H, float* part, int act, const float* beta,
                       void* stream);
int dcahip_bn_bwd_apply(const float* dH, long ldd, const float* Hact, long ldh,
                        const float* xhat, long ldx, const float* inv_std,
                        const float* sums, int E, float n_total, int B, int H,
                        float* dZ, long ldz, float* dbeta, int act, const float* beta, void* stream);
int dcahip_relu_bwd(const float* dH, long ldd, const float* Hact, long ldh, int B, int H,
                    float* dZ, long ldz, int act, void* stream);
int dcahip_relu_fwd(const float* Z, long ldz, int B, int H, float* Hout, long ldh, int act, void* stream);
int dcahip_prelu_workspace_doubles(int h);
int dcahip_prelu_fwd(const float* x, long ldx, const float* alpha, int B, int h, float* out, long ldo, void* stream);
int dcahip_prelu_bwd(float* d, long ldd, const float* x, long ldx, const float* alpha, int B, int h,
                     float* galpha, double* workspace, void* stream);
int dcahip_elempi_workspace_doubles(int G);
int dcahip_elempi_fwd(float* a_mean, long lda, const float* k, const float* c, int B, int G,
                      float* a_pi, long ldp, void* stream);
int dcahip_elempi_bwd(const float* m, long lda, float* d_mean, const float* d_pi, long ldd, const float* k,
                      int B, int G, float* gk, float* gc, double* workspace, void* stream);
int dcahip_bcast_cols(const float* s, long lds, int B, int G, float* out, long ldo, void* stream);
int dcahip_row_sums_strided(const float* x, long ldx, int B, int G, float* out, long ldo, void* stream);

int dcahip_colsum_chain(const float* x, long ldx, int B, int N, const float* theta_w,
                        float* out, void* stream);

int dcahip_prep_chunks(int n);
int dcahip_prep_row_sums(const float* Y, long ldy, int n, int G, float* out, void* stream);
int dcahip_prep_col_pass(const float* Y, long ldy, int n, int G, const float* fac, int do_log,
                         float* X, long ldx, double* col_part, void* stream);
int dcahip_prep_col_finish(const double* col_part, int R, int G, double n_total,
                           float* sums, float* mean, float* stdv, void* stream);
int dcahip_prep_scale(float* X, long ldx, int n, int G, const float* mean, const float* stdv,
                      void* stream);
int dcahip_csr_expand(const int* indptr, const int* indices, const float* values, long nnz, int rows, int G,
                      float* Y, long ldy, int* status, void* stream);

int dcahip_csr_compress(const float* X, long ld, int rows, int G, long base, long* indptr, int* indices, float* values,
                        long cap, int* status, void* stream);
int dcahip_csr_subset(const long* indptr, const int* indices, const float* values, long nnz, int n, int G,
                      const unsigned char* row_keep, const unsigned char* col_keep, int n_out, long* out_indptr,
                      int* out_indices, float* out_values, long cap, int* ws, int* status, void* stream);

int dcahip_csr_gather(const long* indptr, const int* indices, const float* values, long nnz, int n, int G,
                      const int* perm, const long long* cursor, long row0, int B, const float* sf,
                      const float* fac, int do_log, const float* mean, const float* stdv, float* Y, long ldy,
                      float* X, long ldx, float* sf_out, int* status, void* stream);
int dcahip_csr_gather_cols(const long* indptr, const int* indices, const float* values, long nnz, int n, int G,
                           const int* perm, const long long* cursor, long row0, int B, const float* sf,
                           const float* fac, int do_log, const float* mean, const float* stdv, float* Y, long ldy,
                           float* X, long ldx, float* sf_out, int* status, const int* col_out, int G_out, void* stream);
int dcahip_csr_gather_compact(const long* indptr, const int* indices, const float* values, long nnz, int n, int G,
                              const int* perm, const long long* cursor, long row0, int B, const float* sf,
                              const float* fac, int do_log, const float* mean, const float* stdv,
                              unsigned char* Yc, long ldc, int* ovf_ptr, int* ovf_col, float* ovf_val, int ovf_cap,
                              float* X, long ldx, float* sf_out, float* fac_out, int* status, void* stream);
int dcahip_csr_col_pass(const long* indptr, const int* indices, const float* values, long nnz, int n, int G,
                        const float* fac, int do_log, double* col_part, int* status, void* stream);
int dcahip_csr_row_sums(const long* indptr, const int* indices, const float* values, long nnz, int n, int G,
                        float* out, int* status, void* stream);

long dcahip_csr_thin_workspace_bytes(int n, long nnz);
int dcahip_csr_thin(const long* indptr, const int* indices, const float* values, long nnz, int n, int G,
                    const long* row_ids, unsigned long long threshold, unsigned long long seed,
                    long* indptr_a, int* indices_a, float* values_a,
                    long* indptr_b, int* indices_b, float* values_b, long cap,
                    void* workspace, int* status, void* stream);

int dcahip_rmsprop_clip(float* w, const float* g, float* ms, long n, const float* lr,
                        float rho, float eps, float clip, const float* loss, double weight,
                        float* hist, int rows_per_slot, double* acc, long long* cursor, int advance,
                        void* stream);

#define DCAHIP_OPT_SGD       0
#define DCAHIP_OPT_RMSPROP   1
#define DCAHIP_OPT_ADAGRAD   2
#define DCAHIP_OPT_ADADELTA  3
#define DCAHIP_OPT_ADAM      4
#define DCAHIP_OPT_ADAMAX    5
int dcahip_optimizer_step(int kind, float* w, const float* g, float* slot1, float* slot2, long n,
                          const float* lr, const long long* iter, float clip, void* stream);
int dcahip_counter_add(long long* counter, int v, void* stream);
int dcahip_nadam_step(float* w, const float* g, float* m, float* v, long n, const float* lr,
                      const long long* iter, float* m_schedule, float clip, void* stream);
#define DCAHIP_REG_MAX_SEGS 16
typedef struct {
    int nseg;
    long start[DCAHIP_REG_MAX_SEGS];
    long end[DCAHIP_REG_MAX_SEGS];
    float l1[DCAHIP_REG_MAX_SEGS];
    float l2[DCAHIP_REG_MAX_SEGS];
} dcahip_reg_desc;
int dcahip_l1l2_workspace_doubles(void);
int dcahip_l1l2_apply(const dcahip_reg_desc* d, const float* w, float* g, float* loss_inout,
                      double* workspace, void* stream);

int dcahip_dropout_apply(const float* x, long ldx, const int* perm, const long long* cursor, int B, int h,
                         float rate, unsigned long long seed, const long long* step, int layer, long row0,
                         float* out, long ldo, void* stream);

long dcahip_counts_compact_ld(int G);
int dcahip_counts_compact(const float* Y, long ldy, int n, int G, unsigned char* Yc, long ldc, int* status,
                          void* stream);
int dcahip_enc0_sparse_supported(int H1);
int dcahip_enc0_lut(const float* fac, int do_log, int n, void* lutp, void* stream);
int dcahip_enc0_lut_entries(void);
long dcahip_enc0_dw_sparse_workspace_bytes(int B, int G, int H1);
int dcahip_enc0_dw_sparse(const unsigned char* Yc, long ldc, const int* ovf_ptr, const int* ovf_col,
                          const float* ovf_val, const float* fac, int do_log, const void* lutp, const float* mean,
                          const float* stdv, const int* perm, const long long* cursor, long row_base,
                          int B, int G, int H1, const float* dZ, long ldz, float* gW, long ldg,
                          void* workspace, long workspace_bytes, int form, void* stream);
long dcahip_enc0_fwd_lut_workspace_bytes(int B, int G, int H1);
int dcahip_enc0_fwd_lut(const unsigned char* Yc, long ldc, const int* ovf_ptr, const int* ovf_col,
                        const float* ovf_val, const float* fac, int do_log, const void* lutp, const float* mean,
                        const float* stdv, const int* perm, const long long* cursor, long row_base,
                        int B, int G, int H1, const float* W, long ldw, const float* bias,
                        float* Z, long ldz, void* workspace, long workspace_bytes, void* stream);

int dcahip_knn_splits(int nq, int n, int d, int k);
long dcahip_knn_workspace_bytes(int nq, int n, int d, int k, int splits);
int dcahip_knn(const float* Q, long ldq, int nq, const float* X, long ldx, int n, int d, int k,
               long self_offset, int splits, int* idx_out, float* d2_out, long ldo,
               void* ws, int* status, void* stream);

long dcahip_kmeans_workspace_bytes(int n, int d, int k);
int dcahip_kmeans_step(const float* X, long ldx, int n, int d, int k, const float* C_in, long ldc, float* C_out, long ldco,
                       int* labels, float* d2_out, int* counts, double* sums, long lds, double* inertia,
                       int* changed, int* reseeded, int* state, int iter, void* ws, int* status, void* stream);
int dcahip_kmeans_seed(const float* X, long ldx, int n, int d, int k, unsigned long long seed, int init,
                       int* rows_out, float* C_out, long ldc, void* ws, int* status, void* stream);

int dcahip_silhouette_splits(int n, int d, int k);
long dcahip_silhouette_workspace_bytes(int n, int d, int k, int splits);
int dcahip_silhouette(const float* X, long ldx, int n, int d, const int* labels, int k, int splits,
                      double* s_out, double* a_out, double* b_out, int* nearest_out,
                      int* counts, double* cluster_mean, double* mean,
                      void* ws, int* status, void* stream);

long dcahip_graph_symmetrize_workspace_bytes(int n, int k);
int dcahip_graph_symmetrize(const int* idx, long ldi, int n, int k, long* rowptr, int* col, long cap, int* deg,
                            void* ws, int* status, void* stream);
int dcahip_louvain_begin(int n, long nnz, const long* rowptr, const int* col, const int* wt, int* ki, int* labels, int* tot,
                         long twom, int g, long* state, void* stream);
int dcahip_louvain_sweep(int n, long nnz, const long* rowptr, const int* col, const int* wt, const int* ki, int* labels,
                         int* tot, int* labels_new, int* tot_new, long twom, int g, int sweep, int max_sweeps, long* state,
                         void* stream);

long dcahip_peer_slot_bytes(int world, int nmax);
long dcahip_peer_flag_bytes(int world);
int dcahip_peer_exchange(const float* local, int n, float* const* slots, unsigned* const* flags, int rank, int world, int nmax,
                         unsigned long long* epoch, float* out, int reduce, int* status, long timeout_us, void* stream);

#ifdef __cplusplus
}
// ... 3 lines not shown
```

Before: 4.496 million.

## Fold heads weight-gradient reduce and RMSprop update into hidden-stack backward kernel

Defers the output-heads weight-gradient reduction, or the direct optimizer update when gradients are written directly, so that it runs as extra blocks of the hidden-stack backward step kernel instead of separate launches. The global RMSprop kernel gains a hole parameter so it skips the heads parameter range that the rider already updated. The aim is to remove separate reduce and update passes and overlap that bandwidth-bound work with the latency-bound stack backward. It adds coupling between heads, stack and optimizer ordering, plus more block scheduling inside the step kernel.

Result: no change. 4.508 million, median of 6 (+0.3%).

```diff
diff --git a/dca_amd/build.py b/dca_amd/build.py
--- a/dca_amd/build.py
+++ b/dca_amd/build.py
@@ -10,7 +10,7 @@
 SOURCES = ['dcahip_zinb.hip', 'dcahip_gemm.hip', 'dcahip_layers.hip', 'dcahip_heads.hip', 'dcahip_prep.hip', 'dcahip_opt.hip',
            'dcahip_dropout.hip', 'dcahip_sparse.hip', 'dcahip_peer.hip', 'dcahip_knn.hip', 'dcahip_kmeans.hip', 'dcahip_gram.hip',
            'dcahip_silhouette.hip', 'dcahip_ranksum.hip', 'dcahip_louvain.hip']
-HEADERS = ['zinb_math.hpp', 'h2_math.hpp', 'philox.hpp', 'knn_dist.hpp']
+HEADERS = ['zinb_math.hpp', 'h2_math.hpp', 'philox.hpp', 'knn_dist.hpp', 'step_rider.hpp']
 ARCH = 'gfx950'
 HOST_LIB = os.path.join(CSRC, 'libdcahost.so')
 HOST_SOURCES = ['dcahost_tsv.cpp', 'dcahost_read.cpp']
diff --git a/dca_amd/config.py b/dca_amd/config.py
--- a/dca_amd/config.py
+++ b/dca_amd/config.py
@@ -20,6 +20,7 @@
     fused_write: bool = True
     resident: str = 'auto'
     counts_compact: bool = False
+    ride_heads_update: bool = True
     graph_steps: int = 8
     sparse_dw_min: int = 512
     lut_fwd_min: int = 1024
@@ -29,7 +30,7 @@
     _ENV = {'stack': 'DCA_AMD_STACK', 'bwd_chain': 'DCA_AMD_BWD_CHAIN', 'wide_planes': 'DCA_AMD_WIDE_PLANES', 'wide_h2': 'DCA_AMD_WIDE_H2',
             'dp_sharded_opt': 'DCA_AMD_DP_SHARDED_OPT', 'dp_graph': 'DCA_AMD_DP_GRAPH', 'device_prep': 'DCA_AMD_DEVICE_PREP',
             'fused_write': 'DCA_AMD_FUSED_WRITE', 'dp_peer_exchange': 'DCA_AMD_DP_PEER', 'resident': 'DCA_AMD_RESIDENT',
-            'counts_compact': 'DCA_AMD_COUNTS_COMPACT'}
+            'counts_compact': 'DCA_AMD_COUNTS_COMPACT', 'ride_heads_update': 'DCA_AMD_RIDE_HEADS_UPDATE'}
 
     @classmethod
     def from_env(cls):
diff --git a/dca_amd/csrc/dcahip_heads.hip b/dca_amd/csrc/dcahip_heads.hip
--- a/dca_amd/csrc/dcahip_heads.hip
+++ b/dca_amd/csrc/dcahip_heads.hip
@@ -3,6 +3,7 @@
 #include <type_traits>
 #include "dcahip.h"
 #include "zinb_math.hpp"
+#include "step_rider.hpp"
 
 namespace {
 
@@ -820,67 +821,9 @@
 }
 
 
-struct ReduceDwArgs {
-    const float* ws; int S; long stride; int hL; long ldws, ncols; float* gW; long ldg;
-    const float* theta_w; float* g_theta; int G;
-    float scale;
-    const float* ws2; int S2; const int* tail_tiles; int ntail; long plane;
-    int tail_first;
-};
-
-__device__ __forceinline__ void reduce_dw_body(const ReduceDwArgs& q, int bid, int nblk) {
-    const int hL = q.hL;
-    const long ldws = q.ldws, ncols = q.ncols; float* gW = q.gW; const long ldg = q.ldg;
-    const float* theta_w = q.theta_w; float* g_theta = q.g_theta; const int G = q.G;
-    const float sc = q.scale;
-    __shared__ unsigned tailbm[kMaxGrid / 32];
-    if (q.ntail > 0) {
-        for (int i = threadIdx.x; i < kMaxGrid / 32; i += 256) tailbm[i] = 0u;
-        __syncthreads();
-        for (int i = threadIdx.x; i < q.ntail; i += 256) {
-            const int tl = q.tail_tiles ? q.tail_tiles[i] : q.tail_first + i;
-            if (tl >= 0 && tl < kMaxGrid) atomicOr(&tailbm[tl >> 5], 1u << (tl & 31));
-        }
-        __syncthreads();
-    }
-    auto is_tail = [&](long col_in_plane) { const int tl = (int)(col_in_plane / kTG); return q.ntail > 0 && ((tailbm[tl >> 5] >> (tl & 31)) & 1u); };
-    if ((ncols & 3) == 0 && (ldws & 3) == 0 && (ldg & 3) == 0 && (q.stride & 3) == 0 && (q.plane & 3) == 0 &&
-        ((reinterpret_cast<uintptr_t>(q.ws) | reinterpret_cast<uintptr_t>(gW) | reinterpret_cast<uintptr_t>(q.ws2)) & 15) == 0) {
-        const long nq = ncols >> 2, totalq = (long)(hL + 1) * nq;
-        for (long idx = (long)bid * 256 + threadIdx.x; idx < totalq; idx += (long)nblk * 256) {
-            const long i = idx / nq, c = (idx - i * nq) << 2;
-            const bool tl = is_tail(c % q.plane);
-            const float* ws = tl ? q.ws2 : q.ws; const int S = tl ? q.S2 : q.S; const long stride = q.stride;
-            float4 v = *reinterpret_cast<const float4*>(ws + i * ldws + c);
-            for (int s = 1; s < S; ++s) {
-                const float4 x = *reinterpret_cast<const float4*>(ws + (long)s * stride + i * ldws + c);
-                v.x += x.x; v.y += x.y; v.z += x.z; v.w += x.w;
-            }
-            v.x *= sc; v.y *= sc; v.z *= sc; v.w *= sc;
-            *reinterpret_cast<float4*>(gW + i * ldg + c) = v;
-        }
-    } else {
-        const long total = (long)(hL + 1) * ncols;
-        for (long idx = (long)bid * 256 + threadIdx.x; idx < total; idx += (long)nblk * 256) {
-            const long i = idx / ncols, c = idx - i * ncols;
-            const bool tl = is_tail(c % q.plane);
-            const float* ws = tl ? q.ws2 : q.ws; const int S = tl ? q.S2 : q.S;
-            float v = 0.f;
-            for (int s = 0; s < S; ++s) v += ws[(long)s * q.stride + i * ldws + c];
-            gW[i * ldg + c] = v * sc;
-        }
-    }
-    if (g_theta) {
-        for (long c = (long)bid * 256 + threadIdx.x; c < G; c += (long)nblk * 256) {
-            const bool tl = is_tail(c);
-            const float* ws = tl ? q.ws2 : q.ws; const int S = tl ? q.S2 : q.S; const long stride = q.stride;
-            float v = 0.f;
-            for (int s = 0; s < S; ++s) v += ws[(long)s * stride + (long)(hL + 1) * ldws + c];
-            const float e = expf(theta_w[c]);
-            g_theta[c] = (e >= 1e-3f && e <= 1e4f) ? v * sc * e : 0.f;
-        }
-    }
-}
+using step_rider::ReduceDwArgs;
+using step_rider::reduce_dw_body;
+static_assert(step_rider::kTileGenes == kTG && step_rider::kMaxTiles == kMaxGrid, "the tail bitmap of the weight-gradient reduce");
 
 __global__ __launch_bounds__(256) void heads_reduce_dw_kernel(ReduceDwArgs q) { reduce_dw_body(q, blockIdx.x, gridDim.x); }
 
@@ -1510,16 +1453,17 @@
 
 extern "C" int dcahip_heads_tile_order_len(int G) { return G > 0 ? (((G + kTG - 1) / kTG + kWG - 1) / kWG) * kWG : 0; }
 
-extern "C" int dcahip_heads_fused(const float* H, long ldh, const float* Wh, long ldw,
-                                  const float* bh, long plane, const float* theta_w,
-                                  const float* y, long ldy,
-                                  const unsigned char* yc, long ldc, const int* ovf_ptr, const int* ovf_col,
-                                  const float* ovf_val, const float* sf, const int* perm,
-                                  const long long* cursor, int B, int hL, int G, float ridge,
-                                  float inv_n, int flags, float* gW, long ldg, float* g_theta,
-                                  float* dH, long lddh, double* loss_partials, int* n_partials_out,
-                                  void* workspace, long workspace_bytes, const int* tile_order,
-                                  float* loss_out, int d_exp, void* stream) {
+static int heads_fused_run(const float* H, long ldh, const float* Wh, long ldw,
+                           const float* bh, long plane, const float* theta_w,
+                           const float* y, long ldy,
+                           const unsigned char* yc, long ldc, const int* ovf_ptr, const int* ovf_col,
+                           const float* ovf_val, const float* sf, const int* perm,
+                           const long long* cursor, int B, int hL, int G, float ridge,
+                           float inv_n, int flags, float* gW, long ldg, float* g_theta,
+                           float* dH, long lddh, double* loss_partials, int* n_partials_out,
+                           void* workspace, long workspace_bytes, const int* tile_order,
+                           float* loss_out, int d_exp, dcahip_step_rider* pending, void* stream) {
+    if (pending) pending->kind = DCAHIP_RIDER_NONE;
     const bool has_pi = flags & DCAHIP_NLL_HAS_PI, cdisp = flags & DCAHIP_NLL_CONST_DISP;
     HeadsPlan pl;
     if (!make_heads_plan(B, hL, G, plane, flags, &pl)) return DCAHIP_EINVAL;
@@ -1593,7 +1537,17 @@
                               ws_dw2, pl.S2, (pl.ntail > 0 && tile_order) ? tile_order + pl.nmain : nullptr, pl.ntail, plane, pl.nmain};
         const int gl = (nq <= 1024 && pl.npart >= 256) ? 64 : (nq >= 64L * 512 ? 4 : 16);
         const int n_dh = (int)((nq + 256 / gl - 1) / (256 / gl));
-        if (!direct_dw) {
+        const bool ridable = pending && ldg == pl.ldws && al16(gW) && (direct_dw || step_rider::reduce_dw_vec(qw));
+        if (ridable) {
+            dcahip_step_rider& d = *pending;
+            d.kind = direct_dw ? DCAHIP_RIDER_UPDATE : DCAHIP_RIDER_REDUCE;
+            d.ws = direct_dw ? nullptr : qw.ws; d.ws2 = direct_dw ? nullptr : qw.ws2; d.tail_tiles = direct_dw ? nullptr : qw.tail_tiles;
+            d.stride = qw.stride; d.ldws = qw.ldws; d.plane = qw.plane; d.chunks = (long)(hL + 1) * (pl.ldws >> 2);
+            d.S = direct_dw ? 1 : qw.S; d.S2 = direct_dw ? 0 : qw.S2; d.ntail = direct_dw ? 0 : qw.ntail; d.tail_first = qw.tail_first;
+            d.hL = hL; d.G = G; d.scale = qw.scale;
+            d.gW = gW; d.theta_w = direct_dw ? nullptr : qw.theta_w; d.g_theta = direct_dw ? nullptr : qw.g_theta;
+        }
+        if (!direct_dw && !ridable) {
             const dim3 grid(n_dh + (int)gr);
             if (gl == 64) hipLaunchKernelGGL(heads_reduce_both_kernel<64>, grid, dim3(256), 0, s, qh, qw, n_dh);
             else if (gl == 4) hipLaunchKernelGGL(heads_reduce_both_kernel<4>, grid, dim3(256), 0, s, qh, qw, n_dh);
@@ -1607,3 +1561,34 @@
     }
     return rc;
 }
+
+extern "C" int dcahip_heads_fused(const float* H, long ldh, const float* Wh, long ldw,
+                                  const float* bh, long plane, const float* theta_w,
+                                  const float* y, long ldy,
+                                  const unsigned char* yc, long ldc, const int* ovf_ptr, const int* ovf_col,
+                                  const float* ovf_val, const float* sf, const int* perm,
+                                  const long long* cursor, int B, int hL, int G, float ridge,
+                                  float inv_n, int flags, float* gW, long ldg, float* g_theta,
+                                  float* dH, long lddh, double* loss_partials, int* n_partials_out,
+                                  void* workspace, long workspace_bytes, const int* tile_order,
+                                  float* loss_out, int d_exp, void* stream) {
+    return heads_fused_run(H, ldh, Wh, ldw, bh, plane, theta_w, y, ldy, yc, ldc, ovf_ptr, ovf_col, ovf_val, sf, perm, cursor, B, hL, G,
+                           ridge, inv_n, flags, gW, ldg, g_theta, dH, lddh, loss_partials, n_partials_out, workspace,
+                           workspace_bytes, tile_order, loss_out, d_exp, nullptr, stream);
+}
+
+extern "C" int dcahip_heads_fused_deferred(const float* H, long ldh, const float* Wh, long ldw,
+                                           const float* bh, long plane, const float* theta_w,
+                                           const float* y, long ldy,
+                                           const unsigned char* yc, long ldc, const int* ovf_ptr, const int* ovf_col,
+                                           const float* ovf_val, const float* sf, const int* perm,
+                                           const long long* cursor, int B, int hL, int G, float ridge,
+                                           float inv_n, int flags, float* gW, long ldg, float* g_theta,
+                                           float* dH, long lddh, double* loss_partials, int* n_partials_out,
+                                           void* workspace, long workspace_bytes, const int* tile_order,
+                                           float* loss_out, int d_exp, dcahip_step_rider* pending, void* stream) {
+    if (!pending) return DCAHIP_EINVAL;
+    return heads_fused_run(H, ldh, Wh, ldw, bh, plane, theta_w, y, ldy, yc, ldc, ovf_ptr, ovf_col, ovf_val, sf, perm, cursor, B, hL, G,
+                           ridge, inv_n, flags, gW, ldg, g_theta, dH, lddh, loss_partials, n_partials_out, workspace,
+                           workspace_bytes, tile_order, loss_out, d_exp, pending, stream);
+}
diff --git a/dca_amd/csrc/dcahip_layers.hip b/dca_amd/csrc/dcahip_layers.hip
--- a/dca_amd/csrc/dcahip_layers.hip
+++ b/dca_amd/csrc/dcahip_layers.hip
@@ -1,6 +1,7 @@
 #include <hip/hip_runtime.h>
 #include <stdint.h>
 #include "dcahip.h"
+#include "step_rider.hpp"
 
 namespace {
 
@@ -904,7 +905,7 @@
 
 __global__ __launch_bounds__(256) void rmsprop_clip_kernel(float* w, const float* g, float* ms,
                                                            long n, const float* lrp, float rho,
-                                                           float eps, float clip, StepEnd se) {
+                                                           float eps, float clip, StepEnd se, long hole0, long hole) {
     if (se.on && blockIdx.x == 0 && threadIdx.x == 0) {
         const long long c = se.cursor ? *se.cursor : 0;
         if (se.loss) {
@@ -917,27 +918,20 @@
     const float lr = *lrp;
     const long nv = n >> 2;
     const long stride = (long)gridDim.x * 256;
-    for (long i = (long)blockIdx.x * 256 + threadIdx.x; i < nv; i += stride) {
+    for (long k = (long)blockIdx.x * 256 + threadIdx.x; k < nv - hole; k += stride) {
+        const long i = k < hole0 ? k : k + hole;
         float4 gv = reinterpret_cast<const float4*>(g)[i];
         float4 mv = reinterpret_cast<const float4*>(ms)[i];
         float4 wv = reinterpret_cast<const float4*>(w)[i];
-        float* gp = &gv.x; float* mp = &mv.x; float* wp = &wv.x;
-#pragma unroll
-        for (int j = 0; j < 4; ++j) {
-            float gj = gp[j];
-            if (clip > 0.f) gj = fminf(fmaxf(gj, -clip), clip);
-            mp[j] = rho * mp[j] + (1.f - rho) * gj * gj;
-            wp[j] = wp[j] - lr * gj / (sqrtf(mp[j]) + eps);
-        }
+        step_rider::rmsprop_clip_quad(wv, mv, gv, lr, rho, eps, clip);
         reinterpret_cast<float4*>(ms)[i] = mv;
         reinterpret_cast<float4*>(w)[i] = wv;
     }
     for (long i = (nv << 2) + (long)blockIdx.x * 256 + threadIdx.x; i < n; i += stride) {
-        float gj = g[i];
-        if (clip > 0.f) gj = fminf(fmaxf(gj, -clip), clip);
-        const float m = rho * ms[i] + (1.f - rho) * gj * gj;
+        float m = ms[i], x = w[i];
+        step_rider::rmsprop_clip_one(x, m, g[i], lr, rho, eps, clip);
         ms[i] = m;
-        w[i] = w[i] - lr * gj / (sqrtf(m) + eps);
+        w[i] = x;
     }
 }
 
@@ -1435,6 +1429,8 @@
 }
 
 constexpr int kStepRows = 32;
+constexpr int kRiderMaxBlocks = 1024;
+constexpr int kRiderChunks = 4;
 
 struct StepFwdArgs {
     SmallLayer cur, nxt;
@@ -1571,9 +1567,14 @@
     float* part_out;
     float* gwp;
     const float* ext_in;
+    step_rider::StepRider rider;
 };
 
 __global__ __launch_bounds__(256) void stack_bwd_step_kernel(StepBwdArgs a) {
+    if ((int)blockIdx.x >= a.nwg) {
+        step_rider::step_rider_body(a.rider, (int)blockIdx.x - a.nwg);
+        return;
+    }
     __shared__ __attribute__((aligned(16))) float dyt[kStepRows * kStackLd];
     __shared__ __attribute__((aligned(16))) float ht[kStepRows * kStackLd];
     __shared__ __attribute__((aligned(16))) float wl[64 * kStackLd];
@@ -2177,7 +2178,25 @@
     if (grid < 1) grid = 1;
     hipLaunchKernelGGL(rmsprop_clip_kernel, dim3((int)grid), dim3(256), 0,
                        static_cast<hipStream_t>(stream), w, g, ms, n, lr, rho, eps, clip,
-                       StepEnd{loss, weight, hist, rows_per_slot, acc, cursor, advance, (loss || hist || acc || cursor) ? 1 : 0});
+                       StepEnd{loss, weight, hist, rows_per_slot, acc, cursor, advance, (loss || hist || acc || cursor) ? 1 : 0},
+                       0L, 0L);
+    return (int)hipGetLastError();
+}
+
+extern "C" int dcahip_rmsprop_clip_hole(float* w, const float* g, float* ms, long n, long hole_first, long hole_len,
+                                        const float* lr, float rho, float eps, float clip, const float* loss, double weight,
+                                        float* hist, int rows_per_slot, double* acc, long long* cursor, int advance,
+                                        void* stream) {
+    if (!w || !g || !ms || !lr || n <= 0) return DCAHIP_EINVAL;
+    if (!al16(w) || !al16(g) || !al16(ms)) return DCAHIP_EINVAL;
+    if (hole_first < 0 || hole_len < 0 || (hole_first & 3) || (hole_len & 3) || hole_first + hole_len > (n & ~3L)) return DCAHIP_EINVAL;
+    long grid = (((n - hole_len) >> 2) + 255) / 256;
+    if (grid > 2048) grid = 2048;
+    if (grid < 1) grid = 1;
+    hipLaunchKernelGGL(rmsprop_clip_kernel, dim3((int)grid), dim3(256), 0,
+                       static_cast<hipStream_t>(stream), w, g, ms, n, lr, rho, eps, clip,
+                       StepEnd{loss, weight, hist, rows_per_slot, acc, cursor, advance, (loss || hist || acc || cursor) ? 1 : 0},
+                       hole_first >> 2, hole_len >> 2);
     return (int)hipGetLastError();
 }
 
@@ -2318,6 +2337,50 @@
     if (made >= 0 && sums_out)
         hipLaunchKernelGGL(stack_sums_combine_kernel, dim3(1), dim3(64), 0, st, (const float*)q.part_out, nwg, l[made].H, sums_out,
                            l[made].dbeta);
+    return (int)hipGetLastError();
+}
+
+static bool stack_rider_share(const dcahip_step_rider* d, int share, step_rider::StepRider* out) {
+    if (!d || (d->kind != DCAHIP_RIDER_UPDATE && d->kind != DCAHIP_RIDER_REDUCE)) return false;
+    if (d->shares < 1 || share < 0 || share >= d->shares || d->chunks <= 0 || d->hL <= 0 || d->ldws <= 0 || (d->ldws & 3)) return false;
+    if (d->chunks != (long)(d->hL + 1) * (d->ldws >> 2)) return false;
+    if (!d->gW || !d->w || !d->ms || !d->lr || !al16(d->gW) || !al16(d->w) || !al16(d->ms)) return false;
+    step_rider::StepRider r{};
+    r.kind = d->kind;
+    r.q0 = d->chunks * share / d->shares;
+    r.q1 = d->chunks * (share + 1) / d->shares;
+    r.dw = step_rider::ReduceDwArgs{d->ws, d->S, d->stride, d->hL, d->ldws, d->ldws, d->gW, d->ldws, d->theta_w, d->g_theta, d->G,
+                                    d->scale, d->ws2, d->S2, d->tail_tiles, d->ntail, d->plane, d->tail_first};
+    if (d->kind == DCAHIP_RIDER_REDUCE) {
+        if (!d->ws || d->S < 1 || d->ntail < 0 || d->ntail > step_rider::kMaxTiles || (d->ntail > 0 && (!d->ws2 || d->S2 < 1))) return false;
+        if (d->plane <= 0 || d->ldws % d->plane || d->plane > (long)step_rider::kMaxTiles * step_rider::kTileGenes) return false;
+        if (!step_rider::reduce_dw_vec(r.dw)) return false;
+        if ((d->g_theta != nullptr) != (d->theta_w != nullptr) || (d->g_theta && (d->G <= 0 || d->G > d->plane))) return false;
+        r.theta = d->g_theta && share == 0;
+    }
+    r.w = d->w; r.ms = d->ms; r.lr = d->lr; r.rho = d->rho; r.eps = d->eps; r.clip = d->clip;
+    const long nchunk = r.q1 > r.q0 ? r.q1 - r.q0 : (r.theta ? (long)d->G : 0L);
+    long nb = (nchunk + kRiderChunks * 256 - 1) / (kRiderChunks * 256);
+    if (nb > kRiderMaxBlocks) nb = kRiderMaxBlocks;
+    r.nblk = (int)nb;
+    *out = r;
+    return true;
+}
+
+extern "C" int dcahip_hidden_stack_bwd_rider(const dcahip_stack_bwd_layer* layers, int n, int B, float n_total, int act,
+                                             float* dZ0, long ldz0, int rows_per_wg, int step,
+                                             void* workspace, long workspace_bytes,
+                                             const dcahip_step_rider* rider, int share, void* stream) {
+    if (!stack_shape_ok(layers, n, B) || !dZ0 || !stack_workspace_ok(workspace, workspace_bytes, n, B)) return DCAHIP_EINVAL;
+    if (step < 0 || step > n || rows_per_wg != kStepRows) return DCAHIP_EINVAL;
+    int nwg = 0;
+    if (stack_plan(n, B, rows_per_wg, step, step, n + 2, &nwg)) return DCAHIP_EINVAL;
+    StackBwdLayer l[kStackMaxLayers];
+    if (!stack_bwd_layers(layers, n, act, true, l)) return DCAHIP_EINVAL;
+    float* part = reinterpret_cast<float*>(static_cast<char*>(workspace) + 256);
+    StepBwdArgs q = stack_bwd_step(l, n, B, n_total, act, dZ0, ldz0, step, nwg, part);
+    if (!stack_rider_share(rider, share, &q.rider)) return DCAHIP_EINVAL;
+    hipLaunchKernelGGL(stack_bwd_step_kernel, dim3(nwg + q.rider.nblk), dim3(256), 0, static_cast<hipStream_t>(stream), q);
     return (int)hipGetLastError();
 }
 
diff --git a/dca_amd/csrc/step_rider.hpp b/dca_amd/csrc/step_rider.hpp
--- /dev/null
+++ b/dca_amd/csrc/step_rider.hpp
@@ -0,0 +1,157 @@
+#pragma once
+#include <hip/hip_runtime.h>
+#include <stdint.h>
+#include "dcahip.h"
+
+namespace step_rider {
+
+constexpr int kTileGenes = 32;
+constexpr int kMaxTiles = 2048;
+
+__device__ __forceinline__ void rmsprop_clip_one(float& w, float& ms, float g, float lr, float rho, float eps, float clip) {
+    if (clip > 0.f) g = fminf(fmaxf(g, -clip), clip);
+    ms = rho * ms + (1.f - rho) * g * g;
+    w = w - lr * g / (sqrtf(ms) + eps);
+}
+
+__device__ __forceinline__ void rmsprop_clip_quad(float4& wv, float4& mv, const float4& gv, float lr, float rho, float eps,
+                                                  float clip) {
+    const float* gp = &gv.x; float* mp = &mv.x; float* wp = &wv.x;
+#pragma unroll
+    for (int j = 0; j < 4; ++j) rmsprop_clip_one(wp[j], mp[j], gp[j], lr, rho, eps, clip);
+}
+
+struct ReduceDwArgs {
+    const float* ws; int S; long stride; int hL; long ldws, ncols; float* gW; long ldg;
+    const float* theta_w; float* g_theta; int G;
+    float scale;
+    const float* ws2; int S2; const int* tail_tiles; int ntail; long plane;
+    int tail_first;
+};
+
+__device__ __forceinline__ void tail_bitmap_fill(const ReduceDwArgs& q, unsigned* tailbm) {
+    if (q.ntail > 0) {
+        for (int i = threadIdx.x; i < kMaxTiles / 32; i += 256) tailbm[i] = 0u;
+        __syncthreads();
+        for (int i = threadIdx.x; i < q.ntail; i += 256) {
+            const int tl = q.tail_tiles ? q.tail_tiles[i] : q.tail_first + i;
+            if (tl >= 0 && tl < kMaxTiles) atomicOr(&tailbm[tl >> 5], 1u << (tl & 31));
+        }
+        __syncthreads();
+    }
+}
+
+__device__ __forceinline__ bool tail_bitmap_test(const ReduceDwArgs& q, const unsigned* tailbm, long col_in_plane) {
+    const int tl = (int)(col_in_plane / kTileGenes);
+    return q.ntail > 0 && ((tailbm[tl >> 5] >> (tl & 31)) & 1u);
+}
+
+__host__ __device__ __forceinline__ bool reduce_dw_vec(const ReduceDwArgs& q) {
+    return (q.ncols & 3) == 0 && (q.ldws & 3) == 0 && (q.ldg & 3) == 0 && (q.stride & 3) == 0 && (q.plane & 3) == 0 &&
+           ((reinterpret_cast<uintptr_t>(q.ws) | reinterpret_cast<uintptr_t>(q.gW) | reinterpret_cast<uintptr_t>(q.ws2)) & 15) == 0;
+}
+
+__device__ __forceinline__ float4 reduce_dw_quad(const ReduceDwArgs& q, const unsigned* tailbm, long idx, long nq, float** dst) {
+    const long i = idx / nq, c = (idx - i * nq) << 2;
+    const bool tl = tail_bitmap_test(q, tailbm, c % q.plane);
+    const float* ws = tl ? q.ws2 : q.ws; const int S = tl ? q.S2 : q.S; const long stride = q.stride;
+    float4 v = *reinterpret_cast<const float4*>(ws + i * q.ldws + c);
+    if (S == 2) {
+        const float4 x = *reinterpret_cast<const float4*>(ws + stride + i * q.ldws + c);
+        v.x += x.x; v.y += x.y; v.z += x.z; v.w += x.w;
+    } else {
+        for (int s = 1; s < S; ++s) {
+            const float4 x = *reinterpret_cast<const float4*>(ws + (long)s * stride + i * q.ldws + c);
+            v.x += x.x; v.y += x.y; v.z += x.z; v.w += x.w;
+        }
+    }
+    const float sc = q.scale;
+    v.x *= sc; v.y *= sc; v.z *= sc; v.w *= sc;
+    *dst = q.gW + i * q.ldg + c;
+    return v;
+}
+
+__device__ __forceinline__ void reduce_theta_body(const ReduceDwArgs& q, const unsigned* tailbm, int bid, int nblk) {
+    if (!q.g_theta) return;
+    const int hL = q.hL;
+    for (long c = (long)bid * 256 + threadIdx.x; c < q.G; c += (long)nblk * 256) {
+        const bool tl = tail_bitmap_test(q, tailbm, c);
+        const float* ws = tl ? q.ws2 : q.ws; const int S = tl ? q.S2 : q.S; const long stride = q.stride;
+        float v = 0.f;
+        for (int s = 0; s < S; ++s) v += ws[(long)s * stride + (long)(hL + 1) * q.ldws + c];
+        const float e = expf(q.theta_w[c]);
+        q.g_theta[c] = (e >= 1e-3f && e <= 1e4f) ? v * q.scale * e : 0.f;
+    }
+}
+
+__device__ __forceinline__ void reduce_dw_body(const ReduceDwArgs& q, int bid, int nblk) {
+    const int hL = q.hL;
+    const long ldws = q.ldws, ncols = q.ncols; float* gW = q.gW; const long ldg = q.ldg;
+    const float sc = q.scale;
+    __shared__ unsigned tailbm[kMaxTiles / 32];
+    tail_bitmap_fill(q, tailbm);
+    if (reduce_dw_vec(q)) {
+        const long nq = ncols >> 2, totalq = (long)(hL + 1) * nq;
+        for (long idx = (long)bid * 256 + threadIdx.x; idx < totalq; idx += (long)nblk * 256) {
+            float* dst;
+            const float4 v = reduce_dw_quad(q, tailbm, idx, nq, &dst);
+            *reinterpret_cast<float4*>(dst) = v;
+        }
+    } else {
+        const long total = (long)(hL + 1) * ncols;
+        for (long idx = (long)bid * 256 + threadIdx.x; idx < total; idx += (long)nblk * 256) {
+            const long i = idx / ncols, c = idx - i * ncols;
+            const bool tl = tail_bitmap_test(q, tailbm, c % q.plane);
+            const float* ws = tl ? q.ws2 : q.ws; const int S = tl ? q.S2 : q.S;
+            float v = 0.f;
+            for (int s = 0; s < S; ++s) v += ws[(long)s * q.stride + i * ldws + c];
+            gW[i * ldg + c] = v * sc;
+        }
+    }
+    reduce_theta_body(q, tailbm, bid, nblk);
+}
+
+struct StepRider {
+    int kind, nblk, theta;
+    long q0, q1;
+    ReduceDwArgs dw;
+    float* w; float* ms; const float* lr; float rho, eps, clip;
+};
+
+__device__ __forceinline__ void step_rider_body(const StepRider& r, int bid) {
+    __shared__ unsigned tailbm[kMaxTiles / 32];
+    const ReduceDwArgs& q = r.dw;
+    const bool red = r.kind == DCAHIP_RIDER_REDUCE;
+    if (red) tail_bitmap_fill(q, tailbm);
+    const float lr = *r.lr;
+    const long nq = q.ncols >> 2;
+    const long stride = (long)r.nblk * 256;
+    for (long idx = r.q0 + (long)bid * 256 + threadIdx.x; idx < r.q1; idx += 2 * stride) {
+        const long idx1 = idx + stride < r.q1 ? idx + stride : idx;
+        const bool two = idx1 != idx;
+        float4 mv0 = reinterpret_cast<const float4*>(r.ms)[idx], mv1 = reinterpret_cast<const float4*>(r.ms)[idx1];
+        float4 wv0 = reinterpret_cast<const float4*>(r.w)[idx], wv1 = reinterpret_cast<const float4*>(r.w)[idx1];
+        float4 gv0, gv1;
+        if (red) {
+            float* d0; float* d1;
+            gv0 = reduce_dw_quad(q, tailbm, idx, nq, &d0);
+            gv1 = reduce_dw_quad(q, tailbm, idx1, nq, &d1);
+            *reinterpret_cast<float4*>(d0) = gv0;
+            if (two) *reinterpret_cast<float4*>(d1) = gv1;
+        } else {
+            gv0 = reinterpret_cast<const float4*>(q.gW)[idx];
+            gv1 = reinterpret_cast<const float4*>(q.gW)[idx1];
+        }
+        rmsprop_clip_quad(wv0, mv0, gv0, lr, r.rho, r.eps, r.clip);
+        rmsprop_clip_quad(wv1, mv1, gv1, lr, r.rho, r.eps, r.clip);
+        reinterpret_cast<float4*>(r.ms)[idx] = mv0;
+        reinterpret_cast<float4*>(r.w)[idx] = wv0;
+        if (two) {
+            reinterpret_cast<float4*>(r.ms)[idx1] = mv1;
+            reinterpret_cast<float4*>(r.w)[idx1] = wv1;
+        }
+    }
+    if (red && r.theta) reduce_theta_body(q, tailbm, bid, r.nblk);
+}
+
+}
diff --git a/dca_amd/engine.py b/dca_amd/engine.py
--- a/dca_amd/engine.py
+++ b/dca_amd/engine.py
@@ -3,6 +3,7 @@
 import numpy as np
 import torch
 
+from . import hip
 from . import prep as _prep
 
 BN_MOMENTUM = 0.99
@@ -308,6 +309,8 @@
             if lay.elempi else None
         self.ws_heads = None
         self._pending = None
+        self._rode = False
+        self._rider_steps = []
         self.W0T = None
         self.WhT = self.HT = self.XT = self.dZT = None
         self.pl = None
@@ -1301,6 +1304,7 @@
         w, g = self.w, self.g
         if comm.dp:
             self.set_world_counts(world_counts)
+        self._rode = False
         if B > 0:
             if self.csr is not None:
                 with self._t('csr_gather'):
@@ -1329,7 +1333,13 @@
                 self._pending = None
         if self.reg is not None:
             ops.l1l2_apply(self.reg, w, g, g[lay.P:], self.reg_ws)
-        fused_end = self.opt_kind == 'rmsprop' and not self.has_dropout and hasattr(ops, 'rmsprop_clip_end')
+        fused_end = self._fused_end()
+        if fused_end and self._rode:
+            with self._t('rmsprop_clip'):
+                ops.rmsprop_clip_hole_end(w, g, self.ms, lay.P, lay.seg['Wh'][0], (lay.hL + 1) * lay.NH, self.lr, RMS_RHO,
+                                          RMS_EPS, self.clip, g[lay.P:], float(Bg), self.hist,
+                                          rows_per_slot or max(self.Bmax, 1), self.acc, self.cursor, B)
+            return
         if fused_end:
             with self._t('rmsprop_clip'):
                 ops.rmsprop_clip_end(w, g, self.ms, lay.P, self.lr, RMS_RHO, RMS_EPS, self.clip, g[lay.P:], float(Bg),
@@ -1350,6 +1360,16 @@
         ops.step_end(g[lay.P:], float(Bg), self.hist, rows_per_slot or max(self.Bmax, 1), self.acc,
                      self.cursor, B)
 
+    def _fused_end(self):
+        return self.opt_kind == 'rmsprop' and not self.has_dropout and hasattr(self.ops, 'rmsprop_clip_end')
+
+    def _ride_heads(self, B):
+        return (self.cfg.ride_heads_update and not self.comm.dp and self.reg is None and self._fused_end()
+                and self.ws_heads is not None and hasattr(self.ops, 'heads_fused_deferred')
+                and hasattr(self.ops, 'hidden_stack_bwd_rider') and hasattr(self.ops, 'rmsprop_clip_hole_end')
+                and self._stack_coop(B) and not self._stack_chain(B) and not (self.stack_mode == 'coop' and B <= 256 * 64)
+                and self._stack_rows(B) == 32)
+
     def _heads_compact(self):
         kw = {'compact': self.cc} if self.cc is not None else {}
         if getattr(self, 'heads_d_exp', 0):
@@ -1384,25 +1404,50 @@
                 s = torch.zeros(2 * lay.hidden[i], dtype=torch.float32, device=self.dev)
                 self.comm.all_reduce_sum(s)
 
+    def _heads_fused_args(self, B, KL, inv_n):
+        lay, w, g = self.lay, self.w, self.g
+        return ((self._hl[0], self._hl[1], lay.view(w, 'Wh'), lay.NH,
+                 lay.view(w, 'bh'), lay.Gp,
+                 lay.view(w, 'theta_w') if lay.const_disp else None, self.Y,
+                 self.ldy, self.sf, self._kperm, self._kcur, B, KL, lay.G_out,
+                 self.ridge, inv_n, self.flags, lay.view(g, 'Wh'), lay.NH,
+                 lay.view(g, 'theta_w') if lay.const_disp else None,
+                 self._dhl, self._hl[1], self.partials, self.ws_heads),
+                dict(tile_order=self.tile_order, loss_out=g[lay.P:], **self._heads_compact()))
+
+    def _heads_fused_deferred(self, B, KL, inv_n):
+        lay = self.lay
+        args, kw = self._heads_fused_args(B, KL, inv_n)
+        r = self.ops.heads_fused_deferred(*args, **kw)
+        if r.kind == hip.RIDER_NONE:
+            return None
+        assert r.chunks * 4 == (lay.hL + 1) * lay.NH
+        off = lay.seg['Wh'][0]
+        r.w, r.ms, r.lr = hip.ptr(self.w[off:]), hip.ptr(self.ms[off:]), hip.ptr(self.lr)
+        r.rho, r.eps, r.clip = RMS_RHO, RMS_EPS, self.clip
+        L = len(lay.hidden)
+        self._rider_steps = list(range(1, L)) if L >= 2 else list(range(L + 1))
+        r.shares = len(self._rider_steps)
+        return r
+
     def heads_fused_launch(self, B, KL, inv_n):
-        lay, w, g = self.lay, self.w, self.g
-        self.ops.heads_fused(self._hl[0], self._hl[1], lay.view(w, 'Wh'), lay.NH,
-                             lay.view(w, 'bh'), lay.Gp,
-                             lay.view(w, 'theta_w') if lay.const_disp else None, self.Y,
-                             self.ldy, self.sf, self._kperm, self._kcur, B, KL, lay.G_out,
-                             self.ridge, inv_n, self.flags, lay.view(g, 'Wh'), lay.NH,
-                             lay.view(g, 'theta_w') if lay.const_disp else None,
-                             self._dhl, self._hl[1], self.partials, self.ws_heads,
-                             tile_order=self.tile_order, loss_out=g[lay.P:], **self._heads_compact())
+        args, kw = self._heads_fused_args(B, KL, inv_n)
+        self.ops.heads_fused(*args, **kw)
 
     def _forward_backward(self, B, Bg, inv_n):
         lay, ops, comm = self.lay, self.ops, self.comm
         w, g = self.w, self.g
         KL = self._hidden_forward(B, ('perm',), True, self.counts_world)
         self._last_heads_args = (B, KL, inv_n)
+        rider = None
+        self._rode = False
         if self.ws_heads is not None:
             with self._t('heads_fused'):
-                self.heads_fused_launch(B, KL, inv_n)
+                if self._ride_heads(B):
+                    rider = self._heads_fused_deferred(B, KL, inv_n)
+                    self._rode = rider is not None
+                else:
+                    self.heads_fused_launch(B, KL, inv_n)
         else:
             self._heads_backward_unfused(B, KL, inv_n)
         self._launch_heads_bucket()
@@ -1437,6 +1482,10 @@
                 ops.hidden_stack_bwd(layers, B, float(Bg), self.act, self.dZ[0], self.ldh[0], self.ws_stack, rows_per_wg=64)
             else:
                 for st in range(L + 2):
+                    if rider is not None and st in self._rider_steps:
+                        ops.hidden_stack_bwd_rider(layers, B, float(Bg), self.act, self.dZ[0], self.ldh[0], self.ws_stack,
+                                                   st, rider, self._rider_steps.index(st))
+                        continue
                     ops.hidden_stack_bwd(layers, B, float(Bg), self.act, self.dZ[0], self.ldh[0], self.ws_stack,
                                          rows_per_wg=self._stack_rows(B), steps=(st, st))
         for i in reversed(range(L)):
diff --git a/dca_amd/hip.py b/dca_amd/hip.py
--- a/dca_amd/hip.py
+++ b/dca_amd/hip.py
@@ -36,6 +36,20 @@
                 ('l1', _c.c_float * REG_MAX_SEGS), ('l2', _c.c_float * REG_MAX_SEGS)]
 
 
+class StepRider(_c.Structure):
+    _fields_ = [('kind', _c.c_int),
+                ('S', _c.c_int), ('S2', _c.c_int), ('ntail', _c.c_int), ('tail_first', _c.c_int), ('hL', _c.c_int), ('G', _c.c_int),
+                ('scale', _c.c_float),
+                ('ws', _c.c_void_p), ('ws2', _c.c_void_p), ('tail_tiles', _c.c_void_p),
+                ('stride', _c.c_long), ('ldws', _c.c_long), ('plane', _c.c_long), ('chunks', _c.c_long),
+                ('gW', _c.c_void_p), ('theta_w', _c.c_void_p), ('g_theta', _c.c_void_p),
+                ('shares', _c.c_int),
+                ('rho', _c.c_float), ('eps', _c.c_float), ('clip', _c.c_float),
+                ('w', _c.c_void_p), ('ms', _c.c_void_p), ('lr', _c.c_void_p)]
+
+
+RIDER_NONE, RIDER_UPDATE, RIDER_REDUCE = 0, 1, 2
+
 ACT_CODES = {'linear': 0, 'relu': 1, 'tanh': 2, 'sigmoid': 3, 'elu': 4, 'selu': 5, 'softplus': 6,
              'softsign': 7, 'LeakyReLU': 8, 'hard_sigmoid': 10, 'exponential': 11, 'swish': 12, 'gelu': 13}
 ACT_PRE = 12
@@ -44,7 +58,8 @@
 
 _SCALARS = {'int': _c.c_int, 'long': _c.c_long, 'long long': _c.c_long, 'unsigned long long': _c.c_ulonglong,
             'float': _c.c_float, 'double': _c.c_double}
-_STRUCTS = {'dcahip_small_layer': SmallLayer, 'dcahip_stack_bwd_layer': StackBwdLayer, 'dcahip_reg_desc': RegDesc}
+_STRUCTS = {'dcahip_small_layer': SmallLayer, 'dcahip_stack_bwd_layer': StackBwdLayer, 'dcahip_reg_desc': RegDesc,
+            'dcahip_step_rider': StepRider}
 _POINTEES = set(_SCALARS) | {'void', 'unsigned', 'unsigned char'}
 
 
diff --git a/dca_amd/ops.py b/dca_amd/ops.py
--- a/dca_amd/ops.py
+++ b/dca_amd/ops.py
@@ -143,6 +143,25 @@
                                             p(tile_order), p(loss_out), int(d_exp), hip.stream()), 'heads_fused')
         return n.value
 
+    def heads_fused_deferred(self, H, ldh, Wh, ldw, bh, plane, theta_w, Y, ldy, sf, perm, cursor, B, hL, G,
+                             ridge, inv_n, flags, gW, ldg, g_theta, dH, lddh, partials, ws, tile_order=None, loss_out=None,
+                             compact=None, d_exp=0):
+        n = ctypes.c_int(0)
+        pending = hip.StepRider()
+        p = hip.ptr
+        c = compact
+        hip.check(self.L.dcahip_heads_fused_deferred(p(H), ldh, p(Wh), ldw, p(bh), plane, p(theta_w), p(Y), ldy,
+                                                     p(c.Yc) if c is not None else None, c.ldc if c is not None else 0,
+                                                     p(c.ovf_ptr) if c is not None else None,
+                                                     p(c.ovf_col) if c is not None else None,
+                                                     p(c.ovf_val) if c is not None else None,
+                                                     p(sf), p(perm), p(cursor), B, hL, G, ridge, inv_n, flags,
+                                                     p(gW), ldg, p(g_theta), p(dH), lddh, p(partials),
+                                                     ctypes.byref(n), p(ws), ws.numel() * ws.element_size(),
+                                                     p(tile_order), p(loss_out), int(d_exp), ctypes.byref(pending),
+                                                     hip.stream()), 'heads_fused_deferred')
+        return pending
+
     def counts_compact_ld(self, G):
         return int(self.L.dcahip_counts_compact_ld(G))
 
@@ -328,6 +347,13 @@
                                                  int(rows_per_wg), first, last, hip.ptr(ws),
                                                  0 if ws is None else ws.numel() * ws.element_size(),
                                                  hip.stream()), 'hidden_stack_bwd')
+
+    def hidden_stack_bwd_rider(self, layers, B, n_total, act, dZ0, ldz0, ws, step, rider, share):
+        arr = self._bwd_layers(layers)
+        hip.check(self.L.dcahip_hidden_stack_bwd_rider(arr, len(layers), B, float(n_total), int(act), hip.ptr(dZ0), ldz0, 32,
+                                                       int(step), hip.ptr(ws), ws.numel() * ws.element_size(),
+                                                       ctypes.byref(rider), int(share), hip.stream()),
+                  'hidden_stack_bwd_rider')
 
     def _small_layers(self, layers):
         arr = (hip.SmallLayer * len(layers))()
@@ -766,6 +792,13 @@
         hip.check(self.L.dcahip_rmsprop_clip(p(w), p(g), p(ms), n, p(lr), rho, eps, clip, p(loss), weight, p(hist),
                                              rows_per_slot, p(acc), p(cursor), advance, hip.stream()), 'rmsprop_clip')
 
+    def rmsprop_clip_hole_end(self, w, g, ms, n, hole_first, hole_len, lr, rho, eps, clip, loss, weight, hist, rows_per_slot,
+                              acc, cursor, advance):
+        p = hip.ptr
+        hip.check(self.L.dcahip_rmsprop_clip_hole(p(w), p(g), p(ms), n, int(hole_first), int(hole_len), p(lr), rho, eps, clip,
+                                                  p(loss), weight, p(hist), rows_per_slot, p(acc), p(cursor), advance,
+                                                  hip.stream()), 'rmsprop_clip_hole')
+
     def rmsprop_clip(self, w, g, ms, n, lr, rho, eps, clip):
         self.rmsprop_clip_end(w, g, ms, n, lr, rho, eps, clip, None, 0.0, None, 0, None, None, 0)
 
diff --git a/include/dcahip.h b/include/dcahip.h
--- a/include/dcahip.h
+++ b/include/dcahip.h
@@ -87,6 +87,32 @@
                        double* loss_partials, int* n_partials_out,
                        void* workspace, long workspace_bytes, const int* tile_order,
                        float* loss_out, int d_exp, void* stream);
+
+#define DCAHIP_RIDER_NONE   0
+#define DCAHIP_RIDER_UPDATE 1
+#define DCAHIP_RIDER_REDUCE 2
+typedef struct dcahip_step_rider {
+    int kind;
+    int S, S2, ntail, tail_first, hL, G;
+    float scale;
+    const float* ws; const float* ws2; const int* tail_tiles;
+    long stride, ldws, plane, chunks;
+    float* gW; const float* theta_w; float* g_theta;
+    int shares;
+    float rho, eps, clip;
+    float* w; float* ms; const float* lr;
+} dcahip_step_rider;
+int dcahip_heads_fused_deferred(const float* H, long ldh, const float* Wh, long ldw, const float* bh,
+                                long plane, const float* theta_w,
+                                const float* y, long ldy,
+                                const unsigned char* yc, long ldc, const int* ovf_ptr, const int* ovf_col,
+                                const float* ovf_val, const float* sf,
+                                const int* perm, const long long* cursor,
+                                int B, int hL, int G, float ridge, float inv_n, int flags,
+                                float* gW, long ldg, float* g_theta, float* dH, long lddh,
+                                double* loss_partials, int* n_partials_out,
+                                void* workspace, long workspace_bytes, const int* tile_order,
+                                float* loss_out, int d_exp, dcahip_step_rider* pending, void* stream);
 int dcahip_x3_product_32x32(const float* A, const float* B, float* C, int K, void* stream);
 
 int dcahip_sgemm(int ta, int tb, int M, int N, int K,
@@ -168,6 +194,10 @@
 int dcahip_hidden_stack_bwd(const dcahip_stack_bwd_layer* layers, int n, int B, float n_total, int act,
                             float* dZ0, long ldz0, int rows_per_wg, int first_step, int last_step,
                             void* workspace, long workspace_bytes, void* stream);
+int dcahip_hidden_stack_bwd_rider(const dcahip_stack_bwd_layer* layers, int n, int B, float n_total, int act,
+                                  float* dZ0, long ldz0, int rows_per_wg, int step,
+                                  void* workspace, long workspace_bytes,
+                                  const dcahip_step_rider* rider, int share, void* stream);
 
 int dcahip_hidden_stack_step_blocks(int B);
 int dcahip_hidden_stack_fwd_sync(const dcahip_small_layer* layers, int n, int B, float momentum, float eps, int act,
@@ -255,6 +285,10 @@
                         float rho, float eps, float clip, const float* loss, double weight,
                         float* hist, int rows_per_slot, double* acc, long long* cursor, int advance,
                         void* stream);
+int dcahip_rmsprop_clip_hole(float* w, const float* g, float* ms, long n, long hole_first, long hole_len,
+                             const float* lr, float rho, float eps, float clip, const float* loss, double weight,
+                             float* hist, int rows_per_slot, double* acc, long long* cursor, int advance,
+                             void* stream);
 
 #define DCAHIP_OPT_SGD       0
 #define DCAHIP_OPT_RMSPROP   1
```
